# ducha-aiki/mods

Hardware: AMD Instinct MI355X
Metric: image-pairs/sec (1024x768, HessAff+RootSIFT over the affine view ladder, MFMA FGINN match, LO-RANSAC H) (higher is better)
Workload: dtype f32 (detect/describe) + u8 on the int8 matrix cores (distance matrix)

## Files before the change

### include/modsx.h

```cpp
#ifndef MODSX_H
#define MODSX_H
#include <stdint.h>
#ifdef __cplusplus
extern "C" {
#endif

#define MODSX_VERSION 100

typedef enum modsx_status {
  MODSX_OK = 0,
  MODSX_ERR_ARG = -1,
  MODSX_ERR_DEVICE = -2,
  MODSX_ERR_NOMEM = -3,
  MODSX_ERR_INTERNAL = -4,
  MODSX_ERR_CAPACITY = -5,
  MODSX_ERR_TIMEOUT = -6
} modsx_status;

enum { MODSX_FIXED_TH = 0, MODSX_RELATIVE_TH = 1, MODSX_FIXED_REG_NUMBER = 2, MODSX_RELATIVE_REG_NUMBER = 3,
       MODSX_NOT_LESS_THAN_REGIONS = 4 };
enum { MODSX_DET_HESSIAN = 0, MODSX_DET_DOG = 1, MODSX_DET_HARRIS = 2, MODSX_DET_MSER = 3 };
enum { MODSX_DESC_SIFT = 0, MODSX_DESC_ROOT_SIFT = 1, MODSX_DESC_HALF_SIFT = 2, MODSX_DESC_HALF_ROOT_SIFT = 3 };
#define MODSX_MAX_DESC 4
enum { MODSX_HESSIAN_DARK = 0, MODSX_HESSIAN_BRIGHT = 1, MODSX_HESSIAN_SADDLE = 2 };
// ... 40 lines not shown
  int reg_number;
  float rel_threshold, rel_reg_number;
} modsx_mser_params;

typedef struct modsx_sskp {
  int octave, level, r0, c0, r, c, type, pad;
  float b0, b1, b2, val;
  float x, y, s, pixelDistance;
} modsx_sskp;

typedef struct modsx_tentative {
  int q, t0, tj, t1;
  double d1, d2, d2by2ndcl, ratio;
} modsx_tentative;

typedef struct modsx_pair_params {
  modsx_hessaff_params det;
  double ori_mrSize; int ori_patchSize; int ori_maxAngles; double ori_threshold;
  double desc_mrSize; int desc_patchSize; int desc_photoNorm; int desc_type; double desc_maxBinValue;
  double match_ratio; double contradDist; int nn;
  double duplicateDist;
  double err_threshold, confidence; int max_samples; int localOptimization; double HLAFCoef; int doSymmCheck;
  unsigned ransac_seed;
  int useF;
  double LAFCoef;
  int errorType;
  int detector;
  modsx_mser_params mser;
  int n_desc;
  int desc_types[MODSX_MAX_DESC];
  double desc_ratios[MODSX_MAX_DESC];
} modsx_pair_params;

typedef struct modsx_pair_result {
  int n_regions1, n_regions2;
  int n_tentatives;
  int n_unique;
  int n_ransac_inliers;
  int n_verified;
  int ransac_samples, ransac_lo;
  double H[9];
  modsx_tentative *tentatives;
  unsigned char *ransac_inlier;
  unsigned char *verified;
} modsx_pair_result;

typedef struct modsx_view {
  double zoom, tilt, phi, InitSigma;
  int doBlur;
} modsx_view;

typedef struct modsx_ctx modsx_ctx;
typedef struct modsx_image modsx_image;

int modsx_version(void);
const char *modsx_last_error(void);
void modsx_free(void *p);

modsx_ctx *modsx_create(int device_id);
void modsx_destroy(modsx_ctx *ctx);
int modsx_synchronize(modsx_ctx *ctx);

void modsx_default_hessaff_params(modsx_hessaff_params *p);
void modsx_default_pair_params(modsx_pair_params *p);

modsx_image *modsx_image_upload(modsx_ctx *ctx, const void *pixels, int rows, int cols, int channels, int dtype);
int modsx_image_update(modsx_ctx *ctx, modsx_image *img, const void *pixels, int rows, int cols, int channels, int dtype);
modsx_image *modsx_image_wrap_device(modsx_ctx *ctx, const float *dev_pixels, int rows, int cols);
void modsx_image_free(modsx_ctx *ctx, modsx_image *img);
int modsx_image_download(modsx_ctx *ctx, const modsx_image *img, float *out);

int modsx_detect_affine_keypoints(modsx_ctx *ctx, const modsx_image *img, const modsx_hessaff_params *par,
                                  double tilt, double zoom, modsx_keypoint **out);
int modsx_detect_scalespace(modsx_ctx *ctx, const modsx_image *img, const modsx_hessaff_params *par,
                            modsx_sskp **out);
int modsx_octave_levels(modsx_ctx *ctx, const modsx_image *img, const modsx_hessaff_params *par, float *blurs,
                        float *resps);
int modsx_gaussian_blur(modsx_ctx *ctx, const modsx_image *img, float sigma, float *out);
int modsx_resize_half(modsx_ctx *ctx, const modsx_image *img, float *out, int *orows, int *ocols);

int modsx_response(modsx_ctx *ctx, const modsx_image *img, int detector_type, float norm, float *out);

int modsx_detect_affine_regions(const modsx_keypoint *kps, int n, int img_id, int det_type, modsx_region *out);

void modsx_default_mser_params(modsx_mser_params *p);
int modsx_detect_msers(modsx_ctx *ctx, const modsx_image *img, const modsx_mser_params *par, double tilt, double zoom,
                       modsx_keypoint **out);
int modsx_detect_msers_u8(const unsigned char *gray, int rows, int cols, const modsx_mser_params *par, double tilt,
                          double zoom, modsx_keypoint **out);

int modsx_detect_orientation(modsx_ctx *ctx, const modsx_image *img, const modsx_region *in, int n, double mrSize,
                             int patchSize, int doHalfSIFT, int maxAngNum, double th, int addUpRight,
                             modsx_region **out);

int modsx_reproject_regions(modsx_region *regs, int n, const double *H, int orig_w, int orig_h);
int modsx_reproject_regions_touch_boundary(modsx_region *regs, int n, const double *H, int orig_w, int orig_h, double mrSize);

int modsx_describe_regions(modsx_ctx *ctx, const modsx_image *img, const modsx_region *regs, int n, double mrSize,
                           int patchSize, int fast_extraction, int photoNorm, int desc_type, double maxBinValue,
                           float *desc);

int modsx_match_fginn(modsx_ctx *ctx, const float *desc1, int n1, const float *desc2, int n2, const double *pos2,
                      double ratio, double contradDist, int nn, modsx_tentative **out);

int modsx_duplicate_filtering(const double *pts, const double *key, int T, double r, int do_sort, int *order,
                              unsigned char *keep);

int modsx_ransac_h(const double *u, int len, double th, double conf, int max_sam, double *H, unsigned char *inl,
                   int *data_out, int oriented_constraint, int doSymCheck, unsigned seed, double *score_J);

int modsx_loransac_h(const double *pts, const double *laf1, const double *laf2, int T, double err_threshold,
                     double confidence, int max_samples, int localOptimization, double HLAFCoef, int doSymmCheck,
                     unsigned seed, double *H, double *Hraw, unsigned char *inl, unsigned char *keep,
                     int *data_out);

int modsx_ransac_h_errtype(const double *u, int len, double th, double conf, int max_sam, double *H, unsigned char *inl,
                           int *data_out, int oriented_constraint, int doSymCheck, int error_type, unsigned seed,
                           double *score_J);
int modsx_loransac_h_errtype(const double *pts, const double *laf1, const double *laf2, int T, double err_threshold,
                             double confidence, int max_samples, int localOptimization, double HLAFCoef, int doSymmCheck,
                             int error_type, unsigned seed, double *H, double *Hraw, unsigned char *inl,
                             unsigned char *keep, int *data_out);

int modsx_ransac_f(const double *u, int len, double th, double conf, int max_sam, int do_lo, unsigned inl_limit,
                   int error_type, int doSymCheck, unsigned seed, double *F, unsigned char *inl, int *data_out);

int modsx_loransac_f(const double *pts, const double *laf1, const double *laf2, int T, double err_threshold,
                     double confidence, int max_samples, int localOptimization, double LAFCoef, int doSymmCheck,
                     int error_type, unsigned seed, double *F, unsigned char *inl, unsigned char *keep, int *data_out);
int modsx_verify_device_stats(long *out, int reset);
int modsx_verify_device_timing(long *out, int reset);

int modsx_match_pair(modsx_ctx *ctx, const modsx_image *img1, const modsx_image *img2,
                     const modsx_pair_params *par, modsx_pair_result *res);
void modsx_pair_result_release(modsx_pair_result *res);

int modsx_match_pairs(modsx_ctx *const *ctxs, int n_ctx, const modsx_image *const *imgs1,
                      const modsx_image *const *imgs2, int n_pairs, const modsx_pair_params *par,
                      modsx_pair_result *results);

int modsx_match_pairs_views(modsx_ctx *const *ctxs, int n_ctx, const modsx_image *const *imgs1,
                            const modsx_image *const *imgs2, int n_pairs, const modsx_view *views, int n_views,
                            const modsx_pair_params *par, modsx_pair_result *results);

int modsx_last_batch_verify(double *sum_ms, int *pairs, int *threads);
int modsx_last_match_geometry(int *qs, int *fat, int *S, int *tiles_per_split, int *ntiles_ub);
int modsx_describe_counters(modsx_ctx *ctx, long *out, int n);
int modsx_debug_orientation_counts(unsigned long long *launched, unsigned long long *skipped, int reset);
int modsx_debug_reproject_certain_drop(const modsx_region *regs, int n, const double *H, int orig_w, int orig_h, double boxk,
                                       unsigned char *drop);
int modsx_debug_describe_plan(const modsx_region *regs, const int *counts, int nimages, double mr_size, int fast_extraction,
                              unsigned long long arena_floats, long *counters, int n, long *cuts, int cap_cuts, int *n_cuts);
int modsx_debug_baumberg_geometry(int n, int W, int variant, int chunk, int *geometry);
int modsx_debug_baumberg(modsx_ctx *ctx, const modsx_image *const *planes, int nplanes, const int *plane_of, const float *xyspd,
                         int n, const modsx_hessaff_params *par, int variant, int chunk, float *u, int *ok, int *iters,
                         int *geometry);
int modsx_debug_check_borders(const float *tuples, int n, unsigned char *touch);
int modsx_last_timings(modsx_ctx *ctx, double *ms6);

int modsx_set_vs_pars(const double *scale_set, int ns, const double *tilt_set, int nt, double phi_base,
                      double InitSigma, int doBlur, modsx_view *par, int cap, modsx_view *prev, int *nprev,
                      int cap_prev);

modsx_image *modsx_synth_view(modsx_ctx *ctx, const modsx_image *gray, const modsx_view *view, double *H9,
                              int *is_identity);

int modsx_detect_describe_views(modsx_ctx *ctx, const modsx_image *img, const modsx_view *views, int nviews,
                                const modsx_pair_params *par, int view_begin, int view_step, modsx_region **regs,
                                float **desc, void *dev_desc_u8, long dev_cap, int *view_counts);

int modsx_match_fginn_device(modsx_ctx *ctx, const void *dev_desc1_u8, int n1, const void *dev_desc2_u8, int n2,
                             const double *pos2, double ratio, double contradDist, int nn, modsx_tentative **out);

#define MODSX_DB_MAX_ROWS 16777216L
typedef struct modsx_db modsx_db;
modsx_db *modsx_db_create(modsx_ctx *ctx, const void *rows, long n, int dtype);
void modsx_db_free(modsx_ctx *ctx, modsx_db *db);
long modsx_db_rows(const modsx_db *db);
int modsx_db_nearest(modsx_ctx *ctx, const modsx_db *db, const float *desc, int n, float *dmin);
int modsx_match_fginn_db(modsx_ctx *ctx, const float *desc1, int n1, const float *desc2, int n2, const double *pos2,
                         double ratio, double contradDist, int nn, const modsx_db *db, modsx_tentative **out, double **d2byDB);
int modsx_match_fginn_db_device(modsx_ctx *ctx, const void *dev_desc1_u8, int n1, const void *dev_desc2_u8, int n2,
                                const double *pos2, double ratio, double contradDist, int nn, const modsx_db *db,
                                modsx_tentative **out, double **d2byDB);
int modsx_set_fginn_db(modsx_ctx *ctx, const modsx_db *db);

int modsx_match_pair_views(modsx_ctx *ctx, const modsx_image *img1, const modsx_image *img2,
                           const modsx_view *views, int nviews, const modsx_pair_params *par,
                           modsx_pair_result *res);

typedef struct modsx_ladder_step {
  const modsx_view *views;
  int nviews;
  double match_ratio;
  int detector;
  int n_desc;
  int desc_types[MODSX_MAX_DESC];
  double desc_ratios[MODSX_MAX_DESC];
} modsx_ladder_step;
int modsx_match_ladder(modsx_ctx *ctx, const modsx_image *img1, const modsx_image *img2,
                       const modsx_ladder_step *steps, int nsteps, int min_matches, const modsx_pair_params *par,
                       modsx_pair_result *res, int *steps_done);

typedef struct modsx_rep modsx_rep;
modsx_rep *modsx_rep_create(modsx_ctx *ctx);
void modsx_rep_free(modsx_ctx *ctx, modsx_rep *rep);
int modsx_rep_add_views(modsx_ctx *ctx, modsx_rep *rep, const modsx_image *img, const modsx_ladder_step *step,
                        const modsx_pair_params *par);
int modsx_rep_append(modsx_ctx *ctx, modsx_rep *rep, int detector, int desc_type, const modsx_region *regs, const void *desc, int dtype,
                     int n);
int modsx_rep_class(modsx_ctx *ctx, const modsx_rep *rep, int detector, int desc_type, modsx_region **regs, unsigned char **desc_u8);
int modsx_rep_match_fginn(modsx_ctx *ctx, const modsx_rep *rep1, const modsx_rep *rep2, int detector, int desc_type, double ratio,
                          double contradDist, int nn, modsx_tentative **out);
typedef struct { int detector, desc_type; double ratio; } modsx_rep_class_sel;
int modsx_match_reps(modsx_ctx *const *ctxs, int n_ctx, const modsx_rep *rep1, const modsx_rep *const *reps2, int n,
                     const modsx_rep_class_sel *classes, int n_classes, const modsx_pair_params *par, modsx_pair_result *results);
int modsx_match_one_to_many(modsx_ctx *const *ctxs, int n_ctx, const modsx_image *img1, const modsx_image *const *imgs2, int n,
                            const modsx_ladder_step *steps, int nsteps, int min_matches, const modsx_pair_params *par,
                            modsx_pair_result *results, int *steps_done);

typedef struct modsx_comm modsx_comm;
int modsx_comm_unique_id(void *id128);
int modsx_comm_loopback_id(void *id128, int world);
modsx_comm *modsx_comm_create(modsx_ctx *ctx, const void *id128, int rank, int world);
void modsx_comm_destroy(modsx_comm *comm);
int modsx_comm_set_lanes(modsx_comm *comm, int nlanes);
int modsx_comm_attach(modsx_comm *comm, modsx_ctx *ctx, int lane);
int modsx_comm_lane_done(modsx_comm *comm, int lane);
int modsx_comm_reset_lanes(modsx_comm *comm);
int modsx_comm_set_timeout(modsx_comm *comm, int milliseconds);
int modsx_comm_info(const modsx_comm *comm, int *rank, int *world, int *rccl_version, long *bytes_gathered, long *collectives);
int modsx_comm_stats(const modsx_comm *comm, long *out, int n);
#define MODSX_EXCHANGE_ALL_GATHER 0
#define MODSX_EXCHANGE_OWNER 1
int modsx_comm_set_exchange(modsx_comm *comm, int mode);
int modsx_shard_owner_plan(const int *item_counts, int nimages, int nviews, int world, int rank, const int *image_owner, int *sends,
                           int *recvs, int *jobs, int cap, long *n);
int modsx_view_block_order(const int *counts, int world, int nviews, int *src, int cap, int *maxrows_out);
#define MODSX_SHARD_ROW_REGION 0
#define MODSX_SHARD_ROW_KP 1
long modsx_shard_block_bytes(int items, int block_rows, int ndesc, int row_format);
long modsx_shard_block_pack(const modsx_region *regs, const unsigned char *const *desc, int ndesc, int n, const int *counts, int items,
                            int rc_local, int block_rows, int row_format, void *block);
long modsx_shard_blocks_unpack(const void *blocks, int world, int items, int block_rows, int ndesc, int row_format, void *regs_out,
                               unsigned char *const *desc_out, long cap, int *item_counts, int *need_rows);
long modsx_shard_device_pack(modsx_ctx *ctx, const modsx_region *regs, const unsigned char *const *desc, int ndesc, int n, int row_format,
                             void *rows_out);
long modsx_shard_device_unpack(modsx_ctx *ctx, const void *blocks, int world, int items, int block_rows, int ndesc, int row_format,
                               void *regs_out, unsigned char *const *desc_out, double *pos_out, long cap);
int modsx_detect_describe_views_sharded(modsx_ctx *ctx, modsx_comm *comm, const modsx_image *img, const modsx_view *views,
                                        int nviews, const modsx_pair_params *par, modsx_region **regs, void **dev_desc_u8,
                                        int *view_counts);
int modsx_match_fginn_sharded(modsx_ctx *ctx, modsx_comm *comm, const void *dev_desc1_u8, int n1, const void *dev_desc2_u8,
                              int n2, const double *pos2, double ratio, double contradDist, int nn, modsx_tentative **out);
int modsx_match_pair_views_sharded(modsx_ctx *ctx, modsx_comm *comm, const modsx_image *img1, const modsx_image *img2,
                                   const modsx_view *views, int nviews, const modsx_pair_params *par, int owner,
                                   modsx_pair_result *res);
int modsx_match_pairs_views_sharded(modsx_ctx *ctx, modsx_comm *comm, const modsx_image *const *imgs1, const modsx_image *const *imgs2,
                                    int n_pairs, const modsx_view *views, int nviews, const modsx_pair_params *par, int owner_base,
                                    modsx_pair_result *results);
int modsx_match_ladder_sharded(modsx_ctx *ctx, modsx_comm *comm, const modsx_image *img1, const modsx_image *img2,
                               const modsx_ladder_step *steps, int nsteps, int min_matches, const modsx_pair_params *par,
                               modsx_pair_result *res, int *steps_done);

typedef struct modsx_region_class {
  const char *det_name, *desc_name;
  const modsx_region *regs;
  const float *desc;
  int n, dim, stride;
} modsx_region_class;
int modsx_save_regions(const char *path, const modsx_region_class *classes, int nclasses);
int modsx_load_regions(const char *path, const char *det_name, const char *desc_name, modsx_region **regs, float **desc,
                       int *dim, char *found_det, char *found_desc);

int modsx_profile(modsx_ctx *ctx, int enable);
int modsx_kernel_stats(modsx_ctx *ctx, double *ms, double *work, long *launches, int n);

#ifdef __cplusplus
}
#endif
#endif
```

### mods_amd/__init__.py

```python
import ctypes as C
import os
import subprocess

import numpy as np

_HERE = os.path.dirname(os.path.abspath(__file__))
LIB_PATH = os.environ.get("MODSX_LIB", os.path.join(_HERE, "libmodsx.so"))

KEYPOINT = np.dtype([("x", "f8"), ("y", "f8"), ("a11", "f8"), ("a12", "f8"), ("a21", "f8"), ("a22", "f8"),
                     ("s", "f8"), ("response", "f8"), ("octave_number", "i4"), ("pyramid_scale", "f8"),
                     ("sub_type", "i4")], align=True)
REGION = np.dtype([("img_id", "i4"), ("img_reproj_id", "i4"), ("id", "i4"), ("parent_id", "i4"), ("type", "i4"),
                   ("det_kp", KEYPOINT), ("reproj_kp", KEYPOINT)], align=True)
SSKP = np.dtype([("octave", "i4"), ("level", "i4"), ("r0", "i4"), ("c0", "i4"), ("r", "i4"), ("c", "i4"),
                 ("type", "i4"), ("pad", "i4"), ("b0", "f4"), ("b1", "f4"), ("b2", "f4"), ("val", "f4"),
                 ("x", "f4"), ("y", "f4"), ("s", "f4"), ("pixelDistance", "f4")], align=True)
TENT = np.dtype([("q", "i4"), ("t0", "i4"), ("tj", "i4"), ("t1", "i4"), ("d1", "f8"), ("d2", "f8"),
                 ("d2by2ndcl", "f8"), ("ratio", "f8")], align=True)


class HessAffParams(C.Structure):
    _fields_ = [("threshold", C.c_float), ("mode", C.c_int), ("reg_number", C.c_int),
                ("rel_threshold", C.c_float), ("rel_reg_number", C.c_float), ("numberOfScales", C.c_int),
                ("initialSigma", C.c_float), ("edgeEigenValueRatio", C.c_double), ("border", C.c_int),
                ("maxIterations", C.c_int), ("convergenceThreshold", C.c_float), ("smmWindowSize", C.c_int),
                ("affInitialSigma", C.c_float), ("doBaumberg", C.c_int), ("detectorType", C.c_int)]


class MserParams(C.Structure):
    _fields_ = [("min_size", C.c_int), ("max_area", C.c_double), ("min_margin", C.c_double), ("relative", C.c_int),
                ("mode", C.c_int), ("reg_number", C.c_int), ("rel_threshold", C.c_float), ("rel_reg_number", C.c_float)]


class PairParams(C.Structure):
    _fields_ = [("det", HessAffParams),
                ("ori_mrSize", C.c_double), ("ori_patchSize", C.c_int), ("ori_maxAngles", C.c_int),
                ("ori_threshold", C.c_double),
                ("desc_mrSize", C.c_double), ("desc_patchSize", C.c_int), ("desc_photoNorm", C.c_int),
                ("desc_type", C.c_int), ("desc_maxBinValue", C.c_double),
                ("match_ratio", C.c_double), ("contradDist", C.c_double), ("nn", C.c_int),
                ("duplicateDist", C.c_double),
                ("err_threshold", C.c_double), ("confidence", C.c_double), ("max_samples", C.c_int),
                ("localOptimization", C.c_int), ("HLAFCoef", C.c_double), ("doSymmCheck", C.c_int),
                ("ransac_seed", C.c_uint), ("useF", C.c_int), ("LAFCoef", C.c_double), ("errorType", C.c_int),
                ("detector", C.c_int), ("mser", MserParams),
                ("n_desc", C.c_int), ("desc_types", C.c_int * 4), ("desc_ratios", C.c_double * 4)]


class View(C.Structure):
    _fields_ = [("zoom", C.c_double), ("tilt", C.c_double), ("phi", C.c_double), ("InitSigma", C.c_double),
                ("doBlur", C.c_int)]


def make_view(tilt=1.0, phi=0.0, zoom=1.0, init_sigma=0.5, do_blur=1):
    v = View()
    v.zoom, v.tilt, v.phi, v.InitSigma, v.doBlur = zoom, tilt, phi, init_sigma, do_blur
    return v


def _view_array(views):
    arr = (View * len(views))()
    for i, v in enumerate(views):
        arr[i].zoom, arr[i].tilt, arr[i].phi, arr[i].InitSigma, arr[i].doBlur = v.zoom, v.tilt, v.phi, v.InitSigma, v.doBlur
    return arr


class LadderStep(C.Structure):
    _fields_ = [("views", C.c_void_p), ("nviews", C.c_int), ("match_ratio", C.c_double), ("detector", C.c_int),
                ("n_desc", C.c_int), ("desc_types", C.c_int * 4), ("desc_ratios", C.c_double * 4)]


class PairResult(C.Structure):
    _fields_ = [("n_regions1", C.c_int), ("n_regions2", C.c_int), ("n_tentatives", C.c_int), ("n_unique", C.c_int),
                ("n_ransac_inliers", C.c_int), ("n_verified", C.c_int), ("ransac_samples", C.c_int),
                ("ransac_lo", C.c_int), ("H", C.c_double * 9), ("tentatives", C.c_void_p),
                ("ransac_inlier", C.c_void_p), ("verified", C.c_void_p)]


class RepClassSel(C.Structure):
    _fields_ = [("detector", C.c_int), ("desc_type", C.c_int), ("ratio", C.c_double)]


EXPORTS = ["modsx_version", "modsx_last_error", "modsx_free", "modsx_create", "modsx_destroy", "modsx_synchronize",
           "modsx_default_hessaff_params", "modsx_default_pair_params", "modsx_image_upload", "modsx_image_update",
           "modsx_image_wrap_device", "modsx_image_free", "modsx_image_download", "modsx_detect_affine_keypoints",
           "modsx_detect_scalespace", "modsx_octave_levels", "modsx_gaussian_blur", "modsx_resize_half", "modsx_response",
           "modsx_detect_affine_regions", "modsx_detect_orientation", "modsx_reproject_regions", "modsx_reproject_regions_touch_boundary",
           "modsx_describe_regions", "modsx_match_fginn", "modsx_duplicate_filtering", "modsx_ransac_h",
           "modsx_loransac_h", "modsx_ransac_h_errtype", "modsx_loransac_h_errtype", "modsx_ransac_f", "modsx_loransac_f", "modsx_match_pair", "modsx_match_pairs", "modsx_match_pairs_views", "modsx_pair_result_release",
           "modsx_set_vs_pars", "modsx_synth_view", "modsx_detect_describe_views", "modsx_match_fginn_device",
           "modsx_match_pair_views", "modsx_match_ladder", "modsx_save_regions", "modsx_load_regions", "modsx_default_mser_params", "modsx_detect_msers", "modsx_detect_msers_u8", "modsx_last_timings", "modsx_profile",
           "modsx_kernel_stats", "modsx_last_batch_verify", "modsx_last_match_geometry", "modsx_describe_counters", "modsx_comm_unique_id", "modsx_comm_create", "modsx_comm_destroy", "modsx_comm_info",
           "modsx_view_block_order", "modsx_detect_describe_views_sharded", "modsx_match_fginn_sharded",
           "modsx_match_pair_views_sharded", "modsx_match_pairs_views_sharded", "modsx_match_ladder_sharded", "modsx_comm_loopback_id", "modsx_comm_set_lanes",
           "modsx_comm_attach", "modsx_comm_lane_done", "modsx_comm_reset_lanes", "modsx_comm_set_timeout", "modsx_comm_stats",
           "modsx_shard_block_bytes", "modsx_shard_block_pack", "modsx_shard_blocks_unpack", "modsx_shard_device_pack",
           "modsx_shard_device_unpack", "modsx_verify_device_stats", "modsx_verify_device_timing", "modsx_comm_set_exchange",
           "modsx_shard_owner_plan", "modsx_db_create", "modsx_db_free", "modsx_db_rows", "modsx_db_nearest",
           "modsx_match_fginn_db", "modsx_match_fginn_db_device", "modsx_set_fginn_db",
           "modsx_debug_orientation_counts", "modsx_debug_reproject_certain_drop", "modsx_debug_describe_plan",
           "modsx_debug_baumberg_geometry", "modsx_debug_baumberg", "modsx_debug_check_borders",
           "modsx_rep_create", "modsx_rep_free", "modsx_rep_add_views", "modsx_rep_append", "modsx_rep_class",
           "modsx_rep_match_fginn", "modsx_match_reps", "modsx_match_one_to_many"]
EXPORTS_DEGENSAC = ["exp_ransacHcustom", "exp_ransacFcustom", "HDs", "HDsi", "HDsidx", "HDsSym", "HDsiSym", "HDsSymidx",
                    "HDsSymMax", "HDsiSymMax", "HDsSymidxMax", "FDs", "FDsSym", "exFDs", "exFDsSym",
                    "modsx_ransac_set_seed"]

SHARD_ROW_REGION, SHARD_ROW_KP = 0, 1
EXCHANGE_ALL_GATHER, EXCHANGE_OWNER = 0, 1
DESCRIBE_COUNTERS = ("calls", "chunks", "max_chunks", "chunks_mid_image", "chunks_later_image", "jobs", "direct_jobs", "fused_windows",
                     "lds_row_tiles", "lds_col_tiles", "sample_tiles", "global_row_tiles", "global_col_tiles", "clamped_windows")
KP_FIELDS = ("x", "y", "a11", "a12", "a21", "a22", "s")
KERNEL_CLASSES = ["blur_hess", "hessian", "resize", "nms_localize", "baumberg", "orientation", "patch_sample",
                  "blur_rows", "describe", "match_fginn", "gray", "warp_affine", "view_blur", "blur_cols", "match_sweep1", "match_db"]


def build(force=False):
    src = os.path.join(_HERE, "csrc")
    srcs = [os.path.join(src, f) for f in os.listdir(src) if f.endswith((".hip", ".cpp", ".hpp"))]
    srcs.append(os.path.join(_HERE, "..", "include", "modsx.h"))
    stale = (not os.path.exists(LIB_PATH)) or any(os.path.getmtime(s) > os.path.getmtime(LIB_PATH) for s in srcs)
    if force or stale:
        subprocess.check_call(["make", "-C", src, "-j8"], stdout=subprocess.DEVNULL)
    return LIB_PATH


_lib = None


def lib():
    global _lib
    if _lib is None:
        if not os.path.exists(LIB_PATH):
            raise RuntimeError("libmodsx.so is not built; run __graft_entry__.build() (needs hipcc)")
        L = C.CDLL(LIB_PATH)
        L.modsx_last_error.restype = C.c_char_p
        L.modsx_create.restype = C.c_void_p
        L.modsx_create.argtypes = [C.c_int]
        L.modsx_comm_create.restype = C.c_void_p
        L.modsx_comm_create.argtypes = [C.c_void_p, C.c_void_p, C.c_int, C.c_int]
        L.modsx_comm_destroy.argtypes = [C.c_void_p]
        L.modsx_comm_info.argtypes = [C.c_void_p] + [C.c_void_p] * 5
        L.modsx_comm_loopback_id.argtypes = [C.c_void_p, C.c_int]
        L.modsx_comm_set_lanes.argtypes = [C.c_void_p, C.c_int]
        L.modsx_comm_attach.argtypes = [C.c_void_p, C.c_void_p, C.c_int]
        L.modsx_comm_lane_done.argtypes = [C.c_void_p, C.c_int]
        L.modsx_comm_reset_lanes.argtypes = [C.c_void_p]
        L.modsx_comm_set_timeout.argtypes = [C.c_void_p, C.c_int]
        L.modsx_comm_stats.argtypes = [C.c_void_p, C.c_void_p, C.c_int]
        L.modsx_destroy.argtypes = [C.c_void_p]
        L.modsx_free.argtypes = [C.c_void_p]
        L.modsx_image_upload.restype = C.c_void_p
        L.modsx_image_upload.argtypes = [C.c_void_p, C.c_void_p, C.c_int, C.c_int, C.c_int, C.c_int]
        L.modsx_image_update.argtypes = [C.c_void_p, C.c_void_p, C.c_void_p, C.c_int, C.c_int, C.c_int, C.c_int]
        L.modsx_debug_last_batch_verify_each.argtypes = [C.c_void_p, C.c_int]
        L.modsx_image_wrap_device.restype = C.c_void_p
        L.modsx_image_wrap_device.argtypes = [C.c_void_p, C.c_void_p, C.c_int, C.c_int]
        L.modsx_image_free.argtypes = [C.c_void_p, C.c_void_p]
        L.modsx_db_create.restype = C.c_void_p
        L.modsx_db_create.argtypes = [C.c_void_p, C.c_void_p, C.c_long, C.c_int]
        L.modsx_db_free.restype = None
        L.modsx_db_free.argtypes = [C.c_void_p, C.c_void_p]
        L.modsx_db_rows.restype = C.c_long
        L.modsx_db_rows.argtypes = [C.c_void_p]
        L.modsx_db_nearest.argtypes = [C.c_void_p, C.c_void_p, C.c_void_p, C.c_int, C.c_void_p]
        L.modsx_set_fginn_db.argtypes = [C.c_void_p, C.c_void_p]
        L.modsx_debug_reproject_certain_drop.argtypes = [C.c_void_p, C.c_int, C.c_void_p, C.c_int, C.c_int, C.c_double, C.c_void_p]
        L.modsx_describe_counters.argtypes = [C.c_void_p, C.c_void_p, C.c_int]
        L.modsx_debug_orientation_counts.argtypes = [C.c_void_p, C.c_void_p, C.c_int]
        L.modsx_debug_describe_plan.argtypes = [C.c_void_p, C.c_void_p, C.c_int, C.c_double, C.c_int, C.c_ulonglong, C.c_void_p, C.c_int,
                                                C.c_void_p, C.c_int, C.c_void_p]
        L.modsx_debug_baumberg_geometry.argtypes = [C.c_int, C.c_int, C.c_int, C.c_int, C.c_void_p]
        L.modsx_debug_baumberg.argtypes = [C.c_void_p, C.c_void_p, C.c_int, C.c_void_p, C.c_void_p, C.c_int, C.c_void_p, C.c_int, C.c_int,
                                           C.c_void_p, C.c_void_p, C.c_void_p, C.c_void_p]
        L.modsx_debug_check_borders.argtypes = [C.c_void_p, C.c_int, C.c_void_p]
        L.modsx_rep_create.restype = C.c_void_p
        L.modsx_rep_create.argtypes = [C.c_void_p]
        L.modsx_rep_free.restype = None
        L.modsx_rep_free.argtypes = [C.c_void_p, C.c_void_p]
        L.modsx_rep_add_views.argtypes = [C.c_void_p, C.c_void_p, C.c_void_p, C.c_void_p, C.c_void_p]
        L.modsx_rep_append.argtypes = [C.c_void_p, C.c_void_p, C.c_int, C.c_int, C.c_void_p, C.c_void_p, C.c_int, C.c_int]
        L.modsx_rep_class.argtypes = [C.c_void_p, C.c_void_p, C.c_int, C.c_int, C.c_void_p, C.c_void_p]
        L.modsx_rep_match_fginn.argtypes = [C.c_void_p, C.c_void_p, C.c_void_p, C.c_int, C.c_int, C.c_double, C.c_double, C.c_int,
                                            C.c_void_p]
        L.modsx_match_reps.argtypes = [C.c_void_p, C.c_int, C.c_void_p, C.c_void_p, C.c_int, C.c_void_p, C.c_int, C.c_void_p,
                                       C.c_void_p]
        L.modsx_match_one_to_many.argtypes = [C.c_void_p, C.c_int, C.c_void_p, C.c_void_p, C.c_int, C.c_void_p, C.c_int, C.c_int,
                                              C.c_void_p, C.c_void_p, C.c_void_p]
        L.modsx_synth_view.restype = C.c_void_p
        L.modsx_synth_view.argtypes = [C.c_void_p, C.c_void_p, C.c_void_p, C.c_void_p, C.c_void_p]
        _lib = L
    return _lib


def _err():
    return lib().modsx_last_error().decode()


def _p(a):
    return a.ctypes.data_as(C.c_void_p)


def _check(rc, what):
    if rc < 0:
        raise RuntimeError("%s failed (%d): %s" % (what, rc, _err()))
    return rc


def default_hessaff_params(**kw):
    p = HessAffParams()
    lib().modsx_default_hessaff_params(C.byref(p))
    for k, v in kw.items():
        setattr(p, k, v)
    return p


def default_mser_params(**kw):
    p = MserParams()
    lib().modsx_default_mser_params(C.byref(p))
    for k, v in kw.items():
        setattr(p, k, v)
    return p


def detect_msers_u8(gray, params=None, tilt=1.0, zoom=1.0):
    params = params or default_mser_params()
    g = np.ascontiguousarray(gray, np.uint8)
    out = C.c_void_p()
    n = _check(lib().modsx_detect_msers_u8(_p(g), g.shape[0], g.shape[1], C.byref(params), C.c_double(tilt),
                                           C.c_double(zoom), C.byref(out)), "detect_msers_u8")
    return _take(out, n, KEYPOINT)


def default_pair_params(**kw):
    p = PairParams()
    lib().modsx_default_pair_params(C.byref(p))
    descs = kw.pop("descs", None)
    if descs is not None:
        _set_descs(p, descs)
    for k, v in kw.items():
        if hasattr(p.det, k) and not hasattr(p, k):
            setattr(p.det, k, v)
        else:
            setattr(p, k, v)
    return p


def _set_descs(obj, descs):
    obj.n_desc = len(descs)
    for i, (t, r) in enumerate(descs):
        obj.desc_types[i] = int(t)
        obj.desc_ratios[i] = float(r)


def _take(ptr, n, dtype):
    if n <= 0:
        if ptr:
            lib().modsx_free(ptr)
        return np.zeros(0, dtype)
    buf = (C.c_char * (n * dtype.itemsize)).from_address(ptr.value if hasattr(ptr, "value") else ptr)
    arr = np.frombuffer(buf, dtype=dtype, count=n).copy()
    lib().modsx_free(ptr)
    return arr


def detect_affine_regions(kps, img_id=0, det_type=0):
    kps = np.ascontiguousarray(kps, KEYPOINT)
    out = np.zeros(len(kps), REGION)
    _check(lib().modsx_detect_affine_regions(_p(kps), len(kps), img_id, det_type, _p(out)), "detect_affine_regions")
    return out


def reproject_regions(regs, H, w, h):
    regs = np.ascontiguousarray(regs, REGION).copy()
    H = np.ascontiguousarray(H, np.float64).reshape(9)
    n = _check(lib().modsx_reproject_regions(_p(regs), len(regs), _p(H), int(w), int(h)), "reproject_regions")
    return regs[:n].copy()


def reproject_regions_touch_boundary(regs, H, w, h, mr_size=3.0 * 3.0 ** 0.5):
    regs = np.ascontiguousarray(regs, REGION).copy()
    H = np.ascontiguousarray(H, np.float64).reshape(9)
    n = _check(lib().modsx_reproject_regions_touch_boundary(_p(regs), len(regs), _p(H), int(w), int(h), C.c_double(mr_size)),
               "reproject_regions_touch_boundary")
    return regs[:n].copy()


def duplicate_filtering(pts, key, r=2.0, do_sort=True):
    pts = np.ascontiguousarray(pts, np.float64)
    key = np.ascontiguousarray(key, np.float64)
    T = len(pts)
    order = np.zeros(max(T, 1), np.int32)
    keep = np.zeros(max(T, 1), np.uint8)
    _check(lib().modsx_duplicate_filtering(_p(pts), _p(key), T, C.c_double(r), int(do_sort), _p(order), _p(keep)),
           "duplicate_filtering")
    return order[:T], keep[:T].astype(bool)


def ransac_h(u, th, conf=0.99, max_sam=100000, oriented=1, sym_check=1, seed=1):
    u = np.ascontiguousarray(u, np.float64)
    n = len(u)
    H = np.zeros(9)
    inl = np.zeros(n, np.uint8)
    dout = np.zeros(3, np.int32)
    J = C.c_double(0)
    rc = _check(lib().modsx_ransac_h(_p(u), n, C.c_double(th), C.c_double(conf), int(max_sam), _p(H), _p(inl), _p(dout),
                                     int(oriented), int(sym_check), C.c_uint(seed), C.byref(J)), "ransac_h")
    return dict(n=rc, H=H, inl=inl.astype(bool), samples=int(dout[0]), lo_count=int(dout[1]),
                ori_rejects=int(dout[2]), J=J.value)


def loransac_h(pts, laf1, laf2, err_threshold=3.0, confidence=0.99, max_samples=100000, lo=1, hlaf_coef=12.0,
               sym_check=1, seed=1, error_type=0):
    pts = np.ascontiguousarray(pts, np.float64)
    laf1 = np.ascontiguousarray(laf1, np.float64)
    laf2 = np.ascontiguousarray(laf2, np.float64)
    T = len(pts)
    H, Hraw = np.zeros(9), np.zeros(9)
    inl = np.zeros(max(T, 1), np.uint8)
    keep = np.zeros(max(T, 1), np.uint8)
    dout = np.zeros(3, np.int32)
    n = _check(lib().modsx_loransac_h_errtype(_p(pts), _p(laf1), _p(laf2), T, C.c_double(err_threshold),
                                              C.c_double(confidence), int(max_samples), int(lo), C.c_double(hlaf_coef),
                                              int(sym_check), int(error_type), C.c_uint(seed), _p(H), _p(Hraw), _p(inl),
                                              _p(keep), _p(dout)), "loransac_h")
    return dict(n=n, H=H.reshape(3, 3), Hraw=Hraw, inl=inl[:T].astype(bool), keep=keep[:T].astype(bool),
                samples=int(dout[0]), lo_count=int(dout[1]), ori_rejects=int(dout[2]))
# ... 105 lines not shown
        return int(lib().modsx_db_rows(self.h)) if self.h else 0

    def free(self):
        if self.h:
            lib().modsx_db_free(self.ctx.h, self.h)
            self.h = None


def _ladder_steps(steps):
    arr = (LadderStep * len(steps))()
    keep = []
    for i, st in enumerate(steps):
        va = _view_array(st[0])
        keep.append(va)
        arr[i].views = C.cast(va, C.c_void_p)
        arr[i].nviews = len(st[0])
        arr[i].match_ratio = float(st[1])
        arr[i].detector = int(st[2]) if len(st) > 2 else 0
        if len(st) > 3 and st[3] is not None:
            _set_descs(arr[i], st[3])
    return arr, keep


class Rep(object):

    def __init__(self, ctx):
        self.ctx = ctx
        self.h = lib().modsx_rep_create(ctx.h)
        if not self.h:
            raise RuntimeError("modsx_rep_create failed: " + _err())

    def add_views(self, img, views, params, detector=0, descs=None, ctx=None):
        arr, keep = _ladder_steps([(views, 0.0, detector, descs)])
        return _check(lib().modsx_rep_add_views((ctx or self.ctx).h, self.h, img.h, arr, C.addressof(params)), "rep_add_views")

    def append(self, regs, desc, detector=0, desc_type=1, ctx=None):
        regs = np.ascontiguousarray(regs, REGION)
        d = np.ascontiguousarray(desc)
        if d.dtype != np.uint8:
            d = np.ascontiguousarray(d, np.float32)
        if d.shape != (len(regs), 128):
            raise ValueError("rep.append: [n][128] descriptors for n regions are expected")
        return _check(lib().modsx_rep_append((ctx or self.ctx).h, self.h, int(detector), int(desc_type), _p(regs), _p(d),
                                             0 if d.dtype == np.uint8 else 1, len(regs)), "rep_append")

    def regions(self, detector=0, desc_type=1, want_desc=True):
        regs, desc = C.c_void_p(), C.c_void_p()
        n = _check(lib().modsx_rep_class(self.ctx.h, self.h, int(detector), int(desc_type), C.byref(regs),
                                         C.byref(desc) if want_desc else None), "rep_class")
        r = _take(regs, n, REGION)
        if not want_desc:
            return r
        return r, _take(desc, n * 128, np.dtype(np.uint8)).reshape(n, 128)

    def count(self, detector=0, desc_type=1):
        return _check(lib().modsx_rep_class(self.ctx.h, self.h, int(detector), int(desc_type), None, None), "rep_class")

    def free(self):
        if self.h:
            lib().modsx_rep_free(self.ctx.h, self.h)
            self.h = None


class Context(object):

    def __init__(self, device=0):
        self.h = lib().modsx_create(int(device))
        if not self.h:
            raise RuntimeError("modsx_create failed: " + _err())

    def close(self):
        if self.h:
            lib().modsx_destroy(self.h)
            self.h = None

    def __del__(self):
        try:
            self.close()
        except Exception:
            pass

    def _c(self):
        return C.c_void_p(self.h)

    def upload(self, pixels):
        a = np.ascontiguousarray(pixels)
        if a.dtype == np.uint8:
            dtype = 0
        else:
            a = np.ascontiguousarray(a, np.float32)
            dtype = 1
        ch = 1 if a.ndim == 2 else a.shape[2]
        h = lib().modsx_image_upload(self._c(), _p(a), a.shape[0], a.shape[1], ch, dtype)
        if not h:
            raise RuntimeError("modsx_image_upload failed: " + _err())
        return Image(self, h, a.shape[0], a.shape[1])

    def wrap_device(self, dev_ptr, rows, cols):
        h = lib().modsx_image_wrap_device(self._c(), C.c_void_p(dev_ptr), rows, cols)
        if not h:
            raise RuntimeError("modsx_image_wrap_device failed: " + _err())
        return Image(self, h, rows, cols)

    def synchronize(self):
        _check(lib().modsx_synchronize(self._c()), "synchronize")

    def gaussian_blur(self, img, sigma):
        out = np.empty((img.rows, img.cols), np.float32)
        _check(lib().modsx_gaussian_blur(self._c(), C.c_void_p(img.h), C.c_float(sigma), _p(out)), "gaussian_blur")
        return out

    def response(self, img, detector_type, norm):
        out = np.zeros((img.rows, img.cols), np.float32)
        _check(lib().modsx_response(self._c(), C.c_void_p(img.h), int(detector_type), C.c_float(norm), _p(out)), "response")
        return out

    def resize_half(self, img):
        r, c = C.c_int(), C.c_int()
        _check(lib().modsx_resize_half(self._c(), C.c_void_p(img.h), None, C.byref(r), C.byref(c)), "resize_half")
        out = np.empty((r.value, c.value), np.float32)
        _check(lib().modsx_resize_half(self._c(), C.c_void_p(img.h), _p(out), C.byref(r), C.byref(c)), "resize_half")
        return out

    def octave_levels(self, img, params):
        L = params.numberOfScales + 2
        blurs = np.empty((L, img.rows, img.cols), np.float32)
        resps = np.empty((L, img.rows, img.cols), np.float32)
        _check(lib().modsx_octave_levels(self._c(), C.c_void_p(img.h), C.byref(params), _p(blurs), _p(resps)),
               "octave_levels")
        return blurs, resps

    def detect_scalespace(self, img, params):
        out = C.c_void_p()
        n = _check(lib().modsx_detect_scalespace(self._c(), C.c_void_p(img.h), C.byref(params), C.byref(out)),
                   "detect_scalespace")
        return _take(out, n, SSKP)

    def detect_affine_keypoints(self, img, params, tilt=1.0, zoom=1.0):
        out = C.c_void_p()
        n = _check(lib().modsx_detect_affine_keypoints(self._c(), C.c_void_p(img.h), C.byref(params),
                                                       C.c_double(tilt), C.c_double(zoom), C.byref(out)),
                   "detect_affine_keypoints")
        return _take(out, n, KEYPOINT)

    def debug_baumberg(self, planes, plane_of, xyspd, params, variant=0, chunk=0):
        plane_of = np.ascontiguousarray(plane_of, np.int32)
        xyspd = np.ascontiguousarray(xyspd, np.float32).reshape(-1, 4)
        n = len(plane_of)
        assert len(xyspd) == n
        ptrs = (C.c_void_p * max(1, len(planes)))(*[im.h for im in planes])
        u = np.zeros((max(n, 1), 4), np.float32)
        ok, iters = np.zeros(max(n, 1), np.int32), np.zeros(max(n, 1), np.int32)
        geo = np.zeros(4, np.int32)
        _check(lib().modsx_debug_baumberg(self._c(), ptrs, len(planes), _p(plane_of), _p(xyspd), n, C.byref(params), int(variant),
                                          int(chunk), _p(u), _p(ok), _p(iters), _p(geo)), "debug_baumberg")
        return dict(u=u[:n], ok=ok[:n], iters=iters[:n], geometry=dict(zip(BAUMBERG_GEOMETRY, (int(x) for x in geo))))

    def detect_orientation(self, img, regs, mr_size=1.0, patch_size=41, half=0, max_ang=1, th=0.8, upright=0):
        regs = np.ascontiguousarray(regs, REGION)
        out = C.c_void_p()
        n = _check(lib().modsx_detect_orientation(self._c(), C.c_void_p(img.h), _p(regs), len(regs),
                                                  C.c_double(mr_size), patch_size, half, max_ang, C.c_double(th),
                                                  upright, C.byref(out)), "detect_orientation")
        return _take(out, n, REGION)

    def describe_regions(self, img, regs, mr_size=5.1962, patch_size=41, fast=0, photo_norm=1, desc_type=1,
                         max_bin=0.2):
        regs = np.ascontiguousarray(regs, REGION)
        desc = np.zeros((len(regs), 128), np.float32)
        _check(lib().modsx_describe_regions(self._c(), C.c_void_p(img.h), _p(regs), len(regs), C.c_double(mr_size),
                                            patch_size, fast, photo_norm, desc_type, C.c_double(max_bin), _p(desc)),
               "describe_regions")
        return desc

    def describe_counters(self):
        v = (C.c_long * len(DESCRIBE_COUNTERS))()
        n = _check(lib().modsx_describe_counters(self._c(), v, len(DESCRIBE_COUNTERS)), "describe_counters")
        assert n == len(DESCRIBE_COUNTERS), n
        return dict(zip(DESCRIBE_COUNTERS, (int(x) for x in v)))

    def match_fginn(self, d1, d2, pos2, ratio=0.8, contrad_dist=30.0, nn=50):
        d1 = np.ascontiguousarray(d1, np.float32)
        d2 = np.ascontiguousarray(d2, np.float32)
        pos2 = np.ascontiguousarray(pos2, np.float64)
        out = C.c_void_p()
        n = _check(lib().modsx_match_fginn(self._c(), _p(d1), len(d1), _p(d2), len(d2), _p(pos2), C.c_double(ratio),
                                           C.c_double(contrad_dist), nn, C.byref(out)), "match_fginn")
        return _take(out, n, TENT)

    def db_create(self, rows):
        a = np.ascontiguousarray(rows)
        if a.dtype != np.uint8:
            a = np.ascontiguousarray(a, np.float32)
        if a.ndim != 2 or a.shape[1] != 128:
            raise ValueError("db_create: an [n][128] array is expected")
        h = lib().modsx_db_create(self._c(), _p(a), a.shape[0], 0 if a.dtype == np.uint8 else 1)
        if not h:
            raise RuntimeError("modsx_db_create failed: " + _err())
        return Db(self, h)

    def db_nearest(self, db, desc):
        d = np.ascontiguousarray(desc, np.float32)
        out = np.empty(len(d), np.float32)
        _check(lib().modsx_db_nearest(self._c(), C.c_void_p(db.h), _p(d), len(d), _p(out)), "db_nearest")
        return out

    def match_fginn_db(self, d1, d2, pos2, db, ratio=0.8, contrad_dist=30.0, nn=50):
        d1 = np.ascontiguousarray(d1, np.float32)
        d2 = np.ascontiguousarray(d2, np.float32)
        pos2 = np.ascontiguousarray(pos2, np.float64)
        out, dd = C.c_void_p(), C.c_void_p()
        n = _check(lib().modsx_match_fginn_db(self._c(), _p(d1), len(d1), _p(d2), len(d2), _p(pos2), C.c_double(ratio),
                                              C.c_double(contrad_dist), nn, C.c_void_p(db.h if db is not None else None),
                                              C.byref(out), C.byref(dd)), "match_fginn_db")
        return _take(out, n, TENT), _take(dd, n, np.dtype("f8"))

    def match_fginn_db_device(self, d1_ptr, n1, d2_ptr, n2, pos2, db, ratio=0.8, contrad_dist=30.0, nn=50):
        pos2 = np.ascontiguousarray(pos2, np.float64)
        out, dd = C.c_void_p(), C.c_void_p()
        n = _check(lib().modsx_match_fginn_db_device(self._c(), C.c_void_p(d1_ptr), int(n1), C.c_void_p(d2_ptr), int(n2),
                                                     _p(pos2), C.c_double(ratio), C.c_double(contrad_dist), nn,
                                                     C.c_void_p(db.h), C.byref(out), C.byref(dd)), "match_fginn_db_device")
        return _take(out, n, TENT), _take(dd, n, np.dtype("f8"))

    def set_fginn_db(self, db):
        _check(lib().modsx_set_fginn_db(self._c(), C.c_void_p(db.h) if db is not None else None), "set_fginn_db")

    def synth_view(self, img, view):
        H = np.zeros(9)
        ident = C.c_int(0)
        h = lib().modsx_synth_view(self._c(), C.c_void_p(img.h), C.byref(view), _p(H), C.byref(ident))
        if not h:
            raise RuntimeError("modsx_synth_view failed: " + _err())
        rows, cols = C.c_int(), C.c_int()
        out = Image(self, h, 0, 0)
        out.rows, out.cols = _image_dims(h)
        return out, H.reshape(3, 3), bool(ident.value)

    def detect_describe_views(self, img, views, params, view_begin=0, view_step=1, want_desc=True, dev_desc=None,
                              dev_cap=0, want_counts=False):
        arr = _view_array(views)
        regs = C.c_void_p()
        desc = C.c_void_p()
        counts = (C.c_int * len(views))()
        n = _check(lib().modsx_detect_describe_views(self._c(), C.c_void_p(img.h), arr, len(views), C.byref(params),
                                                     int(view_begin), int(view_step), C.byref(regs),
                                                     C.byref(desc) if want_desc else None,
                                                     C.c_void_p(dev_desc) if dev_desc else None, C.c_long(dev_cap),
                                                     counts),
                   "detect_describe_views")
        r = _take(regs, n, REGION)
        d = None
        if want_desc:
            d = _take(desc, n * 128, np.dtype("f4")).reshape(n, 128) if n else np.zeros((0, 128), np.float32)
        if want_counts:
            return r, d, np.array(list(counts), np.int64)
        return r, d

    def match_fginn_device(self, d1_ptr, n1, d2_ptr, n2, pos2, ratio=0.8, contrad_dist=30.0, nn=50):
        pos2 = np.ascontiguousarray(pos2, np.float64)
        out = C.c_void_p()
        n = _check(lib().modsx_match_fginn_device(self._c(), C.c_void_p(d1_ptr), int(n1), C.c_void_p(d2_ptr), int(n2),
                                                  _p(pos2), C.c_double(ratio), C.c_double(contrad_dist), nn,
                                                  C.byref(out)), "match_fginn_device")
        return _take(out, n, TENT)

    def rep_match_fginn(self, rep1, rep2, detector=0, desc_type=1, ratio=0.8, contrad_dist=30.0, nn=50):
        out = C.c_void_p()
        n = _check(lib().modsx_rep_match_fginn(self.h, rep1.h, rep2.h, int(detector), int(desc_type), C.c_double(ratio),
                                               C.c_double(contrad_dist), int(nn), C.byref(out)), "rep_match_fginn")
        return _take(out, n, TENT)

    def match_pair_views(self, img1, img2, views, params):
        arr = _view_array(views)
        res = PairResult()
        _check(lib().modsx_match_pair_views(self._c(), C.c_void_p(img1.h), C.c_void_p(img2.h), arr, len(views),
                                            C.byref(params), C.byref(res)), "match_pair_views")
        return _unpack_pair_result(res)

    def comm_create(self, id128, rank, world):
        h = lib().modsx_comm_create(self._c(), id128, int(rank), int(world))
        if not h:
            raise RuntimeError("modsx_comm_create failed: " + _err())
        return h

    def detect_describe_views_sharded(self, comm, img, views, params):
        arr = _view_array(views)
        regs, dptr = C.c_void_p(), C.c_void_p()
        counts = (C.c_int * len(views))()
        n = _check(lib().modsx_detect_describe_views_sharded(self._c(), C.c_void_p(comm), C.c_void_p(img.h), arr, len(views),
                                                             C.byref(params), C.byref(regs), C.byref(dptr), counts),
                   "detect_describe_views_sharded")
        return _take(regs, n, REGION), dptr.value, np.array(list(counts), np.int64)

    def match_fginn_sharded(self, comm, d1_ptr, n1, d2_ptr, n2, pos2, ratio=0.8, contrad_dist=30.0, nn=50):
        pos2 = np.ascontiguousarray(pos2, np.float64)
        out = C.c_void_p()
        n = _check(lib().modsx_match_fginn_sharded(self._c(), C.c_void_p(comm), C.c_void_p(d1_ptr), int(n1), C.c_void_p(d2_ptr),
                                                   int(n2), _p(pos2), C.c_double(ratio), C.c_double(contrad_dist), nn,
                                                   C.byref(out)), "match_fginn_sharded")
        return _take(out, n, TENT)

    def match_pair_views_sharded(self, comm, img1, img2, views, params, owner=0):
        arr = _view_array(views)
        res = PairResult()
        _check(lib().modsx_match_pair_views_sharded(self._c(), C.c_void_p(comm), C.c_void_p(img1.h), C.c_void_p(img2.h), arr,
                                                    len(views), C.byref(params), int(owner), C.byref(res)),
               "match_pair_views_sharded")
        return _unpack_pair_result(res)

    def match_pairs_views_sharded(self, comm, imgs1, imgs2, views, params, owner_base=0, arrays=True):
        n = len(imgs1)
        a1 = (C.c_void_p * n)(*[im.h for im in imgs1])
        a2 = (C.c_void_p * n)(*[im.h for im in imgs2])
        arr = _view_array(views)
        res = (PairResult * n)()
        _check(lib().modsx_match_pairs_views_sharded(self._c(), C.c_void_p(comm), a1, a2, n, arr, len(views), C.byref(params),
                                                     int(owner_base), res), "match_pairs_views_sharded")
        return [_unpack_pair_result(res[i], arrays) for i in range(n)]

    def shard_device_pack(self, regs, descs, row_format=SHARD_ROW_REGION):
        L = lib()
        L.modsx_shard_device_pack.restype = C.c_long
        regs = np.ascontiguousarray(regs, REGION)
        descs = [np.ascontiguousarray(d, np.uint8) for d in descs]
        out = np.zeros((len(regs), shard_region_bytes(row_format) + 128 * len(descs)), np.uint8)
        _check(L.modsx_shard_device_pack(self._c(), _p(regs), _ptr_array(descs), len(descs), len(regs), int(row_format), _p(out)),
               "shard_device_pack")
        return out

    def shard_device_unpack(self, blocks, world, items, block_rows, ndesc=1, row_format=SHARD_ROW_REGION):
        L = lib()
        L.modsx_shard_device_unpack.restype = C.c_long
        blocks = np.ascontiguousarray(blocks, np.uint8)
        cap = world * block_rows
        regs = np.zeros(cap, REGION) if row_format == SHARD_ROW_REGION else np.zeros((cap, 7), np.float64)
        descs = [np.zeros((cap, 128), np.uint8) for _ in range(ndesc)]
        pos = np.zeros((cap, 2), np.float64)
        _check(L.modsx_shard_device_unpack(self._c(), _p(blocks), int(world), int(items), int(block_rows), int(ndesc), int(row_format),
                                           _p(regs), _ptr_array(descs), _p(pos), C.c_long(cap)), "shard_device_unpack")
        return regs, descs, pos

    def detect_msers(self, img, params=None, tilt=1.0, zoom=1.0):
        params = params or default_mser_params()
        out = C.c_void_p()
        n = _check(lib().modsx_detect_msers(self._c(), C.c_void_p(img.h), C.byref(params), C.c_double(tilt),
                                            C.c_double(zoom), C.byref(out)), "detect_msers")
        return _take(out, n, KEYPOINT)

    def match_ladder(self, img1, img2, steps, params, min_matches=10, comm=None):
        arr = (LadderStep * len(steps))()
        keep = []
        for i, st in enumerate(steps):
            views, ratio = st[0], st[1]
            va = _view_array(views)
            keep.append(va)
            arr[i].views = C.cast(va, C.c_void_p)
            arr[i].nviews = len(views)
            arr[i].match_ratio = float(ratio)
            arr[i].detector = int(st[2]) if len(st) > 2 else 0
            if len(st) > 3 and st[3] is not None:
                _set_descs(arr[i], st[3])
        res = PairResult()
        done = C.c_int(0)
        if comm is not None:
            _check(lib().modsx_match_ladder_sharded(self._c(), C.c_void_p(comm), C.c_void_p(img1.h), C.c_void_p(img2.h), arr,
                                                    len(steps), int(min_matches), C.byref(params), C.byref(res),
                                                    C.byref(done)), "match_ladder_sharded")
        else:
            _check(lib().modsx_match_ladder(self._c(), C.c_void_p(img1.h), C.c_void_p(img2.h), arr, len(steps),
                                            int(min_matches), C.byref(params), C.byref(res), C.byref(done)), "match_ladder")
        return _unpack_pair_result(res), done.value

    def match_pair(self, img1, img2, params):
        res = PairResult()
        _check(lib().modsx_match_pair(self._c(), C.c_void_p(img1.h), C.c_void_p(img2.h), C.byref(params),
                                      C.byref(res)), "match_pair")
        return _unpack_pair_result(res)

    def last_timings(self):
        t = (C.c_double * 6)()
        _check(lib().modsx_last_timings(self._c(), t), "last_timings")
        return dict(zip(["detect", "orient", "describe", "match", "verify", "total"], list(t)))

    def profile(self, enable=True):
        _check(lib().modsx_profile(self._c(), int(enable)), "profile")

    def kernel_stats(self):
        n = len(KERNEL_CLASSES)
        ms, work = (C.c_double * n)(), (C.c_double * n)()
        launches = (C.c_long * n)()
        _check(lib().modsx_kernel_stats(self._c(), ms, work, launches, n), "kernel_stats")
        return {k: dict(ms=ms[i], work=work[i], launches=launches[i]) for i, k in enumerate(KERNEL_CLASSES)}


class _ImageStruct(C.Structure):
    _fields_ = [("d", C.c_void_p), ("rows", C.c_int), ("cols", C.c_int), ("owned", C.c_bool)]


def last_batch_verify_each():
    n = lib().modsx_debug_last_batch_verify_each(None, 0)
    out = np.zeros(max(n, 1), np.float64)
    n = min(n, lib().modsx_debug_last_batch_verify_each(_p(out), len(out)))
    return out[:n]


def last_batch_verify():
    ms, n, t = C.c_double(), C.c_int(), C.c_int()
    lib().modsx_last_batch_verify(C.byref(ms), C.byref(n), C.byref(t))
    return ms.value, n.value, t.value


def last_match_geometry():
    v = [C.c_int() for _ in range(5)]
    lib().modsx_last_match_geometry(*[C.byref(x) for x in v])
    return dict(zip(("qs", "fat", "S", "tiles_per_split", "ntiles_ub"), (x.value for x in v)))


BAUMBERG_GEOMETRY = ("kernel", "chunk", "nchunks", "grid")


def baumberg_geometry(n, W=19, variant=0, chunk=0):
    geo = np.zeros(4, np.int32)
    _check(lib().modsx_debug_baumberg_geometry(int(n), int(W), int(variant), int(chunk), _p(geo)), "baumberg_geometry")
    return dict(zip(BAUMBERG_GEOMETRY, (int(x) for x in geo)))


def check_borders(tuples):
    t = np.ascontiguousarray(tuples, np.float32).reshape(-1, 9)
    out = np.zeros(max(1, len(t)), np.uint8)
    _check(lib().modsx_debug_check_borders(_p(t), len(t), _p(out)), "check_borders")
    return out[:len(t)].astype(bool)


def orientation_counts(reset=False):
    a, b = C.c_ulonglong(), C.c_ulonglong()
    lib().modsx_debug_orientation_counts(C.byref(a), C.byref(b), int(reset))
    return a.value, b.value


def reproject_certain_drop(regs, H, w, h, boxk=2 * 3.0 * 3.0 ** 0.5):
    regs = np.ascontiguousarray(regs, REGION)
    H = np.ascontiguousarray(H, np.float64).reshape(9)
    drop = np.zeros(max(1, len(regs)), np.uint8)
    _check(lib().modsx_debug_reproject_certain_drop(_p(regs), len(regs), _p(H), int(w), int(h), C.c_double(boxk), _p(drop)),
           "reproject_certain_drop")
    return drop[:len(regs)].astype(bool)


DEFAULT_ARENA_FLOATS = 192 << 18


def describe_plan(regs, mr_size, fast=0, arena_floats=DEFAULT_ARENA_FLOATS, max_cuts=4096):
    lists = [regs] if isinstance(regs, np.ndarray) else list(regs)
    counts = np.array([len(r) for r in lists], np.int32)
    flat = np.ascontiguousarray(np.concatenate([np.asarray(r).view(REGION) for r in lists]) if lists else np.zeros(0, REGION), REGION)
    cnt = (C.c_long * len(DESCRIBE_COUNTERS))()
    cuts = (C.c_long * max(1, max_cuts))()
    ncuts = C.c_int(0)
    rc = lib().modsx_debug_describe_plan(_p(flat), _p(counts), len(lists), C.c_double(mr_size), int(fast), int(arena_floats), cnt,
                                         len(DESCRIBE_COUNTERS), cuts, max_cuts, C.byref(ncuts))
    assert ncuts.value <= max_cuts, "describe_plan: %d cuts, room for %d" % (ncuts.value, max_cuts)
    return dict(rc=rc, error=_err() if rc else "", counters=dict(zip(DESCRIBE_COUNTERS, (int(x) for x in cnt))),
                cuts=[int(cuts[i]) for i in range(ncuts.value)])


def view_block_order(counts):
    counts = np.ascontiguousarray(counts, np.int32)
    world, nviews = counts.shape
    total = int(counts.sum())
    src = np.zeros(max(1, total), np.int32)
    mr = C.c_int(0)
    n = _check(lib().modsx_view_block_order(_p(counts), world, nviews, _p(src), len(src), C.byref(mr)), "view_block_order")
    return src[:n].copy(), mr.value


def shard_owner_plan(item_counts, nviews, world, rank, image_owner):
    cnt = np.ascontiguousarray(item_counts, np.int32)
    own = np.ascontiguousarray(image_owner, np.int32)
    nimg = len(own)
    assert len(cnt) == nimg * nviews
    cap = max(1, len(cnt), nimg * world)
    sends, recvs, jobs = (np.zeros((cap, 4), np.int32) for _ in range(3))
    n = (C.c_long * 5)()
    L = lib()
    L.modsx_shard_owner_plan.argtypes = [C.c_void_p, C.c_int, C.c_int, C.c_int, C.c_int, C.c_void_p, C.c_void_p, C.c_void_p, C.c_void_p, C.c_int, C.c_void_p]
    _check(L.modsx_shard_owner_plan(_p(cnt), nimg, nviews, world, rank, _p(own), _p(sends), _p(recvs), _p(jobs), cap, n), "shard_owner_plan")
    return {"sends": sends[:n[0]].copy(), "recvs": recvs[:n[1]].copy(), "jobs": jobs[:n[2]].copy(), "recv_rows": int(n[3]), "list_rows": int(n[4])}


def _ptr_array(arrs):
    return (C.c_void_p * len(arrs))(*[a.ctypes.data for a in arrs])


def shard_region_bytes(row_format):
    return REGION.itemsize if row_format == SHARD_ROW_REGION else 56


def shard_kp_rows(regs):
    k = np.asarray(regs)["reproj_kp"]
    return np.stack([k[f] for f in KP_FIELDS], 1).astype(np.float64) if len(k) else np.zeros((0, 7))


def shard_block_bytes(items, block_rows, ndesc=1, row_format=SHARD_ROW_REGION):
    L = lib()
    L.modsx_shard_block_bytes.restype = C.c_long
    return int(L.modsx_shard_block_bytes(int(items), int(block_rows), int(ndesc), int(row_format)))


def shard_block_pack(regs, descs, counts, block_rows, rc_local=0, row_format=SHARD_ROW_REGION):
    L = lib()
    L.modsx_shard_block_pack.restype = C.c_long
    regs = np.ascontiguousarray(regs, REGION)
    descs = [np.ascontiguousarray(d, np.uint8) for d in descs]
    counts = np.ascontiguousarray(counts, np.int32)
    out = np.zeros(shard_block_bytes(len(counts), block_rows, len(descs), row_format), np.uint8)
    n = _check(L.modsx_shard_block_pack(_p(regs), _ptr_array(descs), len(descs), len(regs), _p(counts), len(counts), int(rc_local),
                                        int(block_rows), int(row_format), _p(out)), "shard_block_pack")
    assert n == len(out)
    return out


def shard_blocks_unpack(blocks, world, items, block_rows, ndesc=1, cap=None, row_format=SHARD_ROW_REGION):
    L = lib()
    L.modsx_shard_blocks_unpack.restype = C.c_long
    blocks = np.ascontiguousarray(blocks, np.uint8)
    cap = int(cap if cap is not None else world * block_rows)
    regs = np.zeros(max(1, cap), REGION) if row_format == SHARD_ROW_REGION else np.zeros((max(1, cap), 7), np.float64)
    descs = [np.zeros((max(1, cap), 128), np.uint8) for _ in range(ndesc)]
    cnt = np.zeros(items, np.int32)
    need = C.c_int(0)
    n = L.modsx_shard_blocks_unpack(_p(blocks), int(world), int(items), int(block_rows), int(ndesc), int(row_format), _p(regs),
                                    _ptr_array(descs), C.c_long(cap), _p(cnt), C.byref(need))
    if n == -5:
        return None, None, need.value
    _check(n, "shard_blocks_unpack")
    return regs[:n].copy(), [d[:n].copy() for d in descs], cnt


def comm_unique_id():
    buf = C.create_string_buffer(128)
    _check(lib().modsx_comm_unique_id(buf), "comm_unique_id")
    return buf.raw


def comm_loopback_id(world):
    buf = C.create_string_buffer(128)
    _check(lib().modsx_comm_loopback_id(buf, int(world)), "comm_loopback_id")
    return buf.raw


COMM_STATS = ["collectives", "bytes_gathered", "block_retries", "agreements", "lanes", "loopback", "dead", "turn_wait_us", "bytes_received",
              "exchanges"]


def comm_stats(comm):
    out = (C.c_long * len(COMM_STATS))()
    lib().modsx_comm_stats(C.c_void_p(comm), out, len(COMM_STATS))
    return dict(zip(COMM_STATS, list(out)))


def _image_dims(handle):
    st = _ImageStruct.from_address(handle)
    return st.rows, st.cols


def match_pairs(ctxs, imgs1, imgs2, params):
    n = len(imgs1)
    carr = (C.c_void_p * len(ctxs))(*[c.h for c in ctxs])
    a1 = (C.c_void_p * n)(*[im.h for im in imgs1])
    a2 = (C.c_void_p * n)(*[im.h for im in imgs2])
    res = (PairResult * n)()
    _check(lib().modsx_match_pairs(carr, len(ctxs), a1, a2, n, C.byref(params), res), "match_pairs")
    return [_unpack_pair_result(res[i]) for i in range(n)]


def match_pairs_views(ctxs, imgs1, imgs2, views, params, arrays=True):
    n = len(imgs1)
    carr = (C.c_void_p * len(ctxs))(*[c.h for c in ctxs])
    a1 = (C.c_void_p * n)(*[im.h for im in imgs1])
# ... 51 lines not shown
```

### mods_amd/csrc/capi.hip

```cpp
#include <math.h>
#include <malloc.h>
#include <atomic>
#include <chrono>
#include <mutex>
#include <thread>
#include <condition_variable>
#include <deque>
#include "engine_api.hpp"
#include "describe_plan.hpp"

using namespace mx;

#define NEED(c)                                             \
  do {                                                      \
    if (!(c)) { mx::set_error("null argument: " #c); return MODSX_ERR_ARG; } \
  } while (0)

template <typename T>
static T *to_malloc(const std::vector<T> &v) {
  T *p = (T *)malloc(sizeof(T) * (v.size() ? v.size() : 1));
  if (p && !v.empty()) memcpy(p, v.data(), sizeof(T) * v.size());
  return p;
}

// ... 185 lines not shown
  MX_HIP(hipStreamSynchronize(ctx->stream));
  return L;
}

int modsx_gaussian_blur(modsx_ctx *ctx, const modsx_image *img, float sigma, float *out) {
  NEED(ctx); NEED(img); NEED(out);
  hipSetDevice(ctx->dev);
  const size_t npx = (size_t)img->rows * img->cols;
  if (!ctx->scratchA.ensure(npx * 4)) return MODSX_ERR_NOMEM;
  BlurBatch b;
  memset(&b, 0, sizeof b);
  int n = blur_ksize(sigma);
  if (n > MAX_TAPS) { mx::set_error("modsx_gaussian_blur: ksize > 17"); return MODSX_ERR_ARG; }
  if (n == 1) {
    MX_HIP(hipMemcpyAsync(out, img->d, npx * 4, hipMemcpyDeviceToHost, ctx->stream));
    MX_HIP(hipStreamSynchronize(ctx->stream));
    return MODSX_OK;
  }
  std::vector<float> k = gaussian_kernel(n, sigma);
  b.n = n;
  for (int i = 0; i < n; i++) b.k[i] = k[i];
  b.j[0].src = img->d; b.j[0].blur = (float *)ctx->scratchA.p; b.j[0].resp = nullptr; b.j[0].rows = img->rows;
  b.j[0].cols = img->cols; b.j[0].norm = 1.f;
  launch_blur_hess(ctx->stream, b, 1, img->rows, img->cols);
  MX_HIP(hipMemcpyAsync(out, ctx->scratchA.p, npx * 4, hipMemcpyDeviceToHost, ctx->stream));
  MX_HIP(hipStreamSynchronize(ctx->stream));
  MX_HIP(hipGetLastError());
  return MODSX_OK;
}

static int blur_any(modsx_ctx *c, const float *src, float *dst, float *tmp, float *dTaps, float *hTaps, int rows, int cols, float sigma) {
  const int n = blur_ksize(sigma);
  if (n == 1) { MX_HIP(hipMemcpyAsync(dst, src, (size_t)rows * cols * 4, hipMemcpyDeviceToDevice, c->stream)); return MODSX_OK; }
  const int nx = cols == 1 ? 1 : n, ny = rows == 1 ? 1 : n;
  std::vector<float> kx = gaussian_kernel(nx, sigma), ky = gaussian_kernel(ny, sigma);
  memcpy(hTaps, kx.data(), nx * 4); memcpy(hTaps + nx, ky.data(), ny * 4);
  MX_HIP(hipMemcpyAsync(dTaps, hTaps, (size_t)(nx + ny) * 4, hipMemcpyHostToDevice, c->stream));
  launch_blur_pass(c->stream, src, tmp, rows, cols, dTaps, nx, 0, 1);
  launch_blur_pass(c->stream, tmp, dst, rows, cols, dTaps + nx, ny, 1, 1);
  return MODSX_OK;
}

int modsx_response(modsx_ctx *ctx, const modsx_image *img, int detector_type, float norm, float *out) {
  NEED(ctx); NEED(img); NEED(out);
  if (detector_type != MODSX_DET_HESSIAN && detector_type != MODSX_DET_DOG && detector_type != MODSX_DET_HARRIS) {
    mx::set_error("modsx_response: detector type must be Hessian (0), DoG (1) or Harris (2)");
    return MODSX_ERR_ARG;
  }
  hipSetDevice(ctx->dev);
  hipStream_t s = ctx->stream;
  const int rows = img->rows, cols = img->cols;
  const size_t npx = (size_t)rows * cols;
  const float sigma = detector_type == MODSX_DET_DOG ? norm : sqrtf((float)(0.6 * norm));
  const int ntap = 2 * std::max(1, blur_ksize(sigma)) * 3 + 16;
  if (ntap > 3 * 4096) { mx::set_error("modsx_response: blur kernel too large"); return MODSX_ERR_ARG; }
  if (!ctx->scratchA.ensure(npx * 4 * 8) || !ctx->viewTaps.ensure((size_t)ntap * 4) || !ctx->hViewTaps.ensure((size_t)ntap * 4)) return MODSX_ERR_NOMEM;
  float *buf = (float *)ctx->scratchA.p, *res = buf, *tmp = buf + npx, *a = buf + 2 * npx, *b = buf + 3 * npx, *cc = buf + 4 * npx;
  float *ba = buf + 5 * npx, *bb = buf + 6 * npx, *bc = buf + 7 * npx;
  float *dT = (float *)ctx->viewTaps.p, *hT = (float *)ctx->hViewTaps.p;
  int rc = MODSX_OK;
  if (detector_type == MODSX_DET_HESSIAN) {
    BlurBatch bt;
    memset(&bt, 0, sizeof bt);
    bt.j[0].src = img->d; bt.j[0].resp = res; bt.j[0].rows = rows; bt.j[0].cols = cols; bt.j[0].norm = norm;
    launch_hessian(s, bt, 1, rows, cols);
  } else if (detector_type == MODSX_DET_DOG) {
    rc = blur_any(ctx, img->d, a, tmp, dT, hT, rows, cols, sigma);
    if (rc) return rc;
    launch_sub(s, img->d, a, res, npx);
  } else {
    launch_grad_products(s, img->d, rows, cols, a, b, cc);
    const int n = blur_ksize(sigma);
    rc = blur_any(ctx, a, ba, tmp, dT, hT, rows, cols, sigma);
    if (!rc) rc = blur_any(ctx, b, bb, tmp, dT + 2 * n + 2, hT + 2 * n + 2, rows, cols, sigma);
    if (!rc) rc = blur_any(ctx, cc, bc, tmp, dT + 4 * n + 4, hT + 4 * n + 4, rows, cols, sigma);
    if (rc) return rc;
    launch_harris_combine(s, ba, bb, bc, (float)(0.6 * norm), res, npx);
  }
  MX_HIP(hipMemcpyAsync(out, res, npx * 4, hipMemcpyDeviceToHost, s));
  MX_HIP(hipStreamSynchronize(s));
  MX_HIP(hipGetLastError());
  return MODSX_OK;
}

int modsx_resize_half(modsx_ctx *ctx, const modsx_image *img, float *out, int *orows, int *ocols) {
  NEED(ctx); NEED(img); NEED(orows); NEED(ocols);
  hipSetDevice(ctx->dev);
  const int dr = (int)lrint(img->rows * 0.5), dc = (int)lrint(img->cols * 0.5);
  *orows = dr; *ocols = dc;
  if (!out) return MODSX_OK;
  if (!ctx->scratchA.ensure((size_t)dr * dc * 4 + 4)) return MODSX_ERR_NOMEM;
  ResizeBatch rb;
  memset(&rb, 0, sizeof rb);
  rb.j[0].src = img->d; rb.j[0].dst = (float *)ctx->scratchA.p;
  rb.j[0].srows = img->rows; rb.j[0].scols = img->cols; rb.j[0].drows = dr; rb.j[0].dcols = dc;
  launch_resize_half(ctx->stream, rb, 1, dr, dc);
  MX_HIP(hipMemcpyAsync(out, ctx->scratchA.p, (size_t)dr * dc * 4, hipMemcpyDeviceToHost, ctx->stream));
  MX_HIP(hipStreamSynchronize(ctx->stream));
  MX_HIP(hipGetLastError());
  return MODSX_OK;
}

int modsx_detect_affine_regions(const modsx_keypoint *kps, int n, int img_id, int det_type, modsx_region *out) {
  if (n < 0 || (n > 0 && (!kps || !out))) { mx::set_error("modsx_detect_affine_regions: bad argument"); return MODSX_ERR_ARG; }
  detect_affine_regions(kps, n, img_id, det_type, out);
  return n;
}

int modsx_detect_orientation(modsx_ctx *ctx, const modsx_image *img, const modsx_region *in, int n, double mrSize,
                             int patchSize, int doHalfSIFT, int maxAngNum, double th, int addUpRight,
                             modsx_region **out) {
  NEED(ctx); NEED(img); NEED(out);
  if (n < 0 || (n > 0 && !in)) { mx::set_error("modsx_detect_orientation: bad argument"); return MODSX_ERR_ARG; }
  hipSetDevice(ctx->dev);
  std::vector<modsx_region> vin[1], vout[1];
  vin[0].assign(in, in + n);
  const modsx_image *imgs[1] = {img};
  int rc = detect_orientation_batch(ctx, imgs, 1, vin, mrSize, patchSize, doHalfSIFT, maxAngNum, th, addUpRight, vout);
  if (rc) return rc;
  *out = to_malloc(vout[0]);
  return (int)vout[0].size();
}

int modsx_reproject_regions(modsx_region *regs, int n, const double *H, int orig_w, int orig_h) {
  if (n < 0 || (n > 0 && !regs) || !H) { mx::set_error("modsx_reproject_regions: bad argument"); return MODSX_ERR_ARG; }
  return reproject_regions(regs, n, H, orig_w, orig_h);
}

int modsx_reproject_regions_touch_boundary(modsx_region *regs, int n, const double *H, int orig_w, int orig_h, double mrSize) {
  if (n < 0 || (n > 0 && !regs) || !H) { mx::set_error("modsx_reproject_regions_touch_boundary: bad argument"); return MODSX_ERR_ARG; }
  return reproject_regions_box(regs, n, H, orig_w, orig_h, mrSize);
}

int modsx_debug_reproject_certain_drop(const modsx_region *regs, int n, const double *H, int orig_w, int orig_h, double boxk,
                                       unsigned char *drop) {
  if (n < 0 || (n > 0 && (!regs || !drop)) || !H) { mx::set_error("modsx_debug_reproject_certain_drop: bad argument"); return MODSX_ERR_ARG; }
  reproject_certain_drop(regs, n, H, orig_w, orig_h, boxk, drop);
  return n;
}

int modsx_debug_orientation_counts(unsigned long long *launched, unsigned long long *skipped, int reset) {
  mx::orientation_counts(launched, skipped, reset != 0);
  return MODSX_OK;
}

int modsx_debug_baumberg_geometry(int n, int W, int variant, int chunk, int *geometry) {
  NEED(geometry);
  const mx::BaumGeo g = mx::baumberg_geometry(n, W, variant, chunk);
  geometry[0] = g.kernel; geometry[1] = g.chunk; geometry[2] = g.nchunks; geometry[3] = g.grid;
  if (g.kernel < 0) { mx::set_error("modsx_debug_baumberg_geometry: no kernel for this window size / variant / chunk"); return MODSX_ERR_ARG; }
  return MODSX_OK;
}

int modsx_debug_baumberg(modsx_ctx *ctx, const modsx_image *const *planes, int nplanes, const int *plane_of, const float *xyspd,
                         int n, const modsx_hessaff_params *par, int variant, int chunk, float *u, int *ok, int *iters,
                         int *geometry) {
  NEED(ctx); NEED(par); NEED(geometry);
  if (n < 0 || nplanes < 0 || (nplanes > 0 && !planes) || (n > 0 && (!plane_of || !xyspd || !u || !ok || !iters))) {
    mx::set_error("modsx_debug_baumberg: bad argument"); return MODSX_ERR_ARG;
  }
  hipSetDevice(ctx->dev);
  return debug_baumberg(ctx, planes, nplanes, plane_of, xyspd, n, *par, variant, chunk, u, ok, iters, geometry);
}

int modsx_debug_check_borders(const float *tuples, int n, unsigned char *touch) {
  if (n < 0 || (n > 0 && (!tuples || !touch))) { mx::set_error("modsx_debug_check_borders: bad argument"); return MODSX_ERR_ARG; }
  for (int i = 0; i < n; i++) {
    const float *t = tuples + 9 * (size_t)i;
    touch[i] = mx::check_borders((int)t[0], (int)t[1], t[2], t[3], t[4], t[5], t[6], t[7], (int)t[8], (int)t[8]) ? 1 : 0;
  }
  return n;
}

int modsx_describe_counters(modsx_ctx *ctx, long *out, int n) {
  NEED(ctx);
  if (n < 0 || (n > 0 && !out)) { mx::set_error("modsx_describe_counters: bad argument"); return MODSX_ERR_ARG; }
  long sum[mx::DC_N] = {0};
  for (const modsx_ctx *head : {(const modsx_ctx *)ctx, (const modsx_ctx *)ctx->peer})
    for (const modsx_ctx *c = head; c; c = c->half)
      for (int q = 0; q < mx::DC_N; q++)
        if (q == mx::DC_MAX_CHUNKS) sum[q] = std::max(sum[q], c->descCnt[q]); else sum[q] += c->descCnt[q];
  for (int q = 0; q < n && q < mx::DC_N; q++) out[q] = sum[q];
  return mx::DC_N;
}

int modsx_debug_describe_plan(const modsx_region *regs, const int *counts, int nimages, double mr_size, int fast_extraction,
                              unsigned long long arena_floats, long *counters, int n, long *cuts, int cap_cuts, int *n_cuts) {
  if (nimages < 0 || (nimages > 0 && !counts) || n < 0 || (n > 0 && !counters) || cap_cuts < 0 || (cap_cuts > 0 && !cuts) || !n_cuts) {
    mx::set_error("modsx_debug_describe_plan: bad argument"); return MODSX_ERR_ARG;
  }
  if (nimages > mx::MAXB) { mx::set_error("describe batch too large"); return MODSX_ERR_ARG; }
  std::vector<modsx_region> v[mx::MAXB];
  long first[mx::MAXB + 1] = {0};
  for (int i = 0; i < nimages; i++) {
    if (counts[i] < 0 || (counts[i] > 0 && !regs)) { mx::set_error("modsx_debug_describe_plan: bad argument"); return MODSX_ERR_ARG; }
    v[i].assign(regs + first[i], regs + first[i] + counts[i]);
    first[i + 1] = first[i] + counts[i];
  }
  mx::HostMark hm;
  mx::DescBatch batch;
  batch.regs = v; batch.n = nimages; batch.mrSize = mr_size; batch.fast = fast_extraction;
  mx::DescCursor cur = mx::describe_windows(batch);
  long cnt[mx::DC_N] = {0};
  int chunkNo = 0, rc = MODSX_OK;
  *n_cuts = 0;
  cnt[mx::DC_CALLS]++;
  for (; cur.img < nimages; chunkNo++) {
    mx::DescChunkPlan cp;
    if (chunkNo) { if (*n_cuts < cap_cuts) cuts[*n_cuts] = first[cur.img] + (long)cur.reg; (*n_cuts)++; }
    rc = mx::describe_plan_chunk(batch, cur, (size_t)arena_floats, cp, hm);
    for (int q = 0; q < mx::DC_N; q++) cnt[q] += cp.cnt[q];
    if (rc) break;
    cur = cp.next;
  }
  if (!rc) cnt[mx::DC_MAX_CHUNKS] = chunkNo;
  for (int q = 0; q < n && q < mx::DC_N; q++) counters[q] = cnt[q];
  return rc;
}

int modsx_describe_regions(modsx_ctx *ctx, const modsx_image *img, const modsx_region *regs, int n, double mrSize,
                           int patchSize, int fast_extraction, int photoNorm, int desc_type, double maxBinValue,
                           float *desc) {
  NEED(ctx); NEED(img);
  if (n < 0 || (n > 0 && (!regs || !desc))) { mx::set_error("modsx_describe_regions: bad argument"); return MODSX_ERR_ARG; }
  if (desc_type < MODSX_DESC_SIFT || desc_type > MODSX_DESC_HALF_ROOT_SIFT) { mx::set_error("descriptor type"); return MODSX_ERR_ARG; }
  hipSetDevice(ctx->dev);
  std::vector<modsx_region> v[1];
  v[0].assign(regs, regs + n);
  const modsx_image *imgs[1] = {img};
  float *hosts[1] = {desc};
  int rc = describe_batch(ctx, imgs, 1, v, mrSize, patchSize, fast_extraction, photoNorm, desc_type, maxBinValue, hosts,
                          nullptr, nullptr);
  if (rc) return rc;
  return n;
}

int modsx_match_fginn(modsx_ctx *ctx, const float *desc1, int n1, const float *desc2, int n2, const double *pos2,
                      double ratio, double contradDist, int nn, modsx_tentative **out) {
  NEED(ctx); NEED(out);
  if (n1 < 0 || n2 < 0 || (n1 > 0 && !desc1) || (n2 > 0 && (!desc2 || !pos2))) { mx::set_error("modsx_match_fginn: bad argument"); return MODSX_ERR_ARG; }
  hipSetDevice(ctx->dev);
  std::vector<modsx_tentative> t;
  int rc = match_host_desc(ctx, desc1, n1, desc2, n2, pos2, ratio, contradDist, nn, t);
  if (rc) return rc;
  *out = to_malloc(t);
  return (int)t.size();
}

int modsx_duplicate_filtering(const double *pts, const double *key, int T, double r, int do_sort, int *order,
                              unsigned char *keep) {
  if (T < 0 || (T > 0 && (!pts || !order || !keep))) { mx::set_error("modsx_duplicate_filtering: bad argument"); return MODSX_ERR_ARG; }
  return duplicate_filtering(pts, key, T, r, do_sort, order, keep);
}

int modsx_ransac_h(const double *u, int len, double th, double conf, int max_sam, double *H, unsigned char *inl,
                   int *data_out, int oriented_constraint, int doSymCheck, unsigned seed, double *score_J) {
  if (!u || !H || !inl || !data_out || len < 4) { mx::set_error("modsx_ransac_h: bad argument"); return MODSX_ERR_ARG; }
  return ransac_h(u, len, th, conf, max_sam, H, inl, data_out, oriented_constraint, doSymCheck, seed, score_J);
}

int modsx_ransac_h_errtype(const double *u, int len, double th, double conf, int max_sam, double *H, unsigned char *inl,
                           int *data_out, int oriented_constraint, int doSymCheck, int error_type, unsigned seed, double *score_J) {
  if (!u || !H || !inl || !data_out || len < 4 || error_type < 0 || error_type > 2) { mx::set_error("modsx_ransac_h_errtype: bad argument"); return MODSX_ERR_ARG; }
  return ransac_h(u, len, th, conf, max_sam, H, inl, data_out, oriented_constraint, doSymCheck, seed, score_J, error_type);
}

int modsx_ransac_f(const double *u, int len, double th, double conf, int max_sam, int do_lo, unsigned inl_limit,
                   int error_type, int doSymCheck, unsigned seed, double *F, unsigned char *inl, int *data_out) {
  if (!u || !F || !inl || !data_out || len < 8) { mx::set_error("modsx_ransac_f: bad argument"); return MODSX_ERR_ARG; }
  return ransac_f(u, len, th, conf, max_sam, F, inl, data_out, do_lo, inl_limit, error_type, doSymCheck, seed);
}

int modsx_loransac_f(const double *pts, const double *laf1, const double *laf2, int T, double err_threshold,
                     double confidence, int max_samples, int localOptimization, double LAFCoef, int doSymmCheck,
                     int error_type, unsigned seed, double *F, unsigned char *inl, unsigned char *keep, int *data_out) {
  if (!pts || !laf1 || !laf2 || !F || !inl || !keep || !data_out || T < 0) {
    mx::set_error("modsx_loransac_f: bad argument");
    return MODSX_ERR_ARG;
  }
  return loransac_f(pts, laf1, laf2, T, err_threshold, confidence, max_samples, localOptimization, LAFCoef, doSymmCheck,
                    error_type, seed, F, inl, keep, data_out);
}

int modsx_loransac_h(const double *pts, const double *laf1, const double *laf2, int T, double err_threshold,
                     double confidence, int max_samples, int localOptimization, double HLAFCoef, int doSymmCheck,
                     unsigned seed, double *H, double *Hraw, unsigned char *inl, unsigned char *keep, int *data_out) {
  if (T < 0 || !H || !Hraw || !data_out || (T > 0 && (!pts || !laf1 || !laf2 || !inl || !keep))) {
    mx::set_error("modsx_loransac_h: bad argument");
    return MODSX_ERR_ARG;
  }
  return loransac_h(pts, laf1, laf2, T, err_threshold, confidence, max_samples, localOptimization, HLAFCoef, doSymmCheck,
                    seed, H, Hraw, inl, keep, data_out);
}

int modsx_loransac_h_errtype(const double *pts, const double *laf1, const double *laf2, int T, double err_threshold,
                             double confidence, int max_samples, int localOptimization, double HLAFCoef, int doSymmCheck,
                             int error_type, unsigned seed, double *H, double *Hraw, unsigned char *inl, unsigned char *keep,
                             int *data_out) {
  if (T < 0 || !H || !Hraw || !data_out || (T > 0 && (!pts || !laf1 || !laf2 || !inl || !keep)) || error_type < 0 || error_type > 2) {
    mx::set_error("modsx_loransac_h_errtype: bad argument");
    return MODSX_ERR_ARG;
  }
  return loransac_h(pts, laf1, laf2, T, err_threshold, confidence, max_samples, localOptimization, HLAFCoef, doSymmCheck,
                    seed, H, Hraw, inl, keep, data_out, error_type);
}

static void verify_timed(mx::VerifyTask &t, const modsx_pair_params &pp) {
  const auto v0 = std::chrono::steady_clock::now();
  mx::verify_tentatives(t.l1, t.l2, t.tents, pp, t.res);
  const long us = std::chrono::duration_cast<std::chrono::microseconds>(std::chrono::steady_clock::now() - v0).count();
  g_verifyUs += us;
  g_verifyPairs++;
  std::lock_guard<std::mutex> lk(g_verifyEachMu);
  g_verifyEachUs.push_back((int)us);
}
// ... 672 lines not shown
```

### mods_amd/csrc/engine.hpp

```cpp
#pragma once
#include <hip/hip_runtime.h>
#include <stdint.h>
#include <stdlib.h>
#include <string.h>
#include <string>
#include <vector>
#include "../../include/modsx.h"
#include "kmath.hpp"

namespace mx {

#ifndef MODSX_MAXB
#define MODSX_MAXB 32
#endif
constexpr int MAXB = MODSX_MAXB;
constexpr int PAIR_GROUP = 4;
constexpr int NMS_MAXJ = 1024;
constexpr int MAX_TAPS = 17;

struct BlurJob {
  const float *src;
  float *blur;
  float *resp;
  int rows, cols;
// ... 20 lines not shown
  const float *low, *cur, *high, *blur;
  int rows, cols, img, octave, level, pad;
};
struct NmsBatch {
  float posTh, negTh, finalTh;
  int border;
  double edgeScoreThreshold;
  int detType, pad;
};
struct Candidate {
  int img, octave, level, type;
  int r0, c0, r, c;
  float b0, b1, b2, val;
};

struct AffJob {
  const float *blur;
  int rows, cols;
  float x, y, s, pixelDistance;
};
struct AffOut { float u11, u12, u21, u22; int ok; int iters; };

struct OriJob {
  int img;
  float x, y, a11, a12, a21, a22;
};
constexpr int ORI_MAX_PEAKS = 18;

struct DescJob {
  int img;
  int P;
  int ksize;
  int tapOfs;
  float x, y, a11, a12, a21, a22;
  float i2p;
  int NC;
  int needOfs;
  int coordOfs;
  int touch;
  int outIdx;
  int rows0;
  int ro1;
  unsigned long long scratchOfs;
  unsigned long long rowOfs;
  unsigned long long gridOfs;
};
struct BlurTile {
  unsigned long long srcOfs, dstOfs;
  int P, NC, n, tapOfs, needOfs;
  int job, pad;
  int first, count, lo, span, magic;
};
struct ImgRef { const float *d; int rows, cols, pad; };
struct DescOut { float *f[MAXB]; uint8_t *u8[MAXB]; uint8_t *u8x[3][MAXB]; };

struct WarpJob {
  const float *src;
  float *dst;
  int srows, scols, drows, dcols;
  double M[6];
  float cval;
  int pad;
};

struct ViewJob {
  const float *src;
  float *rot, *tmp, *dst;
  int srows, scols, rrows, rcols, drows, dcols;
  int kx, ky, tapOfs, doBlur;
  int tileA, tileB;
  int tileF, fused;
  int tileG, pad;
  double R[6], W[6];
  double invW[2];
};

struct MatchRow {
  int t0, t1, nless, nbad;
  int tj;
  float dj;
  float d0, d1;
};
static_assert(sizeof(MatchRow) == 32, "match rows are 32 bytes");

struct DevBuf {
  void *p = nullptr;
  size_t cap = 0;
  bool ensure(size_t bytes);
  void release();
};
struct PinBuf {
  void *p = nullptr;
  size_t cap = 0;
  bool ensure(size_t bytes);
  void release();
};

struct Octave {
  int rows, cols;
  float pixelDistance;
  float *blur[8];
  float *resp[8];
};
struct Pyramid {
  int nOct = 0;
  Octave oct[24];
  DevBuf store;
};

void set_error(const std::string &s);
bool gpu_shared();
struct CtxBusy { modsx_ctx *c; explicit CtxBusy(modsx_ctx *c); ~CtxBusy(); CtxBusy(const CtxBusy &) = delete; CtxBusy &operator=(const CtxBusy &) = delete; };
hipError_t ctx_copy(modsx_ctx *c, void *dst, const void *src, size_t bytes, hipMemcpyKind kind);
hipError_t ctx_sync(modsx_ctx *c);
unsigned ctx_mark(modsx_ctx *c);
bool ctx_mark_reached(modsx_ctx *c, unsigned seq);
hipError_t ctx_wait_mark(modsx_ctx *c, unsigned seq);
bool host_wait_runtime();
int host_cpus_per_rank();
#define MX_HIP(expr)                                                                          \
  do {                                                                                        \
    hipError_t e_ = (expr);                                                                   \
    if (e_ != hipSuccess) {                                                                   \
      mx::set_error(std::string(#expr) + ": " + hipGetErrorString(e_));                       \
      return MODSX_ERR_DEVICE;                                                                \
    }                                                                                         \
  } while (0)

std::vector<float> gaussian_kernel(int n, double sigma);
int blur_ksize(float sigma);
void gauss_mask(float *mask, int size);
void circular_gauss_mask(float *mask, int size, float sigma);
const double *atan_lut_host();
inline bool check_borders_host(int w, int h, float ofsx, float ofsy, float a11, float a12, float a21, float a22, int rw, int rh) {
  return check_borders(w, h, ofsx, ofsy, a11, a12, a21, a22, rw, rh);
}
bool invert3(const double *S, double *t);
void rectify(double &a11, double &a12, double &a21, double &a22);

void launch_blur_hess(hipStream_t s, const BlurBatch &b, int nj, int maxRows, int maxCols);
void launch_hessian(hipStream_t s, const BlurBatch &b, int nj, int maxRows, int maxCols);
void launch_resize_half(hipStream_t s, const ResizeBatch &b, int nj, int maxRows, int maxCols);
void launch_nms(hipStream_t s, const NmsBatch &b, const NmsJob *jobs, const int *tilePrefix, const int *tileJob, int nj,
                int nTiles, int4 *queue, unsigned *qcount, unsigned qcap, Candidate *out, unsigned *counter, unsigned cap,
                const int *octFirst = nullptr, int levelsPerOctave = 0);
size_t cand_sort_temp_bytes(unsigned nsort);
int launch_cand_order(hipStream_t s, const Candidate *cand, const unsigned *counter, unsigned nsort, unsigned long long *keys,
                      unsigned long long *keys2, unsigned *idx, unsigned *idx2, void *temp, size_t tempBytes, unsigned long long *tabKey,
                      unsigned *tabRank, unsigned tabSize, unsigned *slotOf, Candidate *out, unsigned *outCount);
constexpr int NMS_QUEUES = 64;
constexpr int NMS_TILE_ROWS = 16;
void launch_gray(hipStream_t s, const void *src, float *dst, size_t n, int channels, int dtype);
struct BaumGeo { int kernel, chunk, nchunks, grid; };
BaumGeo baumberg_geometry(int n, int W, int variant, int chunk);
void launch_baumberg(hipStream_t s, const AffJob *jobs, AffOut *out, int n, const float *mask, int W, int maxIter,
                     float convTh, float affInitialSigma, int variant = 0, int chunk = 0);
constexpr int ATAN_CASES = 2048 + 64;
constexpr int ORI_NV = 1344;
void launch_orientation(hipStream_t s, const OriJob *jobs, float *out, int n, const ImgRef *imgs,
                        const unsigned short *maskIdx, const float *maskW,
                        const unsigned char *binTab, int doHalf, double th, int maxAngles);
void launch_trunc_u8(hipStream_t s, const float *src, uint8_t *dst, size_t n);
size_t mser_sort_blocks(const int *rows, int n);
void launch_mser_sort(hipStream_t s, const uint8_t *const *u8, const int *rows, const int *cols, const size_t *ordOfs, int n, int *blockHist,
                      int *start, int *order);
void launch_expand_blur_tiles(hipStream_t s, const DescJob *jobs, const int *prefixRows, const int *prefixCols, int nJobs,
                              const int *needTab, BlurTile *tilesRows, BlurTile *tilesCols, float2 *rowStarts);
void launch_sample_rows(hipStream_t s, const DescJob *jobs, const BlurTile *tiles, int nTiles, const ImgRef *imgs, const float *taps,
                        const int *needTab, float *dst, const float2 *rowStarts, float *dstGrid);
void launch_blur_cols(hipStream_t s, const BlurTile *tiles, int nTiles, const float *taps, const int *needTab, const float *src,
                      float *dst);
void launch_expand_tiles(hipStream_t s, const int *prefix, int nJobs, int *tileJob);
void launch_patch_sample(hipStream_t s, const DescJob *jobs, const int *tilePrefix, const int *tileJob, int nTiles,
                         const ImgRef *imgs, float *scratch);
void launch_patch_blur(hipStream_t s, const DescJob *jobs, const int *tilePrefix, const int *tileJob, int nTiles,
                       const float *taps, const int *needTab, const float *src, float *dst, int pass);
void launch_describe(hipStream_t s, const DescJob *jobs, int n, const ImgRef *imgs, const float *grid,
                     const int *needTab, const float *coordTab,
                     const float *mask, const unsigned short *maskIdx, int nmask, const float *oTab, const int *bins,
                     const double *wts, int photoNorm, int descTypes, int nOut, double maxBin, const DescOut &outs);
void launch_warp_affine(hipStream_t s, const WarpJob &jb);
void launch_blur_pass(hipStream_t s, const float *src, float *dst, int rows, int cols, const float *taps, int n, int pass, int border = 0);
void launch_sub(hipStream_t s, const float *a, const float *b, float *o, size_t n);
void launch_grad_products(hipStream_t s, const float *img, int rows, int cols, float *xx, float *yy, float *xy);
void launch_harris_combine(hipStream_t s, const float *bxx, const float *byy, const float *bxy, float sigmasq, float *o, size_t n);
void launch_views_warp(hipStream_t s, const ViewJob *jobs, int n, int tiles, int stage);
void launch_views_blur(hipStream_t s, const ViewJob *jobs, int n, int tiles, const float *taps, int pass);
constexpr int VF_TW = 128, VF_TH = 16, VF_RX = 32, VF_RY = 2;
void launch_views_rotblur(hipStream_t s, const ViewJob *jobs, int n, int tiles, const float *taps, int maxRx, int maxRy);
void launch_views_fused(hipStream_t s, const ViewJob *jobs, int n, int tiles, const float *taps, int maxRx, int maxRy);
size_t match_workspace_bytes(int n1, int n2);
void launch_match(hipStream_t s, const uint8_t *d1, int n1, const uint8_t *d2, int n2, const double *pos2,
                  double sqminratio, double contrDistSq, int nn, MatchRow *rows, void *workspace);
#ifndef MODSX_SR_WIN
#define MODSX_SR_WIN 2400
#define MODSX_FC_ROWS 40
#define MODSX_SR_HALF 1
#define MODSX_SR_WGS 8
#endif
#ifndef MODSX_BLUR_LDS_C
#define MODSX_BLUR_LDS_C 9984
#endif
constexpr int MATCH_NN_MAX = 256;
constexpr int MATCH_MAXB = 4;
void launch_match_batch(hipStream_t s, int nb, const uint8_t *const *d1, const int *n1, const uint8_t *const *d2, const int *n2,
                        const double *const *pos2, double sqminratio, double contrDistSq, int nn, MatchRow *const *rows,
                        void *const *workspace, hipEvent_t *evSweep1 = nullptr,
                        const void *const *trainPack = nullptr);
size_t match_train_pack_bytes(int n2);
void launch_match_pack_trains(hipStream_t s, const uint8_t *d2, int n2, const double *pos2, void *pack);
void last_match_geometry(int *qs, int *fat, int *S, int *tilesPerSplit, int *ntilesUB);
struct DbGeo { int TEp, TOp; };
struct DbSet {
  DevBuf store;
  const unsigned char *tiles = nullptr;
  const int *hrow = nullptr;
  DbGeo geo = {0, 0};
  long rows = 0;
  int dev = 0;
};
DbGeo db_geo(long n, long nOdd);
size_t db_tiles_bytes(const DbGeo &g);
size_t db_hrow_bytes(const DbGeo &g);
int db_pack_blocks(long n);
void launch_db_pack(hipStream_t s, const uint8_t *raw, long n, const int2 *base, long nOdd, const DbGeo &geo, unsigned char *tiles,
                    int *hrow);
void launch_db_select(hipStream_t s, int nb, const MatchRow *const *rows, const int *n1, int nn, bool allPoints, int *const *sel, int *cnt,
                      int *const *dmin);
void launch_dbnn_min(hipStream_t s, int nb, const uint8_t *const *d1, const int *n1, int *const *sel, int *cnt, int *const *dmin,
                     const DbSet &db);

}

namespace mx {
#ifdef MODSX_DUP_BUILD
int dup_count(int cls);
#define MX_DUP(cls) for (int dupLeft_ = mx::dup_count(cls); dupLeft_ > 0; dupLeft_--)
#else
#define MX_DUP(cls)
#endif
enum KClass { K_BLUR_HESS = 0, K_HESSIAN, K_RESIZE, K_NMS, K_BAUMBERG, K_ORIENT, K_PATCH_SAMPLE, K_BLUR_ROWS, K_DESCRIBE,
              K_MATCH, K_GRAY, K_WARP, K_VIEW_BLUR, K_BLUR_COLS, K_MATCH_SWEEP1, K_MATCH_DB, K_NCLASS };
struct Profiler {
  bool enabled = false;
  std::vector<hipEvent_t> evA, evB;
  std::vector<int> cls;
  size_t used = 0;
  double ms[K_NCLASS] = {0};
  double work[K_NCLASS] = {0};
  long launches[K_NCLASS] = {0};
};
}

namespace mx {
enum DescCounter { DC_CALLS = 0, DC_CHUNKS, DC_MAX_CHUNKS, DC_CHUNKS_MID_IMAGE, DC_CHUNKS_LATER_IMAGE, DC_JOBS, DC_DIRECT_JOBS,
                   DC_FUSED_WINDOWS, DC_LDS_ROW_TILES, DC_LDS_COL_TILES, DC_SAMPLE_TILES, DC_GLOBAL_ROW_TILES, DC_GLOBAL_COL_TILES,
                   DC_CLAMPED_WINDOWS, DC_N };
}

struct modsx_db { mx::DbSet set; };

struct modsx_image {
  float *d;
  int rows, cols;
  bool owned;
};

struct modsx_ctx {
  int dev;
  hipStream_t stream;
  mx::Pyramid pyr[mx::MAXB];
  mx::DevBuf candSort, candOut;
  size_t lastSurvivors = 0;
  mx::DevBuf nmsJobs, cand, counter, affJobs, affOut, oriJobs, oriOut, descJobs, tilePrefix, taps, imgRefs, scratchA, scratchB,
      descF[mx::MAXB], descU8[mx::MAXB], descAllF[2], descAllU8[2], descAllU8b[2], descCls[2][4][2], descU8x[3][mx::MAXB], shardLocal, pos2, matchRows, matchWork, dbSel, misc, viewTmp[2], viewTaps, viewJobs, viewImg[mx::MAXB], scratchC, needTab, coordTab, tileJob, blurTiles, nmsQueue, rowStarts;
  mx::ImgRef imgRefsHost[mx::MAXB];
  mx::PinBuf hDescB;
  hipEvent_t descEv[2];
  bool descEvPending[2] = {false, false};
  bool descByEvent[2] = {true, true};
  unsigned descMark[2] = {0, 0};
  unsigned *hFlag = nullptr;
  unsigned flagSeq = 0;
  bool waitRuntime = true;
  mx::PinBuf hCand, hAff, hOri, hDesc, hMisc, hNms, hMatch, hViewTaps, hViewJobs, hMser, hRefs;
  float *dSmmMask = nullptr;
  int smmW = 0;
  std::vector<uint64_t> candKeys, candKeys2, candClaim;
  std::vector<uint32_t> candOrder, candOrder2;
  float *dOriMask = nullptr;
  unsigned short *dOriIdx = nullptr;
  float *dSiftMask = nullptr;
  unsigned short *dSiftMaskIdx = nullptr;
  int nSiftMask = 0;
  double *dAtan = nullptr;
  unsigned char *dOriBinTab = nullptr;
  float *dSiftOTab = nullptr;
  int *dSiftBins = nullptr;
  double *dSiftW = nullptr;
  double timings[6];
  mx::Profiler prof;
  size_t lastCandCount = 0;
  const mx::DbSet *fginnDb = nullptr;
  long descCnt[mx::DC_N] = {0};
  int busyDepth = 0;
  int shardLane = 0;
  modsx_ctx *peer = nullptr;
  modsx_ctx *half = nullptr;
  mx::DevBuf halfDesc[4];
  void *worker = nullptr;
};
```

### mods_amd/csrc/engine_api.hpp

```cpp
#pragma once
#include <stdio.h>
#include <chrono>
#include <functional>
#include <string>
#include <vector>
#include "engine.hpp"

struct modsx_comm;

namespace mx {
const char *last_error();
void prof_collect(modsx_ctx *c);
void prof_reset(modsx_ctx *c, bool enable);
modsx_ctx *ctx_create(int device_id);
void ctx_destroy(modsx_ctx *c);
int build_pyramids(modsx_ctx *c, const modsx_image *const *imgs, int n, const modsx_hessaff_params &p,
                   bool singleOctaveFromFirstLevel);
int detect_scalespace_batch(modsx_ctx *c, const modsx_image *const *imgs, int n, const modsx_hessaff_params &p,
                            std::vector<modsx_sskp> *out);
int detect_keypoints_batch(modsx_ctx *c, const modsx_image *const *imgs, int n, const modsx_hessaff_params &par,
                           const double *tilts, const double *zooms, std::vector<modsx_keypoint> *out);
int debug_baumberg(modsx_ctx *c, const modsx_image *const *planes, int nplanes, const int *planeOf, const float *xyspd, int n,
                   const modsx_hessaff_params &p, int variant, int chunk, float *u, int *ok, int *iters, int *geo);
void detect_affine_regions(const modsx_keypoint *kps, int n, int img_id, int det_type, modsx_region *out);
struct OriReproj { const double *H; int orig_w, orig_h; };
int detect_orientation_batch(modsx_ctx *c, const modsx_image *const *imgs, int n, const std::vector<modsx_region> *in,
                             double mrSize, int patchSize, int doHalfSIFT, int maxAngNum, double th, int addUpRight,
                             std::vector<modsx_region> *out, const OriReproj *reproj = nullptr);
int reproject_regions(modsx_region *regs, int n, const double *H, int orig_w, int orig_h);
int reproject_regions_box(modsx_region *regs, int n, const double *H, int orig_w, int orig_h, double boxk);
void reproject_certain_drop(const modsx_region *regs, int n, const double *H, int orig_w, int orig_h, double boxk, unsigned char *drop);
void orientation_counts(unsigned long long *launched, unsigned long long *skipped, bool reset);
struct DescSet {
  int n = 1;
  int type[MODSX_MAX_DESC] = {MODSX_DESC_ROOT_SIFT, 0, 0, 0};
  double ratio[MODSX_MAX_DESC] = {0, 0, 0, 0};
  bool forceHalf = false;
  bool half() const { for (int i = 0; i < n; i++) if (type[i] >= 2) return true; return forceHalf; }
  int packed() const { int p = 0; for (int i = 0; i < n; i++) p |= (type[i] & 15) << (4 * i); return p; }
};
int resolve_descs(const modsx_pair_params &pp, const modsx_ladder_step *st, DescSet &ds);
void desc_class_order(const DescSet &ds, int *ord);
int describe_batch(modsx_ctx *c, const modsx_image *const *imgs, int n, const std::vector<modsx_region> *regs,
                   double mrSize, int patchSize, int fast, int photoNorm, int descType, double maxBin,
                   float *const *descHost, float *const *devF, uint8_t *const *devU8, const DescSet *ds = nullptr,
                   uint8_t *const *const *devU8x = nullptr);
int set_vs_pars(const double *scale_set, int ns, const double *tilt_set, int nt, double phi_base, double InitSigma,
                int doBlur, modsx_view *par, int cap, modsx_view *prev, int *nprev, int cap_prev);
int synth_view(modsx_ctx *c, const modsx_image *gray, const modsx_view &v, modsx_image **out, double *H, int *identity,
               int slot = -1);
int detect_describe_items(modsx_ctx *c, const modsx_image *const *itemImg, const int *itemView, int nitems, const modsx_view *views,
                          const modsx_pair_params &pp, std::vector<modsx_region> &regs,
                          float *devF, uint8_t *devU8, size_t devCapRegions, float *hostDesc, int *itemCounts,
                          const DescSet *ds = nullptr, uint8_t *const *devU8x = nullptr);
int detect_describe_views(modsx_ctx *c, const modsx_image *gray, const modsx_view *views, int nv,
                          const modsx_pair_params &pp, int view_begin, int view_step, std::vector<modsx_region> &regs,
                          float *devF, uint8_t *devU8, size_t devCapRegions, float *hostDesc, int *viewCounts,
                          const DescSet *ds = nullptr, uint8_t *const *devU8x = nullptr);
struct ClassSide { std::vector<modsx_region> *regs; size_t *cap; DevBuf *buf; };
int class_side_reserve(modsx_ctx *c, const ClassSide &k, size_t keepRows);
int accumulate_views(modsx_ctx *c, const ClassSide *ks, const DescSet &ds, const modsx_image *img, const modsx_view *views, int nv,
                     const modsx_pair_params &pp, modsx_comm *cm = nullptr, bool split = false);
void ctx_worker_stop(modsx_ctx *c);
void rebase_ids(std::vector<modsx_region> &regs, const int *viewCounts, int nv, size_t base);
struct VerifyTask;
int match_ladder(modsx_ctx *c, const modsx_image *img1, const modsx_image *img2, const modsx_ladder_step *steps, int nsteps,
                 int min_matches, const modsx_pair_params &pp, modsx_pair_result *res, int *steps_done, VerifyTask *defer = nullptr,
                 modsx_comm *comm = nullptr, int owner = -1);
int match_pair_views(modsx_ctx *c, const modsx_image *img1, const modsx_image *img2, const modsx_view *views, int nv,
                     const modsx_pair_params &pp, modsx_pair_result *res, VerifyTask *defer = nullptr);
void prof_begin(modsx_ctx *c, int cls, double work, size_t *slot);
void prof_end(modsx_ctx *c, size_t slot);
bool prof_reserve(modsx_ctx *c, int cls, double work, hipEvent_t *ev2);
struct ProfScope {
  modsx_ctx *c;
  size_t slot;
  ProfScope(modsx_ctx *c_, int cls, double work) : c(c_) { prof_begin(c, cls, work, &slot); }
  ~ProfScope() { prof_end(c, slot); }
  ProfScope(const ProfScope &) = delete;
  ProfScope &operator=(const ProfScope &) = delete;
};
struct HostMark {
  bool on; double t;
  HostMark() : on(getenv("MODSX_HOST_TIMING") && atoi(getenv("MODSX_HOST_TIMING")) >= 2), t(0) { if (on) t = now(); }
  static double now() { return std::chrono::duration<double, std::milli>(std::chrono::steady_clock::now().time_since_epoch()).count(); }
  void mark(const char *what) { if (!on) return; const double n = now(); fprintf(stderr, "  host %-28s %.3f ms\n", what, n - t); t = n; }
};
inline double now_ms() { return HostMark::now(); }
inline size_t align_up(size_t bytes, size_t a) { return (bytes + a - 1) & ~(a - 1); }
inline void host_radix_sort_u64(std::vector<uint64_t> &w, std::vector<uint64_t> &tmp, int loBit, int hiBit) {
  constexpr int BITS = 11, NB = 1 << BITS;
  const size_t m = w.size();
  if (!m) return;
  tmp.resize(m);
  uint32_t hist[NB];
  for (int shift = loBit; shift <= hiBit; shift += BITS) {
    memset(hist, 0, sizeof hist);
    for (size_t k = 0; k < m; k++) hist[(w[k] >> shift) & (NB - 1)]++;
    if (hist[(w[0] >> shift) & (NB - 1)] == m) continue;
    uint32_t sum = 0;
    for (int b = 0; b < NB; b++) { const uint32_t h = hist[b]; hist[b] = sum; sum += h; }
    for (size_t k = 0; k < m; k++) tmp[hist[(w[k] >> shift) & (NB - 1)]++] = w[k];
    w.swap(tmp);
  }
}
struct MatchShard { void *comm; int world, per, n1_total, lo; };
int match_shard_begin(modsx_ctx *c, const MatchShard &sh, mx::MatchRow **blk);
int match_shard_gather(modsx_ctx *c, const MatchShard &sh, int local_rc, mx::MatchRow *host);
int detect_describe_views_sharded(modsx_ctx *c, modsx_comm *cm, const modsx_image *img, const modsx_view *views, int nv,
                                  const modsx_pair_params &pp, const DescSet &ds, std::vector<modsx_region> &regs,
                                  DevBuf *const *descAcc, const size_t *base, int *viewCounts);
int detect_describe_items_sharded(modsx_ctx *c, modsx_comm *cm, const modsx_image *const *imgs, int nimg, const modsx_view *views,
                                  int nviews, const modsx_pair_params &pp, const DescSet &ds, std::vector<modsx_region> &regs,
                                  DevBuf *const *descAcc, const size_t *base, int *itemCounts, const unsigned char *wantImg = nullptr,
                                  std::vector<size_t> *regStart = nullptr, double **devPos = nullptr, std::vector<double> *kpRows = nullptr,
                                  const int *ownerImg = nullptr);
void rows_to_tentatives(const MatchRow *rows, int n1, int nn, std::vector<modsx_tentative> &o, const int *ddb = nullptr,
                        double sqminratio = 0, std::vector<double> *d2byDB = nullptr);
int comm_rank(const modsx_comm *cm);
int comm_world(const modsx_comm *cm);
int comm_same_value(modsx_ctx *c, modsx_comm *cm, int value, const char *what);
int match_sharded(modsx_ctx *c, modsx_comm *cm, const uint8_t *d1, int n1, const uint8_t *d2, int n2, const double *pos2Host,
                  double ratioT, double contradDist, int nn, std::vector<modsx_tentative> &out);
int match_device_batch(modsx_ctx *c, int nb, const uint8_t *const *d1, const int *n1, const uint8_t *const *d2, const int *n2,
                       const double *const *pos2Host, double ratioT, double contradDist, int nn,
                       std::vector<modsx_tentative> *out, const MatchShard *shard, const double *const *pos2Dev = nullptr,
                       const DbSet *db = nullptr, std::vector<double> *d2byDB = nullptr,
                       const void *const *trainPack = nullptr);
int match_device(modsx_ctx *c, const uint8_t *d1, int n1, const uint8_t *d2, int n2, const double *pos2Host,
                 double ratioT, double contradDist, int nn, std::vector<modsx_tentative> &out, const DbSet *db = nullptr,
                 std::vector<double> *d2byDB = nullptr);
int match_host_desc(modsx_ctx *c, const float *desc1, int n1, const float *desc2, int n2, const double *pos2,
                    double ratioT, double contradDist, int nn, std::vector<modsx_tentative> &out, const DbSet *db = nullptr,
                    std::vector<double> *d2byDB = nullptr);
DbSet *db_create(modsx_ctx *c, const void *rows, long n, int dtype);
void db_free(DbSet *db);
int db_nearest(modsx_ctx *c, const DbSet &db, const float *desc, int n, float *dmin);
inline const DbSet *fginn_db_for(const modsx_ctx *c, int descType) { return descType == MODSX_DESC_ROOT_SIFT ? c->fginnDb : nullptr; }
struct RegList {
  const modsx_region *p[2 * MODSX_MAX_DESC];
  size_t end[2 * MODSX_MAX_DESC];
  int n = 0;
  void clear() { n = 0; }
  void add(const modsx_region *q, size_t cnt) { p[n] = q; end[n] = (n ? end[n - 1] : 0) + cnt; n++; }
  void add(const std::vector<modsx_region> &v) { add(v.data(), v.size()); }
  size_t size() const { return n ? end[n - 1] : 0; }
  const modsx_region &operator[](size_t i) const {
    int k = 0;
    while (k < n - 1 && i >= end[k]) k++;
    if (i >= end[k]) abort();
    return p[k][i - (k ? end[k - 1] : 0)];
  }
};
void verify_tentatives(const RegList &r1, const RegList &r2, const std::vector<modsx_tentative> &tents,
                       const modsx_pair_params &pp, modsx_pair_result *res);
void verify_tentatives(const std::vector<modsx_region> &r1, const std::vector<modsx_region> &r2,
                       const std::vector<modsx_tentative> &tents, const modsx_pair_params &pp, modsx_pair_result *res);
void verify_tentatives_kp(const double *kp1, size_t n1, const double *kp2, size_t n2, const std::vector<modsx_tentative> &tents,
                          const modsx_pair_params &pp, modsx_pair_result *res);
struct VerifyTask {
  std::vector<std::vector<modsx_region>> own;
  RegList l1, l2;
  std::vector<modsx_tentative> tents;
  modsx_pair_result *res = nullptr;
  int dev = 0;
  VerifyTask() = default;
  VerifyTask(VerifyTask &&) = default;
  VerifyTask &operator=(VerifyTask &&) = default;
  VerifyTask(const VerifyTask &) = delete;
  VerifyTask &operator=(const VerifyTask &) = delete;
};
struct RepSlot {
  std::vector<modsx_region> regs;
  size_t cap = (size_t)1 << 16;
  DevBuf desc, pack;
};
// ... 45 lines not shown
```

### mods_amd/csrc/engine_detect.hip

```cpp
#include <math.h>
#include <algorithm>
#include <mutex>
#include <dlfcn.h>
#include <string>
#include "engine_api.hpp"

namespace mx {

static int cv_round(double v) { return (int)lrint(v); }

struct SigmaPlan {
  int levels;
  float sigmaStep;
  float curSigma[8];
  float incSigma[8];
};

static SigmaPlan make_sigma_plan(const modsx_hessaff_params &p) {
  SigmaPlan s;
  s.levels = p.numberOfScales + 2;
  s.sigmaStep = powf(2.0f, 1.0f / (float)p.numberOfScales);
  float cur = p.initialSigma;
  s.curSigma[0] = cur; s.incSigma[0] = 0;
  for (int i = 1; i < s.levels; i++) {
// ... 56 lines not shown
  }
  return lv;
}

static int launch_first_level(modsx_ctx *c, const modsx_image *const *imgs, const LiveOctave &lv, const modsx_hessaff_params &p,
                              const SigmaPlan &sp, bool hess, bool firstLevelGiven) {
  hipStream_t s = c->stream;
  BlurBatch bb;
  memset(&bb, 0, sizeof bb);
  const float curSigma0 = 0.5f;
  const bool preBlur = !firstLevelGiven && p.initialSigma > curSigma0;
  if (preBlur) {
    float sigma = sqrtf(p.initialSigma * p.initialSigma - curSigma0 * curSigma0);
    int rc = fill_taps(bb, sigma);
    if (rc) return rc;
  }
  for (int k = 0; k < lv.n; k++) {
    const int i = lv.img[k];
    Octave &oc = c->pyr[i].oct[0];
    BlurJob &j = bb.j[k];
    j.src = imgs[i]->d; j.blur = oc.blur[0]; j.resp = hess ? oc.resp[0] : nullptr; j.rows = oc.rows; j.cols = oc.cols;
    j.norm = sp.curSigma[0] * sp.curSigma[0];
    if (!preBlur) {
      MX_HIP(hipMemcpyAsync(oc.blur[0], imgs[i]->d, (size_t)oc.rows * oc.cols * 4, hipMemcpyDeviceToDevice, s));
      j.src = oc.blur[0];
    }
  }
  if (preBlur) { ProfScope ps(c, K_BLUR_HESS, lv.px * 12); launch_blur_hess(s, bb, lv.n, lv.mr, lv.mc); }
  else if (hess) { ProfScope ps(c, K_HESSIAN, lv.px * 8); launch_hessian(s, bb, lv.n, lv.mr, lv.mc); }
  return MODSX_OK;
}

static void launch_resize_level(modsx_ctx *c, const LiveOctave &lv, int o, const modsx_hessaff_params &p, const SigmaPlan &sp, bool hess) {
  ResizeBatch rb;
  memset(&rb, 0, sizeof rb);
  double spx = 0;
  for (int k = 0; k < lv.n; k++) {
    Octave &pv = c->pyr[lv.img[k]].oct[o - 1], &oc = c->pyr[lv.img[k]].oct[o];
    ResizeJob &r = rb.j[k];
    r.src = pv.blur[p.numberOfScales]; r.dst = oc.blur[0];
    r.srows = pv.rows; r.scols = pv.cols; r.drows = oc.rows; r.dcols = oc.cols;
    r.resp = hess ? oc.resp[0] : nullptr; r.norm = sp.curSigma[0] * sp.curSigma[0];
    spx += (double)pv.rows * pv.cols;
  }
  ProfScope ps(c, K_RESIZE, (spx + lv.px) * 4 + lv.px * 4);
  launch_resize_half(c->stream, rb, lv.n, lv.mr, lv.mc);
}

static int launch_other_responses(modsx_ctx *c, const LiveOctave &lv, int o, const modsx_hessaff_params &p, const SigmaPlan &sp) {
  hipStream_t s = c->stream;
  const int L = sp.levels;
  constexpr int RESP_TAPS = 4096;
  constexpr size_t SLICE = 2 * (RESP_TAPS + 4);
  for (int l = 0; l < L; l++) {
    const float norm = sp.curSigma[l] * sp.curSigma[l];
    const float sigma = p.detectorType == MODSX_DET_DOG ? norm : sqrtf((float)(0.6 * norm));
    const int nt = blur_ksize(sigma);
    if (nt > RESP_TAPS) { set_error("response blur kernel too large"); return MODSX_ERR_ARG; }
    if (!c->viewTaps.ensure((size_t)L * SLICE * 4) || !c->hViewTaps.ensure((size_t)L * SLICE * 4)) return MODSX_ERR_NOMEM;
    float *dT = (float *)c->viewTaps.p + (size_t)l * SLICE, *hT = (float *)c->hViewTaps.p + (size_t)l * SLICE;
    bool tapsUp = false;
    for (int k = 0; k < lv.n; k++) {
      Octave &oc = c->pyr[lv.img[k]].oct[o];
      const int rows = oc.rows, cols = oc.cols;
      const size_t npx = (size_t)rows * cols;
      if (!c->scratchA.ensure(npx * 4 * 8)) return MODSX_ERR_NOMEM;
      float *buf = (float *)c->scratchA.p, *tmp = buf, *a = buf + npx, *b = buf + 2 * npx, *cc = buf + 3 * npx;
      float *ba = buf + 4 * npx, *bb2 = buf + 5 * npx, *bc = buf + 6 * npx;
      const int nx = cols == 1 ? 1 : nt, ny = rows == 1 ? 1 : nt;
      if (!tapsUp || nx != nt || ny != nt) {
        std::vector<float> kx = gaussian_kernel(nx, sigma), ky = gaussian_kernel(ny, sigma);
        if (tapsUp) MX_HIP(ctx_sync(c));
        memcpy(hT, kx.data(), nx * 4); memcpy(hT + nx, ky.data(), ny * 4);
        MX_HIP(ctx_copy(c, dT, hT, (size_t)(nx + ny) * 4, hipMemcpyHostToDevice));
        tapsUp = nx == nt && ny == nt;
      }
      auto blur = [&](const float *src, float *dst) {
        if (nt == 1) { MX_HIP(hipMemcpyAsync(dst, src, npx * 4, hipMemcpyDeviceToDevice, s)); return MODSX_OK; }
        launch_blur_pass(s, src, tmp, rows, cols, dT, nx, 0, 1);
        launch_blur_pass(s, tmp, dst, rows, cols, dT + nx, ny, 1, 1);
        return MODSX_OK;
      };
      if (p.detectorType == MODSX_DET_DOG) {
        int rc = blur(oc.blur[l], a);
        if (rc) return rc;
        launch_sub(s, oc.blur[l], a, oc.resp[l], npx);
      } else {
        launch_grad_products(s, oc.blur[l], rows, cols, a, b, cc);
        int rc = blur(a, ba);
        if (!rc) rc = blur(b, bb2);
        if (!rc) rc = blur(cc, bc);
        if (rc) return rc;
        launch_harris_combine(s, ba, bb2, bc, (float)(0.6 * norm), oc.resp[l], npx);
      }
    }
  }
  return MODSX_OK;
}

int build_pyramids(modsx_ctx *c, const modsx_image *const *imgs, int n, const modsx_hessaff_params &p,
                   bool singleOctaveFromFirstLevel) {
  if (n <= 0 || n > MAXB) { set_error("batch size"); return MODSX_ERR_ARG; }
  if (p.numberOfScales < 1 || p.numberOfScales > 6) { set_error("numberOfScales"); return MODSX_ERR_ARG; }
  if (p.detectorType != MODSX_DET_HESSIAN && p.detectorType != MODSX_DET_DOG && p.detectorType != MODSX_DET_HARRIS) {
    set_error("detectorType must be Hessian (0), DoG (1) or Harris (2)");
    return MODSX_ERR_ARG;
  }
  const bool hess = p.detectorType == MODSX_DET_HESSIAN;
  const SigmaPlan sp = make_sigma_plan(p);
  int maxOct = 0;
  int rc = plan_octaves(c, imgs, n, sp.levels, 2 * p.border + 2, singleOctaveFromFirstLevel, &maxOct);
  if (rc) return rc;
  for (int o = 0; o < maxOct; o++) {
    const LiveOctave lv = live_octave(c, n, o);
    if (o == 0) rc = launch_first_level(c, imgs, lv, p, sp, hess, singleOctaveFromFirstLevel);
    else launch_resize_level(c, lv, o, p, sp, hess);
    if (rc) return rc;
    for (int l = 1; l < sp.levels; l++) {
      BlurBatch b2;
      memset(&b2, 0, sizeof b2);
      rc = fill_taps(b2, sp.incSigma[l]);
      if (rc) return rc;
      for (int k = 0; k < lv.n; k++) {
        Octave &oc = c->pyr[lv.img[k]].oct[o];
        BlurJob &j = b2.j[k];
        j.src = oc.blur[l - 1]; j.blur = oc.blur[l]; j.resp = hess ? oc.resp[l] : nullptr; j.rows = oc.rows; j.cols = oc.cols;
        j.norm = sp.curSigma[l] * sp.curSigma[l];
      }
      ProfScope ps(c, K_BLUR_HESS, lv.px * 12);
      launch_blur_hess(c->stream, b2, lv.n, lv.mr, lv.mc);
    }
    if (!hess) rc = launch_other_responses(c, lv, o, p, sp);
    if (rc) return rc;
  }
  MX_HIP(hipGetLastError());
  return MODSX_OK;
}

static const unsigned CAND_CAP = 1u << 21;

static NmsBatch nms_thresholds(const modsx_hessaff_params &p) {
  NmsBatch nb;
  memset(&nb, 0, sizeof nb);
  nb.edgeScoreThreshold = (p.edgeEigenValueRatio + 1.0f) * (p.edgeEigenValueRatio + 1.0f) / p.edgeEigenValueRatio;
  float finalTh = p.threshold;
  float posTh = (float)(0.8 * finalTh);
  float negTh = -posTh;
  if (p.detectorType == MODSX_DET_HESSIAN) finalTh = p.threshold * p.threshold;
  if (p.mode != MODSX_FIXED_TH) finalTh = posTh = negTh = 0.0f;
  nb.posTh = posTh; nb.negTh = negTh; nb.finalTh = finalTh; nb.border = p.border; nb.detType = p.detectorType;
  return nb;
}

static int scan_extrema(modsx_ctx *c, int n, const modsx_hessaff_params &p) {
  hipStream_t s = c->stream;
  if (!c->cand.ensure((size_t)CAND_CAP * sizeof(Candidate)) || !c->nmsQueue.ensure((size_t)CAND_CAP * 16)) return MODSX_ERR_NOMEM;
  if (!c->counter.ensure((NMS_QUEUES + 1) * 128)) return MODSX_ERR_NOMEM;
  MX_HIP(hipMemsetAsync(c->counter.p, 0, 128 + NMS_QUEUES * 128, s));
  bool queuesClean = true;
  const NmsBatch nb = nms_thresholds(p);
  int maxOct = 0;
  for (int i = 0; i < n; i++) maxOct = std::max(maxOct, c->pyr[i].nOct);
  const bool perOctave = p.numberOfScales == 3 && !getenv("MODSX_NMS_PER_LEVEL");
  std::vector<NmsJob> hjobs;
  std::vector<int> hpfx(1, 0), hfirst;
  double px = 0;
  auto flush = [&](bool last) -> int {
    const int nj = (int)hjobs.size();
    if (!nj) return MODSX_OK;
    const int np = (int)hpfx.size() - 1;
    const size_t jobBytes = (size_t)nj * sizeof(NmsJob), pfxBytes = (size_t)(np + 1) * 4, firstBytes = (size_t)std::max<size_t>(1, hfirst.size()) * 4;
    if (!c->nmsJobs.ensure(jobBytes + pfxBytes + firstBytes + 64)) return MODSX_ERR_NOMEM;
    if (!c->hNms.ensure(jobBytes + pfxBytes + firstBytes)) return MODSX_ERR_NOMEM;
    memcpy(c->hNms.p, hjobs.data(), jobBytes);
    memcpy((char *)c->hNms.p + jobBytes, hpfx.data(), pfxBytes);
    if (!hfirst.empty()) memcpy((char *)c->hNms.p + jobBytes + pfxBytes, hfirst.data(), hfirst.size() * 4);
    MX_HIP(ctx_copy(c, c->nmsJobs.p, c->hNms.p, jobBytes + pfxBytes + firstBytes, hipMemcpyHostToDevice));
    if (!c->tileJob.ensure((size_t)hpfx.back() * 4 + 4)) return MODSX_ERR_NOMEM;
    const int *dPfx = (const int *)((char *)c->nmsJobs.p + jobBytes);
    launch_expand_tiles(s, dPfx, np, (int *)c->tileJob.p);
    {
      ProfScope ps(c, K_NMS, px * 12);
      if (!queuesClean) MX_HIP(hipMemsetAsync((unsigned *)c->counter.p + 32, 0, NMS_QUEUES * 128, s));
      queuesClean = false;
      launch_nms(s, nb, (const NmsJob *)c->nmsJobs.p, dPfx, (const int *)c->tileJob.p, nj,
                 hpfx.back(), (int4 *)c->nmsQueue.p, (unsigned *)c->counter.p + 32, CAND_CAP, (Candidate *)c->cand.p,
                 (unsigned *)c->counter.p, CAND_CAP, perOctave ? (const int *)((char *)c->nmsJobs.p + jobBytes + pfxBytes) : nullptr,
                 p.numberOfScales);
    }
    if (!last) MX_HIP(ctx_sync(c));
    hjobs.clear(); hpfx.assign(1, 0); hfirst.clear(); px = 0;
    return MODSX_OK;
  };
  for (int o = 0; o < maxOct; o++)
    for (int i = 0; i < n; i++) {
      if (c->pyr[i].nOct <= o) continue;
      Octave &oc = c->pyr[i].oct[o];
      const int w = oc.cols - 2 * p.border, h = oc.rows - 2 * p.border;
      if (w <= 0 || h <= 0) continue;
      if ((int)hjobs.size() + p.numberOfScales > NMS_MAXJ) { int rcf = flush(false); if (rcf) return rcf; }
      const int tiles = ((w + 63) / 64) * ((h + NMS_TILE_ROWS - 1) / NMS_TILE_ROWS);
      if (perOctave) { hfirst.push_back((int)hjobs.size()); hpfx.push_back(hpfx.back() + tiles); }
      for (int l = 1; l <= p.numberOfScales; l++) {
        NmsJob j;
        j.low = oc.resp[l - 1]; j.cur = oc.resp[l]; j.high = oc.resp[l + 1]; j.blur = oc.blur[l];
        j.rows = oc.rows; j.cols = oc.cols; j.img = i; j.octave = o; j.level = l; j.pad = 0;
        hjobs.push_back(j);
        if (!perOctave) hpfx.push_back(hpfx.back() + tiles);
        px += (double)oc.rows * oc.cols;
      }
    }
  return flush(true);
}

static int download_counted(modsx_ctx *c, const void *devRecords, int recWord, size_t cap, size_t lastCount, unsigned *nrec) {
  if (!c->hMisc.ensure(64)) return MODSX_ERR_NOMEM;
  const size_t spec = std::min<size_t>(cap, lastCount + lastCount / 4 + 1024);
  if (!c->hCand.ensure(std::max<size_t>(spec, 1) * sizeof(Candidate))) return MODSX_ERR_NOMEM;
  MX_HIP(ctx_copy(c, c->hMisc.p, c->counter.p, std::max(2, recWord + 1) * 4, hipMemcpyDeviceToHost));
  MX_HIP(ctx_copy(c, c->hCand.p, devRecords, spec * sizeof(Candidate), hipMemcpyDeviceToHost));
  MX_HIP(ctx_sync(c));
  const unsigned *w = (const unsigned *)c->hMisc.p;
  if (w[0] > CAND_CAP || w[1]) { set_error("candidate buffer overflow"); return MODSX_ERR_NOMEM; }
  c->lastCandCount = w[0];
  *nrec = w[recWord];
  if (w[0] > cap || *nrec <= spec) return MODSX_OK;
  if (!c->hCand.ensure((size_t)*nrec * sizeof(Candidate))) return MODSX_ERR_NOMEM;
  MX_HIP(ctx_copy(c, c->hCand.p, devRecords, (size_t)*nrec * sizeof(Candidate), hipMemcpyDeviceToHost));
  MX_HIP(ctx_sync(c));
  return MODSX_OK;
}

static modsx_sskp sskp_from_candidate(const Candidate &q, const Pyramid &py, const SigmaPlan &sp, int numberOfScales) {
  const float pixelDistance = py.oct[q.octave].pixelDistance;
  const float curScale = sp.curSigma[q.level];
  float scale = curScale * powf(2.0f, q.b2 / numberOfScales);
  modsx_sskp kp;
  kp.octave = q.octave; kp.level = q.level; kp.r0 = q.r0; kp.c0 = q.c0; kp.r = q.r; kp.c = q.c; kp.type = q.type;
  kp.pad = 0;
  kp.b0 = q.b0; kp.b1 = q.b1; kp.b2 = q.b2; kp.val = q.val;
  kp.x = pixelDistance * (q.c + q.b0);
  kp.y = pixelDistance * (q.r + q.b1);
  kp.s = pixelDistance * scale;
  kp.pixelDistance = pixelDistance;
  return kp;
}

static std::vector<uint32_t> image_starts(const Candidate *cd, unsigned nrec, int n) {
  std::vector<uint32_t> imgStart(n + 1, 0);
  for (unsigned k = 0; k < nrec; k++) imgStart[cd[k].img + 1]++;
  for (int i = 0; i < n; i++) imgStart[i + 1] += imgStart[i];
  return imgStart;
}

static int order_on_host(modsx_ctx *c, int n, const modsx_hessaff_params &p, std::vector<modsx_sskp> *out) {
  unsigned cnt = 0;
  int rc = download_counted(c, c->cand.p, 0, CAND_CAP, c->lastCandCount, &cnt);
  if (rc) return rc;
  HostMark hm;
  const Candidate *cd = (const Candidate *)c->hCand.p;
  for (unsigned k = 0; k < cnt; k++) {
    const Candidate &q = cd[k];
    if ((unsigned)q.img >= (unsigned)n || (unsigned)q.octave >= 32u || (unsigned)q.level >= 32u || (unsigned)q.r0 >= (1u << 14) ||
        (unsigned)q.c0 >= (1u << 14) || (unsigned)q.r >= (1u << 24) || (unsigned)q.c >= (1u << 24)) {
      set_error("candidate outside the sort key's range");
      return MODSX_ERR_DEVICE;
    }
  }
  std::vector<uint32_t> &byImg = c->candOrder;
  const std::vector<uint32_t> imgStart = image_starts(cd, cnt, n);
  byImg.resize(cnt);
  {
    std::vector<uint32_t> fill(imgStart.begin(), imgStart.end() - 1);
    for (unsigned k = 0; k < cnt; k++) byImg[fill[cd[k].img]++] = k;
  }
  hm.mark("cand bucket by image");
  const SigmaPlan sp = make_sigma_plan(p);
  host_parallel_light(n, [&](int img) {
    std::vector<modsx_sskp> &dst = out[img];
    dst.clear();
    const uint32_t *idx = byImg.data() + imgStart[img];
    const size_t m = imgStart[img + 1] - imgStart[img];
    if (!m) return;
    static thread_local std::vector<uint64_t> order, order2;
    static_assert(CAND_CAP <= (1u << 21), "index field of the packed sort key");
    order.resize(m);
    for (size_t k = 0; k < m; k++) {
      const Candidate &q = cd[idx[k]];
      order[k] = ((uint64_t)q.octave << 54) | ((uint64_t)q.level << 49) | ((uint64_t)(q.r0 & 0x3fff) << 35) | ((uint64_t)(q.c0 & 0x3fff) << 21) | idx[k];
    }
    host_radix_sort_u64(order, order2, 21, 58);
    size_t tabSize = 64;
    while (tabSize < m * 2 + 16) tabSize <<= 1;
    std::vector<uint64_t> claimed(tabSize, 0);
    dst.reserve(m);
    for (size_t kk = 0; kk < m; kk++) {
      const Candidate &q = cd[order[kk] & 0x1fffffu];
      const uint64_t key = (((uint64_t)q.octave << 48) | ((uint64_t)q.r << 24) | (uint64_t)q.c) + 1;
      size_t h = (size_t)((key * 0x9E3779B97F4A7C15ull) >> 20) & (tabSize - 1);
      bool taken = false;
      while (claimed[h]) { if (claimed[h] == key) { taken = true; break; } h = (h + 1) & (tabSize - 1); }
      if (taken) continue;
      claimed[h] = key;
      dst.push_back(sskp_from_candidate(q, c->pyr[q.img], sp, p.numberOfScales));
    }
  });
  hm.mark("octaveMap claim + sskp");
  return MODSX_OK;
}

struct CandLibrary {
  size_t (*sort_temp_bytes)(unsigned) = nullptr;
  int (*order)(hipStream_t, const Candidate *, const unsigned *, unsigned, unsigned long long *, unsigned long long *, unsigned *, unsigned *,
               void *, size_t, unsigned long long *, unsigned *, unsigned, unsigned *, Candidate *, unsigned *) = nullptr;
};
static const CandLibrary &load_cand_library() {
  static CandLibrary lib;
  static std::once_flag candOnce;
  std::call_once(candOnce, [] {
    Dl_info di;
    std::string path = "libmodsx_cand.so";
    if (dladdr((const void *)&modsx_create, &di) && di.dli_fname) {
      const std::string self(di.dli_fname);
      const size_t sl = self.rfind('/');
      if (sl != std::string::npos) path = self.substr(0, sl + 1) + "libmodsx_cand.so";
    }
    if (void *h = dlopen(path.c_str(), RTLD_NOW | RTLD_LOCAL)) {
      lib.sort_temp_bytes = (decltype(lib.sort_temp_bytes))dlsym(h, "modsx_cand_sort_temp_bytes");
      lib.order = (decltype(lib.order))dlsym(h, "modsx_cand_order");
    }
  });
  return lib;
}

static int order_on_device(modsx_ctx *c, int n, const modsx_hessaff_params &p, std::vector<modsx_sskp> *out) {
  const CandLibrary &lib = load_cand_library();
  if (!lib.sort_temp_bytes || !lib.order) {
    set_error("MODSX_DEVICE_ORDER=1, but libmodsx_cand.so (make -C mods_amd/csrc cand) is not beside libmodsx.so");
    return MODSX_ERR_DEVICE;
  }
  unsigned nsurv = 0;
  for (int attempt = 0;; attempt++) {
    const unsigned nsort = (unsigned)std::min<size_t>(CAND_CAP, attempt ? c->lastCandCount + 64 : c->lastCandCount + c->lastCandCount / 4 + 1024);
    unsigned tabSize = 1024;
    while (tabSize < 2 * nsort + 16) tabSize <<= 1;
    const size_t tempB = lib.sort_temp_bytes(nsort);
    const size_t keyB = align_up((size_t)nsort * 8, 256), idxB = align_up((size_t)nsort * 4, 256);
    const size_t oKeys = 0, oKeys2 = oKeys + keyB, oIdx = oKeys2 + keyB, oIdx2 = oIdx + idxB, oSlot = oIdx2 + idxB, oTabK = oSlot + idxB,
                 oTabR = oTabK + align_up((size_t)tabSize * 8, 256), oTemp = oTabR + align_up((size_t)tabSize * 4, 256),
                 total = oTemp + align_up(tempB, 256) + 256;
    if (!c->candSort.ensure(total) || !c->candOut.ensure((size_t)nsort * sizeof(Candidate) + 64)) return MODSX_ERR_NOMEM;
    char *w = (char *)c->candSort.p;
    unsigned *survivors = (unsigned *)c->counter.p + 2;
    if (lib.order(c->stream, (const Candidate *)c->cand.p, (const unsigned *)c->counter.p, nsort, (unsigned long long *)(w + oKeys),
                  (unsigned long long *)(w + oKeys2), (unsigned *)(w + oIdx), (unsigned *)(w + oIdx2), w + oTemp, tempB,
                  (unsigned long long *)(w + oTabK), (unsigned *)(w + oTabR), tabSize, (unsigned *)(w + oSlot),
                  (Candidate *)c->candOut.p, survivors)) { set_error("device-side detection order failed"); return MODSX_ERR_DEVICE; }
    int rc = download_counted(c, c->candOut.p, 2, nsort, c->lastSurvivors, &nsurv);
    if (rc) return rc;
    if (c->lastCandCount <= nsort) break;
    if (attempt) { set_error("device-side detection order: capacity does not converge"); return MODSX_ERR_INTERNAL; }
  }
  c->lastSurvivors = nsurv;
  HostMark hm;
  const Candidate *cd = (const Candidate *)c->hCand.p;
  const SigmaPlan sp = make_sigma_plan(p);
  for (unsigned k = 0; k < nsurv; k++)
    if ((unsigned)cd[k].img >= (unsigned)n || (unsigned)cd[k].octave >= 32u) { set_error("candidate outside the image / octave range"); return MODSX_ERR_DEVICE; }
  const std::vector<uint32_t> imgStart = image_starts(cd, nsurv, n);
  host_parallel_light(n, [&](int img) {
    std::vector<modsx_sskp> &dst = out[img];
    dst.clear();
    dst.reserve(imgStart[img + 1] - imgStart[img]);
    for (uint32_t k = imgStart[img]; k < imgStart[img + 1]; k++) dst.push_back(sskp_from_candidate(cd[k], c->pyr[cd[k].img], sp, p.numberOfScales));
  });
  hm.mark("sskp from ordered survivors");
  return MODSX_OK;
}

int detect_scalespace_batch(modsx_ctx *c, const modsx_image *const *imgs, int n, const modsx_hessaff_params &p,
                            std::vector<modsx_sskp> *out) {
  int rc = build_pyramids(c, imgs, n, p, false);
  if (!rc) rc = scan_extrema(c, n, p);
  if (rc) return rc;
  static const bool deviceOrder = getenv("MODSX_DEVICE_ORDER") != nullptr && atoi(getenv("MODSX_DEVICE_ORDER")) != 0;
  return deviceOrder ? order_on_device(c, n, p, out) : order_on_host(c, n, p, out);
}

static int ensure_smm_mask(modsx_ctx *c, int W) {
  if (c->smmW == W && c->dSmmMask) return MODSX_OK;
  if (W < 3 || W > 19 || !(W & 1)) { set_error("smmWindowSize must be odd and <= 19"); return MODSX_ERR_ARG; }
  if (c->dSmmMask) hipFree(c->dSmmMask);
  std::vector<float> m(W * W);
  gauss_mask(m.data(), W);
  MX_HIP(hipMalloc(&c->dSmmMask, W * W * 4));
  MX_HIP(hipMemcpy(c->dSmmMask, m.data(), W * W * 4, hipMemcpyHostToDevice));
  c->smmW = W;
  return MODSX_OK;
}

int debug_baumberg(modsx_ctx *c, const modsx_image *const *planes, int nplanes, const int *planeOf, const float *xyspd, int n,
                   const modsx_hessaff_params &p, int variant, int chunk, float *u, int *ok, int *iters, int *geo) {
  const BaumGeo g = baumberg_geometry(n, p.smmWindowSize, variant, chunk);
  if (g.kernel < 0) { set_error("modsx_debug_baumberg: no kernel for this window size / variant / chunk"); return MODSX_ERR_ARG; }
  geo[0] = g.kernel; geo[1] = g.chunk; geo[2] = g.nchunks; geo[3] = g.grid;
  for (int i = 0; i < nplanes; i++)
    if (!planes[i] || !planes[i]->d || planes[i]->rows < 4 || planes[i]->cols < 4) { set_error("modsx_debug_baumberg: planes must be at least 4 x 4"); return MODSX_ERR_ARG; }
  for (int k = 0; k < n; k++) {
    const float *q = xyspd + 4 * (size_t)k;
    if ((unsigned)planeOf[k] >= (unsigned)nplanes || !std::isfinite(q[0]) || !std::isfinite(q[1]) || !std::isfinite(q[2]) ||
        !(q[3] > 0.f) || !std::isfinite(q[3])) {
      set_error("modsx_debug_baumberg: job outside the contract (plane index, finite x / y / s, pixelDistance > 0)");
      return MODSX_ERR_ARG;
    }
  }
  if (!n) return MODSX_OK;
  int rc = ensure_smm_mask(c, p.smmWindowSize);
  if (rc) return rc;
  const size_t total = (size_t)n;
  if (!c->hAff.ensure(total * sizeof(AffJob) + total * sizeof(AffOut))) return MODSX_ERR_NOMEM;
  if (!c->affJobs.ensure(total * sizeof(AffJob)) || !c->affOut.ensure(total * sizeof(AffOut))) return MODSX_ERR_NOMEM;
  AffJob *hj = (AffJob *)c->hAff.p;
  AffOut *ho = (AffOut *)((char *)c->hAff.p + total * sizeof(AffJob));
  for (int k = 0; k < n; k++) {
    const modsx_image *im = planes[planeOf[k]];
    const float *q = xyspd + 4 * (size_t)k;
    AffJob &j = hj[k];
    j.blur = im->d; j.rows = im->rows; j.cols = im->cols;
    j.x = q[0]; j.y = q[1]; j.s = q[2]; j.pixelDistance = q[3];
  }
  hipStream_t s = c->stream;
  MX_HIP(hipMemcpyAsync(c->affJobs.p, hj, total * sizeof(AffJob), hipMemcpyHostToDevice, s));
  MX_HIP(hipMemsetAsync(c->affOut.p, 0xFF, total * sizeof(AffOut), s));
  launch_baumberg(s, (AffJob *)c->affJobs.p, (AffOut *)c->affOut.p, n, c->dSmmMask, p.smmWindowSize, p.maxIterations,
                  p.convergenceThreshold, p.affInitialSigma, variant, chunk);
  MX_HIP(hipGetLastError());
  MX_HIP(hipMemcpyAsync(ho, c->affOut.p, total * sizeof(AffOut), hipMemcpyDeviceToHost, s));
  MX_HIP(hipStreamSynchronize(s));
  for (int k = 0; k < n; k++) {
    u[4 * k] = ho[k].u11; u[4 * k + 1] = ho[k].u12; u[4 * k + 2] = ho[k].u21; u[4 * k + 3] = ho[k].u22;
    ok[k] = ho[k].ok; iters[k] = ho[k].iters;
  }
  return MODSX_OK;
}

static void prepare_keys_for_export(std::vector<modsx_keypoint> &keys, const modsx_hessaff_params &p) {
  if (keys.empty() || p.mode == MODSX_FIXED_TH) return;
  auto cmpv = [](modsx_keypoint k1, modsx_keypoint k2) { return fabs(k1.response) > fabs(k2.response); };
  std::sort(keys.begin(), keys.end(), cmpv);
  double maxResponse = fabs(keys[0].response);
  int regNumber = (int)keys.size();
  auto cmp = [](const modsx_keypoint &k1, const modsx_keypoint &k2) { return fabs(k1.response) > fabs(k2.response); };
  switch (p.mode) {
    case MODSX_RELATIVE_TH: {
      modsx_keypoint t = keys[0];
      t.response = (float)(maxResponse * p.rel_threshold);
      keys.resize(std::lower_bound(keys.begin(), keys.end(), t, cmp) - keys.begin());
      break;
    }
    case MODSX_FIXED_REG_NUMBER: {
      int nn = p.reg_number;
      if (p.doBaumberg) nn = (int)floor(3.0 * (double)nn);
      if ((nn < regNumber) && (nn >= 0)) keys.resize(nn);
      break;
    }
    case MODSX_RELATIVE_REG_NUMBER: {
      keys.resize((int)floor(p.rel_reg_number * (double)keys.size()));
      break;
    }
    case MODSX_NOT_LESS_THAN_REGIONS: {
      modsx_keypoint t = keys[0];
      t.response = p.threshold;
      int fix = (int)(std::lower_bound(keys.begin(), keys.end(), t, cmp) - keys.begin());
      if (fix < p.reg_number) keys.resize(std::min(p.reg_number, regNumber));
      else keys.resize(std::min(fix, regNumber));
      break;
    }
    default: break;
  }
  if (p.mode == MODSX_FIXED_REG_NUMBER && (int)keys.size() > p.reg_number) keys.resize(p.reg_number);
}

int detect_keypoints_batch(modsx_ctx *c, const modsx_image *const *imgs, int n, const modsx_hessaff_params &par,
                           const double *tilts, const double *zooms, std::vector<modsx_keypoint> *out) {
  modsx_hessaff_params p = par;
  std::vector<modsx_sskp> ss[MAXB];
  int rc = detect_scalespace_batch(c, imgs, n, p, ss);
  if (rc) return rc;
  HostMark hm;
  rc = ensure_smm_mask(c, p.smmWindowSize);
  if (rc) return rc;
  size_t total = 0;
  for (int i = 0; i < n; i++) total += ss[i].size();
  for (int i = 0; i < n; i++) out[i].clear();
  if (!total) return MODSX_OK;
  hipStream_t s = c->stream;
  if (!c->hAff.ensure(total * sizeof(AffJob) + total * sizeof(AffOut))) return MODSX_ERR_NOMEM;
  if (!c->affJobs.ensure(total * sizeof(AffJob)) || !c->affOut.ensure(total * sizeof(AffOut))) return MODSX_ERR_NOMEM;
  AffJob *hj = (AffJob *)c->hAff.p;
  AffOut *ho = (AffOut *)((char *)c->hAff.p + total * sizeof(AffJob));
  size_t first[MAXB + 1];
  first[0] = 0;
  for (int i = 0; i < n; i++) first[i + 1] = first[i] + ss[i].size();
  host_parallel_light(n, [&](int i) {
    size_t k = first[i];
    for (const modsx_sskp &q : ss[i]) {
      const Octave &oc = c->pyr[i].oct[q.octave];
      AffJob &j = hj[k++];
      j.blur = oc.blur[q.level - 1];
      j.rows = oc.rows; j.cols = oc.cols;
      j.x = q.x; j.y = q.y; j.s = q.s; j.pixelDistance = q.pixelDistance;
    }
  });
  hm.mark("AffJob build");
  if (p.doBaumberg) {
    MX_HIP(ctx_copy(c, c->affJobs.p, hj, total * sizeof(AffJob), hipMemcpyHostToDevice));
    ProfScope ps(c, K_BAUMBERG, (double)total * 361 * 4 * 2);
    launch_baumberg(s, (AffJob *)c->affJobs.p, (AffOut *)c->affOut.p, (int)total, c->dSmmMask, p.smmWindowSize,
                    p.maxIterations, p.convergenceThreshold, p.affInitialSigma);
    MX_HIP(ctx_copy(c, ho, c->affOut.p, total * sizeof(AffOut), hipMemcpyDeviceToHost));
    MX_HIP(ctx_sync(c));
  } else {
    for (size_t i = 0; i < total; i++) { ho[i].u11 = 1; ho[i].u12 = 0; ho[i].u21 = 0; ho[i].u22 = 1; ho[i].ok = 1; ho[i].iters = 0; }
  }
  hm.mark("baumberg launch + wait");
  host_parallel_light(n, [&](int i) {
    size_t k = first[i];
    out[i].reserve(ss[i].size());
    for (const modsx_sskp &q : ss[i]) {
      const AffOut &a = ho[k++];
      if (!a.ok) continue;
      modsx_keypoint kp;
      memset(&kp, 0, sizeof kp);
      kp.x = q.x; kp.y = q.y; kp.s = q.s;
      kp.a11 = a.u11; kp.a12 = a.u12; kp.a21 = a.u21; kp.a22 = a.u22;
      kp.response = q.val;
      kp.sub_type = q.type;
      out[i].push_back(kp);
    }
    modsx_hessaff_params pe = p;
    const double tilt = tilts ? tilts[i] : 1.0, zoom = zooms ? zooms[i] : 1.0;
    if ((tilt > 2.0) || (zoom < 0.5)) pe.reg_number = (int)floor(zoom * (double)pe.reg_number / tilt);
    prepare_keys_for_export(out[i], pe);
  });
  hm.mark("keypoints + export");
  return MODSX_OK;
}

void detect_affine_regions(const modsx_keypoint *kps, int n, int img_id, int det_type, modsx_region *out) {
  for (int i = 0; i < n; i++) {
    modsx_keypoint k = kps[i];
    modsx_region &r = out[i];
    memset(&r, 0, sizeof r);
    r.img_id = img_id; r.img_reproj_id = 0; r.type = det_type; r.id = i;
    r.det_kp.s = k.s * sqrt(fabs(k.a11 * k.a22 - k.a12 * k.a21));
    rectify(k.a11, k.a12, k.a21, k.a22);
    r.det_kp.x = k.x; r.det_kp.y = k.y;
    r.det_kp.a11 = k.a11; r.det_kp.a12 = k.a12; r.det_kp.a21 = k.a21; r.det_kp.a22 = k.a22;
    r.det_kp.response = k.response;
    r.det_kp.sub_type = k.sub_type;
  }
}

}
```

### mods_amd/csrc/kernels_affine.hip

```cpp
#include "engine.hpp"

namespace mx {

constexpr int AW_MAX = 19;

MX_D void inv_sqrt_wave(int lane, float &a, float &b, float &c, float &l1, float &l2) {
  double t, r;
  if (b != 0) {
    r = double(c - a) / (2 * b);
    if (r >= 0) t = 1.0 / (r + sqrt(1 + r * r));
    else t = -1.0 / (-r + sqrt(1 + r * r));
    r = 1.0 / sqrt(1 + t * t);
    t = t * r;
  } else { r = 1; t = 0; }
  const bool odd = lane & 1;
  const double rr = r * r, tt = t * t, m = 2 * r * t * b;
  const double first = (odd ? tt : rr) * a, last = (odd ? rr : tt) * c;
  double w = 1.0 / sqrt((odd ? first + m : first - m) + last);
  double x = __shfl(w, 0), z = __shfl(w, 1);
  const double d = sqrt(x * z);
  w = (odd ? z : x) / d;
  x = __shfl(w, 0); z = __shfl(w, 1);
  if (x < z) { l1 = float(z); l2 = float(x); } else { l1 = float(x); l2 = float(z); }
  a = float(r * r * x + t * t * z);
  b = float(-r * t * x + t * r * z);
  c = float(t * t * x + r * r * z);
}

template <int WT>
__global__ __launch_bounds__(64) void k_baumberg(const AffJob *jobs, AffOut *out, int n, const float *mask, int Warg,
                                                 int maxIter, float convTh, float affInitialSigma) {
  const int W = WT ? WT : Warg;
  const int k = blockIdx.x;
  if (k >= n) return;
  const int lane = threadIdx.x;
  __shared__ __attribute__((aligned(16))) float pa[AW_MAX * AW_MAX + 3], pb[AW_MAX * AW_MAX + 3], pc[AW_MAX * AW_MAX + 3];
  float *const simg = pc;
  const AffJob jb = jobs[k];
  const int WW = W * W, half = W >> 1;
  constexpr int PERM = (AW_MAX * AW_MAX + 63) / 64;
  float vmask[PERM];
  int pp[PERM], oxp[PERM], oxm[PERM], oyp[PERM], oym[PERM];
#pragma unroll
  for (int u = 0; u < PERM; u++) {
    const int i = lane + 64 * u;
    vmask[u] = i < WW ? mask[i] : 0.f;
    const int p = i < WW ? i : WW - 1;
    const int r = p / W, c = p - r * W;
    pp[u] = p;
    oxp[u] = c == W - 1 ? p : p + 1;
    oxm[u] = c == 0 ? p : p - 1;
    oyp[u] = r == W - 1 ? p : p + W;
    oym[u] = r == 0 ? p : p - W;
  }
  float u11 = 1.0f, u12 = 0.0f, u21 = 0.0f, u22 = 1.0f, l1 = 1.0f, l2 = 1.0f;
  float era = 0.0f, erb = 0.0f;
  const float lx = jb.x / jb.pixelDistance, ly = jb.y / jb.pixelDistance;
  const float ratio = jb.s / (affInitialSigma * jb.pixelDistance);
  const gcfloat_p img = as_global(jb.blur);
  int ok = 0, l = 0;
  __syncthreads();
  for (l = 0; l < maxIter; l++) {
    const float a11 = u11 * ratio, a12 = u12 * ratio, a21 = u21 * ratio, a22 = u22 * ratio;
    const bool touch = check_borders(jb.cols, jb.rows, lx, ly, a11, a12, a21, a22, W, W);
    {
      float rx = lx - (float)half * a12, ry = ly - (float)half * a22;
      if (WT) {
#pragma unroll
        for (int j = 1; j < (WT ? WT : 1); j++)
          if (lane >= j) { rx += a12; ry += a22; }
      } else {
        for (int j = 0; j < lane && j < W; j++) { rx += a12; ry += a22; }
      }
      if (lane < W) {
        float WX = rx - (float)half * a11;
        float WY = ry - (float)half * a21;
        if (WT) {
#pragma unroll
          for (int i = 0; i < (WT ? WT : 1); i++) {
            pa[lane * W + i] = WX;
            pb[lane * W + i] = WY;
            WX += a11;
            WY += a21;
          }
        } else {
#pragma unroll 1
          for (int i = 0; i < W; i++) {
            pa[lane * W + i] = WX;
            pb[lane * W + i] = WY;
            WX += a11;
            WY += a21;
          }
        }
      }
    }
    __syncthreads();
    {
      float sv[PERM];
      if (!touch) {
#pragma unroll
        for (int u = 0; u < PERM; u++) sv[u] = bilinear_tap(img, jb.rows, jb.cols, pa[pp[u]], pb[pp[u]], false);
      } else {
#pragma unroll
        for (int u = 0; u < PERM; u++) sv[u] = bilinear_tap_touch_select(img, jb.rows, jb.cols, pa[pp[u]], pb[pp[u]]);
      }
#pragma unroll
      for (int u = 0; u < PERM; u++)
        if (lane + 64 * u < WW) simg[lane + 64 * u] = sv[u];
    }
    __syncthreads();
    {
      float qa[PERM], qb[PERM], qc[PERM];
#pragma unroll
      for (int u = 0; u < PERM; u++) {
        const float gx = simg[oxp[u]] - simg[oxm[u]];
        const float gy = simg[oyp[u]] - simg[oym[u]];
        const float v = vmask[u];
        const float gxy = gx * gy;
        qa[u] = gx * gx * v;
        qb[u] = gxy * v;
        qc[u] = gy * gy * v;
      }
      __syncthreads();
#pragma unroll
      for (int u = 0; u < PERM; u++) {
        const int p = lane + 64 * u;
        if (p < WW) { pa[p] = qa[u]; pb[p] = qb[u]; pc[p] = qc[u]; }
      }
    }
    __syncthreads();
    float acc = 0.f;
    if (lane < 3) {
      const float *arr = lane == 0 ? pa : (lane == 1 ? pb : pc);
      const float4 *a4 = reinterpret_cast<const float4 *>(arr);
      const int full = WW >> 2;
#pragma unroll 6
      for (int i = 0; i < full; i++) { const float4 v = a4[i]; acc += v.x; acc += v.y; acc += v.z; acc += v.w; }
      for (int i = full * 4; i < WW; i++) acc += arr[i];
      acc /= (float)WW;
    }
    float a = __shfl(acc, 0), b = __shfl(acc, 1), c = __shfl(acc, 2);
    inv_sqrt_wave(lane, a, b, c, l1, l2);
    if ((a != a) || (b != b) || (c != c)) break;
    erb = era;
    era = (float)(1.0 - (double)(l2 / l1));
    const float u11t = u11, u12t = u12;
    u11 = a * u11t + b * u21;
    u12 = a * u12t + b * u22;
    u21 = b * u11t + c * u21;
    u22 = b * u12t + c * u22;
    if (!eigenvalues(u11, u12, u21, u22, l1, l2)) break;
    if ((l1 / l2 > 6) || (l2 / l1 > 6)) break;
    if (era < convTh && erb < convTh) { ok = 1; break; }
    __syncthreads();
  }
  if (lane == 0) {
    AffOut o;
    o.u11 = u11; o.u12 = u12; o.u21 = u21; o.u22 = u22; o.ok = ok; o.iters = l;
    out[k] = o;
  }
}

MX_D void wave_lds_sync() { asm volatile("s_waitcnt lgkmcnt(0)" ::: "memory"); }
#ifdef BAUM_TRACE
__device__ unsigned long long g_btrace[16];
#define BT(i) do { asm volatile("s_waitcnt vmcnt(0) lgkmcnt(0)" ::: "memory"); const unsigned long long t_ = __builtin_readcyclecounter(); bt_[i] += t_ - btl_; btl_ = t_; } while (0)
#else
#define BT(i) do { } while (0)
#endif

#ifndef MODSX_BAUMBERG_K
#define MODSX_BAUMBERG_K 2
#endif
template <int K>
__global__ __launch_bounds__(64) void k_baumberg_stream(const AffJob *jobs, AffOut *out, int n, const float *mask, int chunk,
                                                        int nchunks, int maxIter, float convTh, float affInitialSigma) {
  constexpr int W = AW_MAX, WW = W * W, half = W >> 1, CH = AW_MAX * AW_MAX + 3;
  constexpr int PERM = (WW + 63) / 64;
  __shared__ __attribute__((aligned(16))) float buf[K][3][CH];
  const int lane = threadIdx.x;
  float vmask[PERM];
  int pp[PERM], oxp[PERM], oxm[PERM], oyp[PERM], oym[PERM];
#pragma unroll
  for (int u = 0; u < PERM; u++) {
    const int i = lane + 64 * u;
    vmask[u] = i < WW ? mask[i] : 0.f;
    const int p = i < WW ? i : WW - 1;
    const int r = p / W, c = p - r * W;
    pp[u] = p;
    oxp[u] = c == W - 1 ? p : p + 1;
    oxm[u] = c == 0 ? p : p - 1;
    oyp[u] = r == W - 1 ? p : p + W;
    oym[u] = r == 0 ? p : p - W;
  }
  const int kq = lane >> 1;
  const bool slotLane = lane < 2 * K;
  float u11 = 1.0f, u12 = 0.0f, u21 = 0.0f, u22 = 1.0f, l1 = 1.0f, l2 = 1.0f, era = 0.0f, erb = 0.0f, ratio = 0.f;
  float slx = 0.f, sly = 0.f;
  int scols = 4, srows = 4;
  int ok = 0, it = 0, kidx = -1;
  int next = min(xcd_chunk(blockIdx.x, nchunks) * chunk, n);
  const int end = min(next + chunk, n);
  bool live = false;
  if (maxIter <= 0) {
    for (int i = next + lane; i < end; i += 64) { AffOut o; o.u11 = 1; o.u12 = 0; o.u21 = 0; o.u22 = 1; o.ok = 0; o.iters = 0; out[i] = o; }
    return;
  }
#ifdef BAUM_TRACE
  unsigned long long bt_[9] = {0, 0, 0, 0, 0, 0, 0, 0, 0}, btl_ = __builtin_readcyclecounter();
#endif
  for (;;) {
    {
      const bool want = slotLane && !live;
      const unsigned long long wm = __ballot(want && !(lane & 1));
      const int rank = __popcll(wm & ((1ull << (lane & ~1)) - 1ull));
      const int cand = next + rank;
      if (want && cand < end) {
        kidx = cand;
        const AffJob sj = jobs[cand];
        ratio = sj.s / (affInitialSigma * sj.pixelDistance);
        slx = sj.x / sj.pixelDistance; sly = sj.y / sj.pixelDistance;
        scols = sj.cols; srows = sj.rows;
        u11 = 1.0f; u12 = 0.0f; u21 = 0.0f; u22 = 1.0f; l1 = 1.0f; l2 = 1.0f; era = 0.0f; erb = 0.0f;
        ok = 0; it = 0;
        live = true;
      }
      next = min(next + __popcll(wm), end);
    }
    const unsigned long long liveMask = __ballot(live);
    if (!liveMask) break;
    BT(0);
    const float A11 = u11 * ratio, A12 = u12 * ratio, A21 = u21 * ratio, A22 = u22 * ratio;
    const unsigned long long touchMask = __ballot(check_borders(scols, srows, slx, sly, A11, A12, A21, A22, W, W));
    if constexpr (K % 2 == 0) {
#pragma unroll
      for (int sp = 0; sp < K; sp += 2) {
      const int dq = sp + (lane >> 5), dc = (lane >> 4) & 1, di = lane & 15;
      const float s11 = __shfl(A11, 2 * dq), s12 = __shfl(A12, 2 * dq), s21 = __shfl(A21, 2 * dq), s22 = __shfl(A22, 2 * dq);
      const float sox = __shfl(slx, 2 * dq), soy = __shfl(sly, 2 * dq);
      const float so = dc ? soy : sox;
      const float stepR = dc ? s22 : s12, stepC = dc ? s21 : s11;
      float v = so - (float)half * stepR;
#define MX_ROWSTEP "s_nop 1\n\tv_add_f32_dpp %0, %0, %1 row_shr:1 row_mask:0xf bank_mask:0xf\n\t"
      asm volatile("s_nop 4\n\t" MX_ROWSTEP MX_ROWSTEP MX_ROWSTEP MX_ROWSTEP MX_ROWSTEP MX_ROWSTEP MX_ROWSTEP MX_ROWSTEP MX_ROWSTEP MX_ROWSTEP
                   MX_ROWSTEP MX_ROWSTEP MX_ROWSTEP MX_ROWSTEP MX_ROWSTEP "s_nop 1"
                   : "+v"(v)
                   : "v"(stepR));
#undef MX_ROWSTEP
      const float e16 = __shfl(v, lane | 15) + stepR, e17 = e16 + stepR, e18 = e17 + stepR;
      const float vx = di == 0 ? e16 : (di == 1 ? e17 : e18);
      const float hc = (float)half * stepC;
      typedef float v2f __attribute__((ext_vector_type(2)));
      v2f wv = {v - hc, vx - hc};
      const v2f st = {stepC, stepC};
      float *const b1 = &buf[dq][dc][di * W];
      float *const b2 = di < 3 ? &buf[dq][dc][(16 + di) * W] : &buf[dq][2][0];
#pragma unroll
      for (int i = 0; i < W; i++) {
        b1[i] = wv.x;
        b2[i] = wv.y;
        wv += st;
      }
      }
    }
    BT(1);
#pragma unroll
    for (int q = 0; q < K; q++) {
      if (!((liveMask >> (2 * q)) & 1)) continue;
#ifdef MODSX_BAUM_VECTOR_JOB
      const AffJob jb = jobs[__shfl(kidx, 2 * q)];
#else
      const AffJob jb = jobs[__builtin_amdgcn_readlane(kidx, 2 * q)];
#endif
      const gcfloat_p img = as_global(jb.blur);
      float *const pa = buf[q][0], *const pb = buf[q][1], *const pc = buf[q][2];
      float *const simg = pc;
      const bool touch = (touchMask >> (2 * q)) & 1;
#ifdef BAUM_TRACE
      const float a11 = __shfl(A11, 2 * q), a12 = __shfl(A12, 2 * q), a21 = __shfl(A21, 2 * q), a22 = __shfl(A22, 2 * q);
#endif
#ifdef BAUM_TRACE
      if (lane == 0) {
        const float bw = 18.f * (fabsf(a11) + fabsf(a12)) + 3.f, bh = 18.f * (fabsf(a21) + fabsf(a22)) + 3.f;
        const float m = fmaxf(bw, bh);
        const int b = m <= 16.f ? 0 : m <= 24.f ? 1 : m <= 32.f ? 2 : m <= 40.f ? 3 : m <= 48.f ? 4 : m <= 64.f ? 5 : 6;
        atomicAdd(&g_btrace[9 + b], 1ull);
      }
#endif
      if constexpr (K % 2 != 0) {
        const float lx = __shfl(slx, 2 * q), ly = __shfl(sly, 2 * q);
        const float a11 = __shfl(A11, 2 * q), a12 = __shfl(A12, 2 * q), a21 = __shfl(A21, 2 * q), a22 = __shfl(A22, 2 * q);
        float rx = lx - (float)half * a12, ry = ly - (float)half * a22;
#pragma unroll
        for (int j = 1; j < W; j++)
          if (lane >= j) { rx += a12; ry += a22; }
        if (lane < W) {
          float WX = rx - (float)half * a11;
          float WY = ry - (float)half * a21;
#pragma unroll
          for (int i = 0; i < W; i++) {
            pa[lane * W + i] = WX;
            pb[lane * W + i] = WY;
            WX += a11;
            WY += a21;
          }
        }
      }
      wave_lds_sync();
      {
        float sv[PERM];
        if (!touch) {
#pragma unroll
          for (int u = 0; u < PERM; u++) sv[u] = bilinear_tap(img, jb.rows, jb.cols, pa[pp[u]], pb[pp[u]], false);
        } else {
#pragma unroll
          for (int u = 0; u < PERM; u++) sv[u] = bilinear_tap_touch_select(img, jb.rows, jb.cols, pa[pp[u]], pb[pp[u]]);
        }
        wave_lds_sync();
#pragma unroll
        for (int u = 0; u < PERM; u++)
          if (lane + 64 * u < WW) simg[lane + 64 * u] = sv[u];
      }
      wave_lds_sync();
      BT(2 + 2 * (q & 1));
      {
        float qa[PERM], qb[PERM], qc[PERM];
#pragma unroll
        for (int u = 0; u < PERM; u++) {
          const float gx = simg[oxp[u]] - simg[oxm[u]];
          const float gy = simg[oyp[u]] - simg[oym[u]];
          const float v = vmask[u];
          const float gxy = gx * gy;
          qa[u] = gx * gx * v;
          qb[u] = gxy * v;
          qc[u] = gy * gy * v;
        }
        wave_lds_sync();
#pragma unroll
        for (int u = 0; u < PERM; u++) {
          const int p = lane + 64 * u;
          if (p < WW) { pa[p] = qa[u]; pb[p] = qb[u]; pc[p] = qc[u]; }
        }
      }
      BT(3 + 2 * (q & 1));
    }
    wave_lds_sync();
    float acc = 0.f;
    if (lane < 3 * K) {
      const int q3 = lane / 3, ch = lane - 3 * q3;
      const float *arr = buf[q3][ch];
      const float4 *a4 = reinterpret_cast<const float4 *>(arr);
#pragma unroll 6
      for (int i = 0; i < WW / 4; i++) { const float4 v = a4[i]; acc += v.x; acc += v.y; acc += v.z; acc += v.w; }
      acc += arr[WW - 1];
      acc /= (float)WW;
    }
    float a = __shfl(acc, 3 * kq), b = __shfl(acc, 3 * kq + 1), c = __shfl(acc, 3 * kq + 2);
    BT(6);
    if (live) {
      {
        double t, r;
        if (b != 0) {
          r = double(c - a) / (2 * b);
          if (r >= 0) t = 1.0 / (r + sqrt(1 + r * r));
          else t = -1.0 / (-r + sqrt(1 + r * r));
          r = 1.0 / sqrt(1 + t * t);
          t = t * r;
        } else { r = 1; t = 0; }
        const bool odd = lane & 1;
        const double rr = r * r, tt = t * t, m = 2 * r * t * b;
        const double first = (odd ? tt : rr) * a, last = (odd ? rr : tt) * c;
        double w = 1.0 / sqrt((odd ? first + m : first - m) + last);
        double x = __shfl(w, lane & ~1), z = __shfl(w, lane | 1);
        const double d = sqrt(x * z);
        w = (odd ? z : x) / d;
        x = __shfl(w, lane & ~1); z = __shfl(w, lane | 1);
        if (x < z) { l1 = float(z); l2 = float(x); } else { l1 = float(x); l2 = float(z); }
        a = float(r * r * x + t * t * z);
        b = float(-r * t * x + t * r * z);
        c = float(t * t * x + r * r * z);
      }
      bool stop = false;
      int iters = it;
      if ((a != a) || (b != b) || (c != c)) stop = true;
      else {
        erb = era;
        era = (float)(1.0 - (double)(l2 / l1));
        const float u11t = u11, u12t = u12;
        u11 = a * u11t + b * u21;
        u12 = a * u12t + b * u22;
        u21 = b * u11t + c * u21;
        u22 = b * u12t + c * u22;
        if (!eigenvalues(u11, u12, u21, u22, l1, l2)) stop = true;
        else if ((l1 / l2 > 6) || (l2 / l1 > 6)) stop = true;
        else if (era < convTh && erb < convTh) { ok = 1; stop = true; }
      }
      it++;
      if (!stop && it >= maxIter) { stop = true; iters = maxIter; }
      if (stop) {
        live = false;
        if (!(lane & 1)) {
          AffOut o;
          o.u11 = u11; o.u12 = u12; o.u21 = u21; o.u22 = u22; o.ok = ok; o.iters = iters;
          out[kidx] = o;
        }
      }
    }
    BT(7);
  }
#ifdef BAUM_TRACE
  if (lane == 0) {
    for (int i = 0; i < 8; i++) atomicAdd(&g_btrace[i], bt_[i]);
    atomicAdd(&g_btrace[8], 1ull);
  }
#endif
}

#ifndef MODSX_BAUMBERG_CHUNK
#define MODSX_BAUMBERG_CHUNK 8
#endif

BaumGeo baumberg_geometry(int n, int W, int variant, int chunk) {
  constexpr int K = MODSX_BAUMBERG_K;
  BaumGeo g = {-1, 0, 0, 0};
  if (n < 0 || chunk < 0 || W < 3 || W > AW_MAX || !(W & 1)) return g;
  if (variant == 0) g.kernel = W == AW_MAX ? (K > 1 ? 0 : 1) : 2;
  else if (variant == 1 && W == AW_MAX) g.kernel = 1;
  else if (variant == 2) g.kernel = 2;
  else return g;
  if (g.kernel != 0) { g.chunk = 1; g.nchunks = n; g.grid = n; return g; }
  if (!chunk) {
    chunk = n / 16384;
    chunk = chunk < K ? K : (chunk > MODSX_BAUMBERG_CHUNK ? MODSX_BAUMBERG_CHUNK : chunk);
  }
  g.chunk = chunk;
  g.nchunks = (int)(((long long)n + chunk - 1) / chunk);
  g.grid = 8 * ((g.nchunks + 7) / 8);
  return g;
}

void launch_baumberg(hipStream_t s, const AffJob *jobs, AffOut *out, int n, const float *mask, int W, int maxIter,
                     float convTh, float affInitialSigma, int variant, int chunk) {
  if (n <= 0) return;
  constexpr int K = MODSX_BAUMBERG_K;
  const BaumGeo g = baumberg_geometry(n, W, variant, chunk);
  if (g.kernel == 0) {
    MX_DUP(K_BAUMBERG) hipLaunchKernelGGL(k_baumberg_stream<K>, dim3(g.grid), dim3(64), 0, s, jobs, out, n, mask, g.chunk, g.nchunks, maxIter,
                       convTh, affInitialSigma);
  } else if (g.kernel == 1) hipLaunchKernelGGL(k_baumberg<19>, dim3(n), dim3(64), 0, s, jobs, out, n, mask, W, maxIter, convTh, affInitialSigma);
  else if (g.kernel == 2) hipLaunchKernelGGL(k_baumberg<0>, dim3(n), dim3(64), 0, s, jobs, out, n, mask, W, maxIter, convTh, affInitialSigma);
}

}

#ifdef BAUM_TRACE
extern "C" __attribute__((visibility("default"))) int modsx_debug_baum_trace(unsigned long long *out, int reset) {
  int rc = (int)hipMemcpyFromSymbol(out, HIP_SYMBOL(mx::g_btrace), 16 * 8, 0, hipMemcpyDeviceToHost);
  if (reset) { unsigned long long z[16] = {0}; rc |= (int)hipMemcpyToSymbol(HIP_SYMBOL(mx::g_btrace), z, sizeof z, 0, hipMemcpyHostToDevice); }
  return rc;
}
#endif
```

Baseline: 221.9.

## Replace static Baumberg chunking with persistent atomic work queue and range stealing

The Baumberg affine-adaptation kernel now runs a persistent grid sized from the occupancy query. Instead of a fixed chunk per block, waves pull keypoints from eight atomic range counters and steal from other ranges once their own is empty. The aim is to even out the load when per-keypoint iteration counts vary, so no long tail of waves keeps running after the others finish. The cost is atomics on every refill, an extra memset of the queue counters, and an error path if the occupancy query fails. The queue form is on by default and can be turned off with the MODSX_BAUMBERG_QUEUE environment variable.

```diff
diff --git a/include/modsx.h b/include/modsx.h
--- a/include/modsx.h
+++ b/include/modsx.h
@@ -216,9 +216,11 @@
 int modsx_debug_describe_plan(const modsx_region *regs, const int *counts, int nimages, double mr_size, int fast_extraction,
                               unsigned long long arena_floats, long *counters, int n, long *cuts, int cap_cuts, int *n_cuts);
 int modsx_debug_baumberg_geometry(int n, int W, int variant, int chunk, int *geometry);
+int modsx_debug_baumberg_geometry_ctx(modsx_ctx *ctx, int n, int W, int variant, int chunk, int *geometry);
+int modsx_debug_baumberg_variant(int W);
 int modsx_debug_baumberg(modsx_ctx *ctx, const modsx_image *const *planes, int nplanes, const int *plane_of, const float *xyspd,
                          int n, const modsx_hessaff_params *par, int variant, int chunk, float *u, int *ok, int *iters,
-                         int *geometry);
+                         int *geometry, int *handed_out);
 int modsx_debug_check_borders(const float *tuples, int n, unsigned char *touch);
 int modsx_last_timings(modsx_ctx *ctx, double *ms6);
 
diff --git a/mods_amd/__init__.py b/mods_amd/__init__.py
--- a/mods_amd/__init__.py
+++ b/mods_amd/__init__.py
@@ -99,7 +99,8 @@
            "modsx_shard_owner_plan", "modsx_db_create", "modsx_db_free", "modsx_db_rows", "modsx_db_nearest",
            "modsx_match_fginn_db", "modsx_match_fginn_db_device", "modsx_set_fginn_db",
            "modsx_debug_orientation_counts", "modsx_debug_reproject_certain_drop", "modsx_debug_describe_plan",
-           "modsx_debug_baumberg_geometry", "modsx_debug_baumberg", "modsx_debug_check_borders",
+           "modsx_debug_baumberg_geometry", "modsx_debug_baumberg_geometry_ctx", "modsx_debug_baumberg_variant",
+           "modsx_debug_baumberg", "modsx_debug_check_borders",
            "modsx_rep_create", "modsx_rep_free", "modsx_rep_add_views", "modsx_rep_append", "modsx_rep_class",
            "modsx_rep_match_fginn", "modsx_match_reps", "modsx_match_one_to_many"]
 EXPORTS_DEGENSAC = ["exp_ransacHcustom", "exp_ransacFcustom", "HDs", "HDsi", "HDsidx", "HDsSym", "HDsiSym", "HDsSymidx",
@@ -172,7 +173,9 @@
                                                 C.c_void_p, C.c_int, C.c_void_p]
         L.modsx_debug_baumberg_geometry.argtypes = [C.c_int, C.c_int, C.c_int, C.c_int, C.c_void_p]
         L.modsx_debug_baumberg.argtypes = [C.c_void_p, C.c_void_p, C.c_int, C.c_void_p, C.c_void_p, C.c_int, C.c_void_p, C.c_int, C.c_int,
-                                           C.c_void_p, C.c_void_p, C.c_void_p, C.c_void_p]
+                                           C.c_void_p, C.c_void_p, C.c_void_p, C.c_void_p, C.c_void_p]
+        L.modsx_debug_baumberg_variant.argtypes = [C.c_int]
+        L.modsx_debug_baumberg_geometry_ctx.argtypes = [C.c_void_p, C.c_int, C.c_int, C.c_int, C.c_int, C.c_void_p]
         L.modsx_debug_check_borders.argtypes = [C.c_void_p, C.c_int, C.c_void_p]
         L.modsx_rep_create.restype = C.c_void_p
         L.modsx_rep_create.argtypes = [C.c_void_p]
@@ -584,9 +587,16 @@
         u = np.zeros((max(n, 1), 4), np.float32)
         ok, iters = np.zeros(max(n, 1), np.int32), np.zeros(max(n, 1), np.int32)
         geo = np.zeros(4, np.int32)
+        handed = C.c_int(0)
         _check(lib().modsx_debug_baumberg(self._c(), ptrs, len(planes), _p(plane_of), _p(xyspd), n, C.byref(params), int(variant),
-                                          int(chunk), _p(u), _p(ok), _p(iters), _p(geo)), "debug_baumberg")
-        return dict(u=u[:n], ok=ok[:n], iters=iters[:n], geometry=dict(zip(BAUMBERG_GEOMETRY, (int(x) for x in geo))))
+                                          int(chunk), _p(u), _p(ok), _p(iters), _p(geo), C.byref(handed)), "debug_baumberg")
+        return dict(u=u[:n], ok=ok[:n], iters=iters[:n], geometry=dict(zip(BAUMBERG_GEOMETRY, (int(x) for x in geo))),
+                    handed_out=handed.value)
+
+    def baumberg_geometry(self, n, W=19, variant=0, chunk=0):
+        geo = np.zeros(4, np.int32)
+        _check(lib().modsx_debug_baumberg_geometry_ctx(self._c(), int(n), int(W), int(variant), int(chunk), _p(geo)), "baumberg_geometry")
+        return dict(zip(BAUMBERG_GEOMETRY, (int(x) for x in geo)))
 
     def detect_orientation(self, img, regs, mr_size=1.0, patch_size=41, half=0, max_ang=1, th=0.8, upright=0):
         regs = np.ascontiguousarray(regs, REGION)
@@ -858,6 +868,10 @@
     return dict(zip(BAUMBERG_GEOMETRY, (int(x) for x in geo)))
 
 
+def baumberg_production_variant(W=19):
+    return int(lib().modsx_debug_baumberg_variant(int(W)))
+
+
 def check_borders(tuples):
     t = np.ascontiguousarray(tuples, np.float32).reshape(-1, 9)
     out = np.zeros(max(1, len(t)), np.uint8)
diff --git a/mods_amd/csrc/capi.hip b/mods_amd/csrc/capi.hip
--- a/mods_amd/csrc/capi.hip
+++ b/mods_amd/csrc/capi.hip
@@ -361,15 +361,23 @@
   return MODSX_OK;
 }
 
+int modsx_debug_baumberg_geometry_ctx(modsx_ctx *ctx, int n, int W, int variant, int chunk, int *geometry) {
+  NEED(ctx); NEED(geometry);
+  hipSetDevice(ctx->dev);
+  return debug_baumberg_geometry(ctx, n, W, variant, chunk, geometry);
+}
+
+int modsx_debug_baumberg_variant(int W) { return mx::baumberg_production_variant(W); }
+
 int modsx_debug_baumberg(modsx_ctx *ctx, const modsx_image *const *planes, int nplanes, const int *plane_of, const float *xyspd,
                          int n, const modsx_hessaff_params *par, int variant, int chunk, float *u, int *ok, int *iters,
-                         int *geometry) {
+                         int *geometry, int *handed_out) {
   NEED(ctx); NEED(par); NEED(geometry);
   if (n < 0 || nplanes < 0 || (nplanes > 0 && !planes) || (n > 0 && (!plane_of || !xyspd || !u || !ok || !iters))) {
     mx::set_error("modsx_debug_baumberg: bad argument"); return MODSX_ERR_ARG;
   }
   hipSetDevice(ctx->dev);
-  return debug_baumberg(ctx, planes, nplanes, plane_of, xyspd, n, *par, variant, chunk, u, ok, iters, geometry);
+  return debug_baumberg(ctx, planes, nplanes, plane_of, xyspd, n, *par, variant, chunk, u, ok, iters, geometry, handed_out);
 }
 
 int modsx_debug_check_borders(const float *tuples, int n, unsigned char *touch) {
diff --git a/mods_amd/csrc/engine.hpp b/mods_amd/csrc/engine.hpp
--- a/mods_amd/csrc/engine.hpp
+++ b/mods_amd/csrc/engine.hpp
@@ -196,9 +196,13 @@
 constexpr int NMS_TILE_ROWS = 16;
 void launch_gray(hipStream_t s, const void *src, float *dst, size_t n, int channels, int dtype);
 struct BaumGeo { int kernel, chunk, nchunks, grid; };
-BaumGeo baumberg_geometry(int n, int W, int variant, int chunk);
-void launch_baumberg(hipStream_t s, const AffJob *jobs, AffOut *out, int n, const float *mask, int W, int maxIter,
-                     float convTh, float affInitialSigma, int variant = 0, int chunk = 0);
+BaumGeo baumberg_geometry(int n, int W, int variant, int chunk, int resident = 0);
+int baumberg_resident_waves();
+int baumberg_production_variant(int W);
+constexpr int BAUM_RANGES = 8, BAUM_COUNTER_STRIDE = 32, BAUM_QUEUE_BYTES = BAUM_RANGES * BAUM_COUNTER_STRIDE * 4;
+MX_HD int baum_range_start(int n, int r) { return (int)(((long long)n * r) / BAUM_RANGES); }
+bool launch_baumberg(hipStream_t s, const AffJob *jobs, AffOut *out, int n, const float *mask, int W, int maxIter,
+                     float convTh, float affInitialSigma, int variant, int chunk, int resident, unsigned *queue, bool queueClean);
 constexpr int ATAN_CASES = 2048 + 64;
 constexpr int ORI_NV = 1344;
 void launch_orientation(hipStream_t s, const OriJob *jobs, float *out, int n, const ImgRef *imgs,
@@ -329,6 +333,7 @@
   bool waitRuntime = true;
   mx::PinBuf hCand, hAff, hOri, hDesc, hMisc, hNms, hMatch, hViewTaps, hViewJobs, hMser, hRefs;
   float *dSmmMask = nullptr;
+  int baumResident = 0;
   int smmW = 0;
   std::vector<uint64_t> candKeys, candKeys2, candClaim;
   std::vector<uint32_t> candOrder, candOrder2;
diff --git a/mods_amd/csrc/engine_api.hpp b/mods_amd/csrc/engine_api.hpp
--- a/mods_amd/csrc/engine_api.hpp
+++ b/mods_amd/csrc/engine_api.hpp
@@ -20,8 +20,9 @@
                             std::vector<modsx_sskp> *out);
 int detect_keypoints_batch(modsx_ctx *c, const modsx_image *const *imgs, int n, const modsx_hessaff_params &par,
                            const double *tilts, const double *zooms, std::vector<modsx_keypoint> *out);
+int debug_baumberg_geometry(modsx_ctx *c, int n, int W, int variant, int chunk, int *geo);
 int debug_baumberg(modsx_ctx *c, const modsx_image *const *planes, int nplanes, const int *planeOf, const float *xyspd, int n,
-                   const modsx_hessaff_params &p, int variant, int chunk, float *u, int *ok, int *iters, int *geo);
+                   const modsx_hessaff_params &p, int variant, int chunk, float *u, int *ok, int *iters, int *geo, int *handedOut);
 void detect_affine_regions(const modsx_keypoint *kps, int n, int img_id, int det_type, modsx_region *out);
 struct OriReproj { const double *H; int orig_w, orig_h; };
 int detect_orientation_batch(modsx_ctx *c, const modsx_image *const *imgs, int n, const std::vector<modsx_region> *in,
diff --git a/mods_amd/csrc/engine_detect.hip b/mods_amd/csrc/engine_detect.hip
--- a/mods_amd/csrc/engine_detect.hip
+++ b/mods_amd/csrc/engine_detect.hip
@@ -232,11 +232,18 @@
   return nb;
 }
 
+constexpr size_t COUNTER_BYTES = (NMS_QUEUES + 1) * 128 + BAUM_QUEUE_BYTES;
+static unsigned *baum_queue(modsx_ctx *c) { return (unsigned *)c->counter.p + (NMS_QUEUES + 1) * 32; }
+static int baum_resident(modsx_ctx *c) {
+  if (!c->baumResident) { const int w = baumberg_resident_waves(); c->baumResident = w > 0 ? w : -1; }
+  return c->baumResident > 0 ? c->baumResident : 0;
+}
+
 static int scan_extrema(modsx_ctx *c, int n, const modsx_hessaff_params &p) {
   hipStream_t s = c->stream;
   if (!c->cand.ensure((size_t)CAND_CAP * sizeof(Candidate)) || !c->nmsQueue.ensure((size_t)CAND_CAP * 16)) return MODSX_ERR_NOMEM;
-  if (!c->counter.ensure((NMS_QUEUES + 1) * 128)) return MODSX_ERR_NOMEM;
-  MX_HIP(hipMemsetAsync(c->counter.p, 0, 128 + NMS_QUEUES * 128, s));
+  if (!c->counter.ensure(COUNTER_BYTES)) return MODSX_ERR_NOMEM;
+  MX_HIP(hipMemsetAsync(c->counter.p, 0, COUNTER_BYTES, s));
   bool queuesClean = true;
   const NmsBatch nb = nms_thresholds(p);
   int maxOct = 0;
@@ -479,9 +486,17 @@
   return MODSX_OK;
 }
 
+int debug_baumberg_geometry(modsx_ctx *c, int n, int W, int variant, int chunk, int *geo) {
+  const BaumGeo g = baumberg_geometry(n, W, variant, chunk, baum_resident(c));
+  geo[0] = g.kernel; geo[1] = g.chunk; geo[2] = g.nchunks; geo[3] = g.grid;
+  if (g.kernel < 0) { set_error("modsx_debug_baumberg_geometry_ctx: no kernel for this window size / variant / chunk"); return MODSX_ERR_ARG; }
+  return MODSX_OK;
+}
+
 int debug_baumberg(modsx_ctx *c, const modsx_image *const *planes, int nplanes, const int *planeOf, const float *xyspd, int n,
-                   const modsx_hessaff_params &p, int variant, int chunk, float *u, int *ok, int *iters, int *geo) {
-  const BaumGeo g = baumberg_geometry(n, p.smmWindowSize, variant, chunk);
+                   const modsx_hessaff_params &p, int variant, int chunk, float *u, int *ok, int *iters, int *geo, int *handedOut) {
+  const BaumGeo g = baumberg_geometry(n, p.smmWindowSize, variant, chunk, baum_resident(c));
+  if (handedOut) *handedOut = 0;
   if (g.kernel < 0) { set_error("modsx_debug_baumberg: no kernel for this window size / variant / chunk"); return MODSX_ERR_ARG; }
   geo[0] = g.kernel; geo[1] = g.chunk; geo[2] = g.nchunks; geo[3] = g.grid;
   for (int i = 0; i < nplanes; i++)
@@ -500,6 +515,7 @@
   const size_t total = (size_t)n;
   if (!c->hAff.ensure(total * sizeof(AffJob) + total * sizeof(AffOut))) return MODSX_ERR_NOMEM;
   if (!c->affJobs.ensure(total * sizeof(AffJob)) || !c->affOut.ensure(total * sizeof(AffOut))) return MODSX_ERR_NOMEM;
+  if (!c->counter.ensure(COUNTER_BYTES) || !c->hMisc.ensure(BAUM_QUEUE_BYTES)) return MODSX_ERR_NOMEM;
   AffJob *hj = (AffJob *)c->hAff.p;
   AffOut *ho = (AffOut *)((char *)c->hAff.p + total * sizeof(AffJob));
   for (int k = 0; k < n; k++) {
@@ -512,11 +528,22 @@
   hipStream_t s = c->stream;
   MX_HIP(hipMemcpyAsync(c->affJobs.p, hj, total * sizeof(AffJob), hipMemcpyHostToDevice, s));
   MX_HIP(hipMemsetAsync(c->affOut.p, 0xFF, total * sizeof(AffOut), s));
-  launch_baumberg(s, (AffJob *)c->affJobs.p, (AffOut *)c->affOut.p, n, c->dSmmMask, p.smmWindowSize, p.maxIterations,
-                  p.convergenceThreshold, p.affInitialSigma, variant, chunk);
+  if (!launch_baumberg(s, (AffJob *)c->affJobs.p, (AffOut *)c->affOut.p, n, c->dSmmMask, p.smmWindowSize, p.maxIterations,
+                       p.convergenceThreshold, p.affInitialSigma, variant, chunk, baum_resident(c), baum_queue(c), false)) {
+    MX_HIP(hipGetLastError());
+    set_error("modsx_debug_baumberg: nothing was launched"); return MODSX_ERR_INTERNAL;
+  }
   MX_HIP(hipGetLastError());
   MX_HIP(hipMemcpyAsync(ho, c->affOut.p, total * sizeof(AffOut), hipMemcpyDeviceToHost, s));
+  if (g.kernel == 3) MX_HIP(hipMemcpyAsync(c->hMisc.p, baum_queue(c), BAUM_QUEUE_BYTES, hipMemcpyDeviceToHost, s));
   MX_HIP(hipStreamSynchronize(s));
+  if (g.kernel == 3 && handedOut) {
+    const unsigned *w = (const unsigned *)c->hMisc.p;
+    for (int r = 0; r < BAUM_RANGES; r++) {
+      const unsigned len = (unsigned)(baum_range_start(n, r + 1) - baum_range_start(n, r));
+      *handedOut += (int)std::min(w[BAUM_COUNTER_STRIDE * r], len);
+    }
+  }
   for (int k = 0; k < n; k++) {
     u[4 * k] = ho[k].u11; u[4 * k + 1] = ho[k].u12; u[4 * k + 2] = ho[k].u21; u[4 * k + 3] = ho[k].u22;
     ok[k] = ho[k].ok; iters[k] = ho[k].iters;
@@ -596,8 +623,16 @@
   if (p.doBaumberg) {
     MX_HIP(ctx_copy(c, c->affJobs.p, hj, total * sizeof(AffJob), hipMemcpyHostToDevice));
     ProfScope ps(c, K_BAUMBERG, (double)total * 361 * 4 * 2);
-    launch_baumberg(s, (AffJob *)c->affJobs.p, (AffOut *)c->affOut.p, (int)total, c->dSmmMask, p.smmWindowSize,
-                    p.maxIterations, p.convergenceThreshold, p.affInitialSigma);
+    const int variant = baumberg_production_variant(p.smmWindowSize);
+    if (variant == 3 && !baum_resident(c)) {
+      set_error("Baumberg: the occupancy query that sizes the queue form's grid failed (MODSX_BAUMBERG_QUEUE=0 runs the static chunks)");
+      return MODSX_ERR_DEVICE;
+    }
+    if (!launch_baumberg(s, (AffJob *)c->affJobs.p, (AffOut *)c->affOut.p, (int)total, c->dSmmMask, p.smmWindowSize, p.maxIterations,
+                         p.convergenceThreshold, p.affInitialSigma, variant, 0, baum_resident(c), baum_queue(c), true)) {
+      MX_HIP(hipGetLastError());
+      set_error("Baumberg: no kernel for this window size"); return MODSX_ERR_INTERNAL;
+    }
     MX_HIP(ctx_copy(c, ho, c->affOut.p, total * sizeof(AffOut), hipMemcpyDeviceToHost));
     MX_HIP(ctx_sync(c));
   } else {
diff --git a/mods_amd/csrc/kernels_affine.hip b/mods_amd/csrc/kernels_affine.hip
--- a/mods_amd/csrc/kernels_affine.hip
+++ b/mods_amd/csrc/kernels_affine.hip
@@ -1,4 +1,5 @@
 #include "engine.hpp"
+#include <algorithm>
 
 namespace mx {
 
@@ -172,9 +173,13 @@
 #ifndef MODSX_BAUMBERG_K
 #define MODSX_BAUMBERG_K 2
 #endif
-template <int K>
+#ifndef MODSX_BAUMBERG_STEAL
+#define MODSX_BAUMBERG_STEAL 1
+#endif
+template <int K, bool QUEUE>
 __global__ __launch_bounds__(64) void k_baumberg_stream(const AffJob *jobs, AffOut *out, int n, const float *mask, int chunk,
-                                                        int nchunks, int maxIter, float convTh, float affInitialSigma) {
+                                                        int nchunks, int maxIter, float convTh, float affInitialSigma,
+                                                        unsigned *queue) {
   constexpr int W = AW_MAX, WW = W * W, half = W >> 1, CH = AW_MAX * AW_MAX + 3;
   constexpr int PERM = (WW + 63) / 64;
   __shared__ __attribute__((aligned(16))) float buf[K][3][CH];
@@ -199,10 +204,25 @@
   float slx = 0.f, sly = 0.f;
   int scols = 4, srows = 4;
   int ok = 0, it = 0, kidx = -1;
-  int next = min(xcd_chunk(blockIdx.x, nchunks) * chunk, n);
-  const int end = min(next + chunk, n);
+  int next = QUEUE ? 0 : min(xcd_chunk(blockIdx.x, nchunks) * chunk, n);
+  const int end = QUEUE ? 0 : min(next + chunk, n);
+  int rg = blockIdx.x & (BAUM_RANGES - 1);
+  unsigned emptyRanges = MODSX_BAUMBERG_STEAL ? 0u : ((1u << BAUM_RANGES) - 1u) & ~(1u << rg);
   bool live = false;
   if (maxIter <= 0) {
+    if constexpr (QUEUE) {
+      for (int t = 0; t < BAUM_RANGES; t++, rg = (rg + 1) & (BAUM_RANGES - 1)) {
+        const int lo = baum_range_start(n, rg), len = baum_range_start(n, rg + 1) - lo;
+        for (;;) {
+          unsigned got = 0;
+          if (lane == 0) got = atomicAdd(queue + BAUM_COUNTER_STRIDE * rg, 64u);
+          got = __builtin_amdgcn_readfirstlane(got);
+          if (got >= (unsigned)len) break;
+          if (got + lane < (unsigned)len) { AffOut o; o.u11 = 1; o.u12 = 0; o.u21 = 0; o.u22 = 1; o.ok = 0; o.iters = 0; out[lo + (int)got + lane] = o; }
+        }
+      }
+      return;
+    }
     for (int i = next + lane; i < end; i += 64) { AffOut o; o.u11 = 1; o.u12 = 0; o.u21 = 0; o.u22 = 1; o.ok = 0; o.iters = 0; out[i] = o; }
     return;
   }
@@ -214,18 +234,45 @@
       const bool want = slotLane && !live;
       const unsigned long long wm = __ballot(want && !(lane & 1));
       const int rank = __popcll(wm & ((1ull << (lane & ~1)) - 1ull));
-      const int cand = next + rank;
-      if (want && cand < end) {
-        kidx = cand;
-        const AffJob sj = jobs[cand];
-        ratio = sj.s / (affInitialSigma * sj.pixelDistance);
-        slx = sj.x / sj.pixelDistance; sly = sj.y / sj.pixelDistance;
-        scols = sj.cols; srows = sj.rows;
-        u11 = 1.0f; u12 = 0.0f; u21 = 0.0f; u22 = 1.0f; l1 = 1.0f; l2 = 1.0f; era = 0.0f; erb = 0.0f;
-        ok = 0; it = 0;
-        live = true;
-      }
-      next = min(next + __popcll(wm), end);
+      if constexpr (QUEUE) {
+        int need = __popcll(wm), done = 0;
+        while (need > 0 && emptyRanges != (1u << BAUM_RANGES) - 1u) {
+          const int lo = baum_range_start(n, rg), len = baum_range_start(n, rg + 1) - lo;
+          unsigned got = 0;
+          if (lane == 0) got = atomicAdd(queue + BAUM_COUNTER_STRIDE * rg, (unsigned)need);
+          got = __builtin_amdgcn_readfirstlane(got);
+          const int avail = got >= (unsigned)len ? 0 : min(need, len - (int)got);
+          if (want && rank >= done && rank < done + avail) {
+            const int cand = lo + (int)got + (rank - done);
+            kidx = cand;
+            const AffJob sj = jobs[cand];
+            ratio = sj.s / (affInitialSigma * sj.pixelDistance);
+            slx = sj.x / sj.pixelDistance; sly = sj.y / sj.pixelDistance;
+            scols = sj.cols; srows = sj.rows;
+            u11 = 1.0f; u12 = 0.0f; u21 = 0.0f; u22 = 1.0f; l1 = 1.0f; l2 = 1.0f; era = 0.0f; erb = 0.0f;
+            ok = 0; it = 0;
+            live = true;
+          }
+          done += avail; need -= avail;
+          if (need > 0) {
+            emptyRanges |= 1u << rg;
+            for (int t = 1; t < BAUM_RANGES && ((emptyRanges >> rg) & 1u); t++) rg = (rg + 1) & (BAUM_RANGES - 1);
+          }
+        }
+      } else {
+        const int cand = next + rank;
+        if (want && cand < end) {
+          kidx = cand;
+          const AffJob sj = jobs[cand];
+          ratio = sj.s / (affInitialSigma * sj.pixelDistance);
+          slx = sj.x / sj.pixelDistance; sly = sj.y / sj.pixelDistance;
+          scols = sj.cols; srows = sj.rows;
+          u11 = 1.0f; u12 = 0.0f; u21 = 0.0f; u22 = 1.0f; l1 = 1.0f; l2 = 1.0f; era = 0.0f; erb = 0.0f;
+          ok = 0; it = 0;
+          live = true;
+        }
+        next = min(next + __popcll(wm), end);
+      }
     }
     const unsigned long long liveMask = __ballot(live);
     if (!liveMask) break;
@@ -420,10 +467,37 @@
 #define MODSX_BAUMBERG_CHUNK 8
 #endif
 
-BaumGeo baumberg_geometry(int n, int W, int variant, int chunk) {
+int baumberg_resident_waves() {
+  int dev = 0, cus = 0, perCu = 0;
+  if (hipGetDevice(&dev) != hipSuccess || hipDeviceGetAttribute(&cus, hipDeviceAttributeMultiprocessorCount, dev) != hipSuccess ||
+      hipOccupancyMaxActiveBlocksPerMultiprocessor(&perCu, k_baumberg_stream<MODSX_BAUMBERG_K, true>, 64, 0) != hipSuccess ||
+      cus <= 0 || perCu <= 0) { (void)hipGetLastError(); return 0; }
+  return cus * perCu;
+}
+
+#ifndef MODSX_BAUMBERG_QUEUE_DEFAULT
+#define MODSX_BAUMBERG_QUEUE_DEFAULT 1
+#endif
+int baumberg_production_variant(int W) {
+  static const char *const env = getenv("MODSX_BAUMBERG_QUEUE");
+  static const bool queue = env ? atoi(env) != 0 : MODSX_BAUMBERG_QUEUE_DEFAULT != 0;
+  return (queue && W == AW_MAX && MODSX_BAUMBERG_K > 1) ? 3 : 0;
+}
+
+BaumGeo baumberg_geometry(int n, int W, int variant, int chunk, int resident) {
   constexpr int K = MODSX_BAUMBERG_K;
   BaumGeo g = {-1, 0, 0, 0};
   if (n < 0 || chunk < 0 || W < 3 || W > AW_MAX || !(W & 1)) return g;
+  if (variant == 3) {
+    if (W != AW_MAX || K <= 1 || chunk > (1 << 20)) return g;
+    if (!chunk) {
+      if (resident <= 0) return g;
+      const long long waves = std::min<long long>(resident, ((long long)n + K - 1) / K);
+      chunk = (int)((waves + BAUM_RANGES - 1) / BAUM_RANGES);
+    }
+    g.kernel = 3; g.chunk = chunk; g.nchunks = BAUM_RANGES; g.grid = BAUM_RANGES * chunk;
+    return g;
+  }
   if (variant == 0) g.kernel = W == AW_MAX ? (K > 1 ? 0 : 1) : 2;
   else if (variant == 1 && W == AW_MAX) g.kernel = 1;
   else if (variant == 2) g.kernel = 2;
@@ -439,16 +513,25 @@
   return g;
 }
 
-void launch_baumberg(hipStream_t s, const AffJob *jobs, AffOut *out, int n, const float *mask, int W, int maxIter,
-                     float convTh, float affInitialSigma, int variant, int chunk) {
-  if (n <= 0) return;
+bool launch_baumberg(hipStream_t s, const AffJob *jobs, AffOut *out, int n, const float *mask, int W, int maxIter,
+                     float convTh, float affInitialSigma, int variant, int chunk, int resident, unsigned *queue, bool queueClean) {
+  if (n <= 0) return true;
   constexpr int K = MODSX_BAUMBERG_K;
-  const BaumGeo g = baumberg_geometry(n, W, variant, chunk);
+  const BaumGeo g = baumberg_geometry(n, W, variant, chunk, resident);
   if (g.kernel == 0) {
-    MX_DUP(K_BAUMBERG) hipLaunchKernelGGL(k_baumberg_stream<K>, dim3(g.grid), dim3(64), 0, s, jobs, out, n, mask, g.chunk, g.nchunks, maxIter,
-                       convTh, affInitialSigma);
+    MX_DUP(K_BAUMBERG) hipLaunchKernelGGL((k_baumberg_stream<K, false>), dim3(g.grid), dim3(64), 0, s, jobs, out, n, mask, g.chunk, g.nchunks,
+                       maxIter, convTh, affInitialSigma, (unsigned *)nullptr);
+  } else if (g.kernel == 3 && queue) {
+    MX_DUP(K_BAUMBERG) {
+      if (!queueClean && hipMemsetAsync(queue, 0, BAUM_QUEUE_BYTES, s) != hipSuccess) return false;
+      queueClean = false;
+      hipLaunchKernelGGL((k_baumberg_stream<K, true>), dim3(g.grid), dim3(64), 0, s, jobs, out, n, mask, g.chunk, g.nchunks, maxIter,
+                         convTh, affInitialSigma, queue);
+    }
   } else if (g.kernel == 1) hipLaunchKernelGGL(k_baumberg<19>, dim3(n), dim3(64), 0, s, jobs, out, n, mask, W, maxIter, convTh, affInitialSigma);
   else if (g.kernel == 2) hipLaunchKernelGGL(k_baumberg<0>, dim3(n), dim3(64), 0, s, jobs, out, n, mask, W, maxIter, convTh, affInitialSigma);
+  else return false;
+  return true;
 }
 
 }
```

After: 228.7, median of 6. 3.1% higher.
